# LilYau350/Variance-Aware-Weight

Hardware: AMD Instinct MI355X
Metric: training images/sec (higher is better)
Workload: dtype bf16; 1 GPU; DiT-B/4, 4x32x32 latents, 1000 classes; Trainer.train_step: q_sample + fwd + lambda-weighted MSE + bwd + AdamW + EMA; global batch 256 = 256 per GPU; global_batch=256, per_gpu_batch=256, parallelism=dp1, weight_type=lambda, hip_graph=False

## Files before the change

### include/vaw_hip.h

```cpp
#ifndef VAW_HIP_H
#define VAW_HIP_H
#include <stdint.h>

#ifdef __cplusplus
extern "C" {
#endif

typedef enum { VAW_OK = 0, VAW_ERR_INVALID = -1, VAW_ERR_LAUNCH = -2, VAW_ERR_UNSUPPORTED = -3 } vaw_status;
typedef enum { VAW_F32 = 0, VAW_BF16 = 1,
               VAW_FP8 = 2, VAW_BF8 = 3  } vaw_dtype;
typedef void* vaw_stream;

int vaw_version(void);
const char* vaw_last_error_string(void);


int vaw_qsample_fwd(const float* x0, const float* noise, const int64_t* t, const float* tab_a, const float* tab_s,
                    int num_timesteps, float* x_t, int B, int64_t per_sample, vaw_stream stream);

int vaw_mix_rows(const float* x, const float* y, const float* ca, const float* cb, float* out, int B,
                 int64_t per_sample, vaw_stream stream);

int vaw_wmse_fwd(const float* model_out, const float* x0, const float* noise, const float* ca, const float* cb,
                 const float* w, float* mse, int B, int64_t per_sample, vaw_stream stream);
int vaw_wmse_bwd(const float* model_out, const float* x0, const float* noise, const float* ca, const float* cb,
                 const float* w, const float* gmse, float* dout, int B, int64_t per_sample, vaw_stream stream);

int vaw_vb_fwd(const float* mean_out, const float* var_out, const float* x0, const float* x_t, const float* coef,
               int mean_mode, int var_mode, float scale, float* vb, int B, int64_t per_sample, vaw_stream stream);
int vaw_vb_bwd(const float* mean_out, const float* var_out, const float* x0, const float* x_t, const float* coef,
               int mean_mode, int var_mode, float scale, const float* gvb, float* d_mean, float* d_var, int B,
               int64_t per_sample, vaw_stream stream);

int vaw_sample_step(int kind, const float* mean_out, const float* var_out, const float* x, const float* noise,
                    const float* coef, int mean_mode, int var_mode, int clip_denoised, float eta, float* sample,
                    float* pred_xstart, float* mean, float* log_variance, int B, int64_t per_sample, vaw_stream stream);


typedef struct {
    const float* bias;
    int act;
    const void* aux_in;
    void* aux_out;
    const float* gate;
    int64_t gate_ld;
    const void* resid;
    const float* rowadd;
    int rows_per_batch;
    float alpha;
    float beta;
    int out_f32;
    float* colsum_out;
    float colsum_beta;
    int resid_is_act;
    float* rowsum_a_out;
    float rowsum_a_beta;
    float* colsum_partial_out;
    int64_t* colsum_rows_out;
} vaw_epilogue;

int vaw_gemm(vaw_dtype dt, int a_kmajor, int b_kmajor, int64_t M, int64_t N, int64_t K, const void* A, int64_t lda,
             const void* B, int64_t ldb, void* C, int64_t ldc, const vaw_epilogue* epi_host, float* workspace,
             int64_t workspace_floats, vaw_stream stream);

typedef struct {
    const void* dy;
    const void* x;
    float* dw;
    int64_t M, N, ld_dy, ld_x, ld_dw;
    float alpha;
    int pad_;
    const float* scale_dy;
    const float* scale_x;
} vaw_wgrad_problem;
int64_t vaw_wgrad_grouped_desc_bytes(int n_problems);
int vaw_wgrad_grouped(vaw_dtype dt, int n_problems, const vaw_wgrad_problem* problems, int64_t K, float beta, void* desc_dev,
                      int upload, float* workspace, int64_t workspace_floats, vaw_stream stream);

int64_t vaw_fp8_quantize_workspace_floats(void);
int vaw_fp8_quantize(vaw_dtype src_dt, vaw_dtype dst_format, const void* src, int64_t R, int64_t C, int64_t ld, void* q, int64_t ldq,
                     void* qt, int64_t ldt, float* scale_out, float* workspace, int64_t workspace_floats, vaw_stream stream);
int vaw_fp8_quantize_delayed(vaw_dtype src_dt, vaw_dtype dst_format, const void* src, int64_t R, int64_t C, int64_t ld, void* q,
                             int64_t ldq, void* qt, int64_t ldt, float* state, vaw_stream stream);
int vaw_fp8_scale_update(float* states, int64_t n, vaw_stream stream);
typedef struct {
    const float* src;
    void* q;
    void* qt;
    float* state;
    int64_t R, C, ld, ldq, ldt;
} vaw_fp8_quant_job;
int64_t vaw_fp8_quantize_batched_desc_bytes(int n_jobs);
int vaw_fp8_quantize_delayed_batched(int n_jobs, const vaw_fp8_quant_job* jobs, void* desc_dev, int upload, vaw_stream stream);
int vaw_gemm_fp8(vaw_dtype a_format, int64_t M, int64_t N, int64_t K, const void* A, int64_t lda, const float* scale_a,
                 const void* B, int64_t ldb, const float* scale_b, void* C, int64_t ldc, const vaw_epilogue* epi_host,
                 float* c_fp8_state, vaw_dtype c_fp8_format, float* workspace, int64_t workspace_floats, vaw_stream stream);
int vaw_fp8_transpose(const void* q, int64_t R, int64_t C, int64_t ldq, void* qt, int64_t ldt, vaw_stream stream);

void vaw_p8_set_reserved_cus(int n);
int vaw_gemm_uses_bf16_mfma(vaw_dtype dt, int64_t M, int64_t N, int64_t K, const void* A, int64_t lda, const void* B,
                            int64_t ldb);

int64_t vaw_colsum_workspace_floats(int64_t M, int64_t N);
int vaw_colsum(vaw_dtype dt, const void* X, int64_t M, int64_t N, int64_t ldx, float* out, float beta,
               float* workspace, int64_t workspace_floats, vaw_stream stream);
int vaw_reduce_rows(const float* partial, int64_t R, int64_t N, float* out, float beta, vaw_stream stream);
typedef struct {
    const float* partial;
    float* out;
    int64_t R, N;
} vaw_reduce_job;
int64_t vaw_reduce_rows_batched_desc_bytes(int n_jobs);
int vaw_reduce_rows_batched(int n_jobs, const vaw_reduce_job* jobs, float beta, void* desc_dev, int upload, vaw_stream stream);


int vaw_ln_modulate_fwd(vaw_dtype dt, const float* x, const float* shift, const float* scale, int64_t mod_ld,
                        void* out, float* mean, float* rstd, int B, int T, int D, float eps, vaw_stream stream);
int vaw_ln_modulate_bwd(vaw_dtype dt, const void* dout, const float* x, const float* mean, const float* rstd,
                        const float* scale, int64_t mod_ld, const float* dres_in, float* dx, float* dshift,
                        float* dscale, int64_t dmod_ld, int B, int T, int D, float* workspace, int64_t workspace_floats,
                        vaw_stream stream);
int vaw_ln_modulate_fwd_fp8(const float* x, const float* shift, const float* scale, int64_t mod_ld, void* q_out, float* q_state,
                            vaw_dtype q_format, float* mean, float* rstd, int B, int T, int D, float eps, vaw_stream stream);
int vaw_gate_bwd_fp8(const float* dres, const void* y, const float* gate, int64_t mod_ld, void* dy_q, float* q_state,
                     vaw_dtype q_format, float* dgate, int64_t dmod_ld, float* dy_colsum_partial, int B, int T, int D,
                     float* workspace, int64_t workspace_floats, vaw_stream stream);
int64_t vaw_row_bwd_workspace_floats(int B, int T, int D);
typedef enum { VAW_ROW_LN_FWD = 0, VAW_ROW_LN_FWD_FP8 = 1, VAW_ROW_LN_BWD = 2, VAW_ROW_GATE_BWD = 3, VAW_ROW_GATE_BWD_FP8 = 4,
               VAW_ROW_LN_BWD_GATE = 5, VAW_ROW_LN_BWD_GATE_FP8 = 6, VAW_ROW_COLSUM = 7 } vaw_row_kind;
typedef enum {
    VAW_RV_LN_FWD = 0,
    VAW_RV_ROW_BWD = 1,
    VAW_RV_ROW_GATE = 2,
    VAW_RV_ROW_FUSE = 3,
    VAW_RV_ROW_FUSE8 = 4,
    VAW_RV_COLSUM_BF16X8 = 5, VAW_RV_COLSUM_VEC4 = 6, VAW_RV_COLSUM_SCALAR = 7
} vaw_row_variant;
typedef struct {
    int variant;
    int nv;
    int nc, rows_per_chunk;
    int grid_x, block;
    int64_t lds_bytes;
    int64_t workspace_floats;
} vaw_row_launch;
int vaw_row_plan(vaw_row_kind kind, vaw_dtype dt, int64_t B, int64_t T, int64_t D, int64_t ldx, int64_t base_addr,
                 int64_t workspace_floats, vaw_row_launch* out);
int vaw_gate_bwd(vaw_dtype dt, const float* dres, const void* y, const float* gate, int64_t mod_ld, void* dy,
                 float* dgate, int64_t dmod_ld, float* dy_colsum_partial, int B, int T, int D, float* workspace, int64_t workspace_floats, vaw_stream stream);
int vaw_ln_modulate_bwd_gate(vaw_dtype dt, const void* dout, const float* x, const float* mean, const float* rstd,
                             const float* scale, int64_t mod_ld, const float* dres_in, float* dx, float* dshift, float* dscale,
                             int64_t dmod_ld, const void* y_next, const float* gate_next, void* dy_next, float* dgate_next,
                             float* dy_colsum_partial, int B, int T, int D, float* workspace, int64_t workspace_floats, vaw_stream stream);
int vaw_ln_modulate_bwd_gate_fp8(const void* dout, const float* x, const float* mean, const float* rstd, const float* scale,
                                 int64_t mod_ld, const float* dres_in, float* dx, float* dshift, float* dscale, int64_t dmod_ld,
                                 const void* y_next, const float* gate_next, void* dy_q, float* q_state, vaw_dtype q_format,
                                 float* dgate_next, float* dy_colsum_partial, int B, int T, int D, float* workspace,
                                 int64_t workspace_floats, vaw_stream stream);

int vaw_patchify(vaw_dtype dt, const float* img, void* tok, int B, int C, int H, int W, int p, vaw_stream stream);
int vaw_patchify_bwd(const float* dtok, float* dimg, int B, int C, int H, int W, int p, vaw_stream stream);
int vaw_unpatchify(vaw_dtype dt, const float* tok, float* img, int B, int C, int H, int W, int p,
                   vaw_stream stream);
int vaw_unpatchify_bwd(vaw_dtype dt, const float* dimg, void* dtok, int B, int C, int H, int W, int p,
                       vaw_stream stream);

int vaw_timestep_embedding(vaw_dtype dt, const float* t, void* out, int B, int dim, float max_period,
                           vaw_stream stream);
int vaw_silu_fwd(vaw_dtype dt, const float* x, void* out, int64_t n, vaw_stream stream);
int vaw_silu_bwd(const float* x, const float* dy, float* dx, int64_t n, vaw_stream stream);
int vaw_add_embedding(const float* a, const float* table, const int64_t* idx, float* out, int B, int D,
                      int num_rows, vaw_stream stream);
int vaw_embedding_bwd(const float* dc, const int64_t* idx, float* dtable, int B, int D, int num_rows, float beta,
                      vaw_stream stream);

typedef struct {
    int B, H, T, hd;
    int64_t q_sb, q_sh, q_st, q_sd;
    int64_t o_sb, o_sh, o_st, o_sd;
    float scale;
} vaw_attn_desc;
int vaw_attn_fwd(vaw_dtype dt, const vaw_attn_desc* d_host, const void* q, const void* k, const void* v, void* o,
                 float* lse, vaw_stream stream);
int vaw_attn_bwd(vaw_dtype dt, const vaw_attn_desc* d_host, const void* q, const void* k, const void* v,
                 const void* o, const void* d_o, const float* lse, float* delta, void* dq, void* dk, void* dv,
                 vaw_stream stream);
int vaw_attn_bwd_colsum(vaw_dtype dt, const vaw_attn_desc* d, const void* q, const void* k, const void* v, const void* o,
                        const void* d_o, const float* lse, float* delta, void* dq, void* dk, void* dv, float* colsum_partial,
                        int64_t* rows_out, vaw_stream stream);

typedef enum { VAW_ATTN_DIR_FWD = 0, VAW_ATTN_DIR_BWD = 1, VAW_ATTN_DIR_BWD_COLSUM = 2 } vaw_attn_dir;
typedef enum {
    VAW_AV_ROWWISE = 0,
    VAW_AV_FWD_T64 = 1,
    VAW_AV_FWD_G1 = 2,
    VAW_AV_FWD_G2 = 3,
    VAW_AV_FWD_BIG = 4,
    VAW_AV_BWD_T64 = 5,
    VAW_AV_BWD_G1 = 6,
    VAW_AV_BWD_G2 = 7,
    VAW_AV_BWD_BIG_NT2 = 8,
    VAW_AV_BWD_BIG_NT4 = 9
} vaw_attn_variant;
typedef struct {
    int variant;
    int hd_image;
    int launches;
    int grid_x, grid_y, block;
    int64_t lds_bytes;
    int lds_cap_raised;
    int64_t colsum_rows;
    int status;
} vaw_attn_launch;
int vaw_attn_plan(int dir, vaw_dtype dt, const vaw_attn_desc* d, int64_t q, int64_t k, int64_t v, int64_t o_or_do, int64_t dq,
                  int64_t dk, int64_t dv, vaw_attn_launch* out);


int vaw_conv3x3_narrow(vaw_dtype dt, int mode, const void* in, const void* w, const float* bias, void* out, int B, int H,
                       int W, int Cn, int Cw, vaw_stream stream);

int64_t vaw_groupnorm_workspace_floats(int B, int HW, int C);
int vaw_groupnorm_fwd(vaw_dtype dt, const void* x, const float* gamma, const float* beta, const float* scale,
                      const float* shift, int64_t film_ld, int silu, void* y, float* mean, float* rstd, int B, int HW,
                      int C, int G, float eps, float* workspace, vaw_stream stream);
int vaw_groupnorm_bwd(vaw_dtype dt, const void* dout, const void* x, const float* mean, const float* rstd,
                      const float* gamma, const float* beta, const float* scale, const float* shift, int64_t film_ld,
                      int silu, const void* dx_add, void* dx, float* dgamma, float* dbeta, float grad_beta, float* dscale,
                      float* dshift, int64_t dfilm_ld, int B, int HW, int C, int G, float* workspace, vaw_stream stream);
int vaw_im2col3x3(vaw_dtype dt, const void* x, void* col, int B, int H, int W, int C, vaw_stream stream);
int vaw_col2im3x3(vaw_dtype dt, const void* dcol, void* dx, int B, int H, int W, int C, vaw_stream stream);
int vaw_conv3x3(vaw_dtype dt, int mode, const void* act, const void* act2, const void* w, void* out, int B, int H, int W,
                int Ci, int Co, const vaw_epilogue* epi_host, float* workspace, int64_t workspace_floats, vaw_stream stream);
int64_t vaw_conv3x3_wgrad_small_workspace_floats(int B, int H, int W, int Ci, int Co);
int vaw_conv3x3_wgrad_small(vaw_dtype dt, const void* dy, const void* x, float* dw, float beta, int B, int H, int W, int Ci,
                            int Co, float* workspace, int64_t workspace_floats, vaw_stream stream);
int vaw_resample2(vaw_dtype dt, const void* in, void* out, int B, int Ho, int Wo, int C, int mode, float s,
                  vaw_stream stream);
int vaw_concat_channels(vaw_dtype dt, void* a, void* b, void* cat, int64_t M, int Ca, int Cb, int split,
                        vaw_stream stream);
int vaw_add_inplace(vaw_dtype dt, void* dst, const void* src, int64_t n, vaw_stream stream);
int vaw_mul(vaw_dtype dt, const void* a, const void* b, void* out, int64_t n, vaw_stream stream);
int vaw_subsample2(vaw_dtype dt, const void* in, void* out, int B, int Ho, int Wo, int C, int mode, vaw_stream stream);
int vaw_rowvec_add(vaw_dtype dt, void* h, const float* e, int64_t ld, int B, int HW, int C, vaw_stream stream);
int vaw_rowvec_sum(vaw_dtype dt, const void* dh, float* de, int64_t ld, int B, int HW, int C, float beta, vaw_stream stream);
int vaw_nchw_to_nhwc(vaw_dtype dt, const float* nchw, void* nhwc, int B, int C, int HW, vaw_stream stream);
int vaw_nhwc_to_nchw(vaw_dtype dt, const void* nhwc, float* nchw, int B, int C, int HW, vaw_stream stream);


int64_t vaw_sumsq_workspace_floats(void);
int vaw_sumsq(const float* g, int64_t n, float* sumsq_out, int accumulate, float* workspace, vaw_stream stream);
int vaw_adamw_ema_step(float* p, float* g, float* m, float* v, float* ema, void* shadow_bf16, int64_t n, float lr,
                       float beta1, float beta2, float eps, float weight_decay, float bc1, float bc2,
                       float ema_decay, const float* sumsq, float clip_max_norm, int zero_grad, vaw_stream stream);
// ... 21 lines not shown
```

### variance-aware-weight_amd/_lib.py

```python
import ctypes as C
import os

import torch

_HERE = os.path.dirname(os.path.abspath(__file__))
LIB_PATH = os.environ.get("VAW_HIP_LIB") or os.path.join(_HERE, "libvaw_hip.so")

F32, BF16, FP8, BF8 = 0, 1, 2, 3
TORCH_DTYPE = {F32: torch.float32, BF16: torch.bfloat16}

_p, _i, _l, _f = C.c_void_p, C.c_int, C.c_int64, C.c_float


class Epilogue(C.Structure):
    _fields_ = [("bias", _p), ("act", _i), ("aux_in", _p), ("aux_out", _p), ("gate", _p), ("gate_ld", _l),
                ("resid", _p), ("rowadd", _p), ("rows_per_batch", _i), ("alpha", _f), ("beta", _f), ("out_f32", _i),
                ("colsum_out", _p), ("colsum_beta", _f), ("resid_is_act", _i), ("rowsum_a_out", _p), ("rowsum_a_beta", _f),
                ("colsum_partial_out", _p), ("colsum_rows_out", C.POINTER(C.c_int64))]


class AttnDesc(C.Structure):
    _fields_ = [("B", _i), ("H", _i), ("T", _i), ("hd", _i), ("q_sb", _l), ("q_sh", _l), ("q_st", _l), ("q_sd", _l),
                ("o_sb", _l), ("o_sh", _l), ("o_st", _l), ("o_sd", _l), ("scale", _f)]


class RowLaunch(C.Structure):
    _fields_ = [("variant", _i), ("nv", _i), ("nc", _i), ("rows_per_chunk", _i), ("grid_x", _i), ("block", _i), ("lds_bytes", _l),
                ("workspace_floats", _l)]


class AttnLaunch(C.Structure):
    _fields_ = [("variant", _i), ("hd_image", _i), ("launches", _i), ("grid_x", _i), ("grid_y", _i), ("block", _i), ("lds_bytes", _l),
                ("lds_cap_raised", _i), ("colsum_rows", _l), ("status", _i)]


ATTN_FWD, ATTN_BWD, ATTN_BWD_COLSUM = range(3)
(AV_ROWWISE, AV_FWD_T64, AV_FWD_G1, AV_FWD_G2, AV_FWD_BIG, AV_BWD_T64, AV_BWD_G1, AV_BWD_G2, AV_BWD_BIG_NT2,
 AV_BWD_BIG_NT4) = range(10)
AV_NAMES = ("rowwise", "fwd_t64", "fwd_g1", "fwd_g2", "fwd_big", "bwd_t64", "bwd_g1", "bwd_g2", "bwd_big_nt2", "bwd_big_nt4")

ROW_LN_FWD, ROW_LN_FWD_FP8, ROW_LN_BWD, ROW_GATE_BWD, ROW_GATE_BWD_FP8, ROW_LN_BWD_GATE, ROW_LN_BWD_GATE_FP8, ROW_COLSUM = range(8)
RV_LN_FWD, RV_ROW_BWD, RV_ROW_GATE, RV_ROW_FUSE, RV_ROW_FUSE8, RV_COLSUM_BF16X8, RV_COLSUM_VEC4, RV_COLSUM_SCALAR = range(8)

_PROTOS = {
    "vaw_qsample_fwd": [_p, _p, _p, _p, _p, _i, _p, _i, _l, _p],
    "vaw_mix_rows": [_p, _p, _p, _p, _p, _i, _l, _p],
    "vaw_wmse_fwd": [_p, _p, _p, _p, _p, _p, _p, _i, _l, _p],
    "vaw_wmse_bwd": [_p, _p, _p, _p, _p, _p, _p, _p, _i, _l, _p],
    "vaw_gemm": [_i, _i, _i, _l, _l, _l, _p, _l, _p, _l, _p, _l, C.POINTER(Epilogue), _p, _l, _p],
    "vaw_gemm_uses_bf16_mfma": [_i, _l, _l, _l, _p, _l, _p, _l],
    "vaw_colsum": [_i, _p, _l, _l, _l, _p, _f, _p, _l, _p],
    "vaw_ln_modulate_fwd": [_i, _p, _p, _p, _l, _p, _p, _p, _i, _i, _i, _f, _p],
    "vaw_ln_modulate_bwd": [_i, _p, _p, _p, _p, _p, _l, _p, _p, _p, _p, _l, _i, _i, _i, _p, _l, _p],
    "vaw_gate_bwd": [_i, _p, _p, _p, _l, _p, _p, _l, _p, _i, _i, _i, _p, _l, _p],
    "vaw_reduce_rows": [_p, _l, _l, _p, _f, _p],
    "vaw_reduce_rows_batched": [_i, _p, _f, _p, _i, _p],
    "vaw_ln_modulate_bwd_gate": [_i, _p, _p, _p, _p, _p, _l, _p, _p, _p, _p, _l, _p, _p, _p, _p, _p, _i, _i, _i, _p, _l, _p],
    "vaw_ln_modulate_bwd_gate_fp8": [_p, _p, _p, _p, _p, _l, _p, _p, _p, _p, _l, _p, _p, _p, _p, _i, _p, _p, _i, _i, _i, _p, _l, _p],
    "vaw_patchify": [_i, _p, _p, _i, _i, _i, _i, _i, _p],
    "vaw_patchify_bwd": [_p, _p, _i, _i, _i, _i, _i, _p],
    "vaw_unpatchify": [_i, _p, _p, _i, _i, _i, _i, _i, _p],
    "vaw_unpatchify_bwd": [_i, _p, _p, _i, _i, _i, _i, _i, _p],
    "vaw_timestep_embedding": [_i, _p, _p, _i, _i, _f, _p],
    "vaw_silu_fwd": [_i, _p, _p, _l, _p],
    "vaw_silu_bwd": [_p, _p, _p, _l, _p],
    "vaw_add_embedding": [_p, _p, _p, _p, _i, _i, _i, _p],
    "vaw_embedding_bwd": [_p, _p, _p, _i, _i, _i, _f, _p],
    "vaw_attn_fwd": [_i, C.POINTER(AttnDesc), _p, _p, _p, _p, _p, _p],
    "vaw_attn_bwd": [_i, C.POINTER(AttnDesc), _p, _p, _p, _p, _p, _p, _p, _p, _p, _p, _p],
    "vaw_attn_bwd_colsum": [_i, C.POINTER(AttnDesc), _p, _p, _p, _p, _p, _p, _p, _p, _p, _p, _p, C.POINTER(C.c_int64), _p],
    "vaw_comm_unique_id": [_p],
    "vaw_comm_init": [_p, _i, _i],
    "vaw_comm_world": [],
    "vaw_comm_destroy": [],
    "vaw_allreduce_bucket_start": [_p, _l, _i, _p],
    "vaw_reduce_scatter_bucket_start": [_p, _l, _i, _p],
    "vaw_allgather_bucket_start": [_p, _l, _i, _p],
    "vaw_allreduce_bucket_wait": [_p],
    "vaw_groupnorm_fwd": [_i, _p, _p, _p, _p, _p, _l, _i, _p, _p, _p, _i, _i, _i, _i, _f, _p, _p],
    "vaw_groupnorm_bwd": [_i, _p, _p, _p, _p, _p, _p, _p, _p, _l, _i, _p, _p, _p, _p, _f, _p, _p, _l, _i, _i, _i, _i, _p, _p],
    "vaw_im2col3x3": [_i, _p, _p, _i, _i, _i, _i, _p],
    "vaw_col2im3x3": [_i, _p, _p, _i, _i, _i, _i, _p],
    "vaw_conv3x3": [_i, _i, _p, _p, _p, _p, _i, _i, _i, _i, _i, C.POINTER(Epilogue), _p, _l, _p],
    "vaw_vb_fwd": [_p, _p, _p, _p, _p, _i, _i, _f, _p, _i, _l, _p],
    "vaw_vb_bwd": [_p, _p, _p, _p, _p, _i, _i, _f, _p, _p, _p, _i, _l, _p],
    "vaw_sample_step": [_i, _p, _p, _p, _p, _p, _i, _i, _i, _f, _p, _p, _p, _p, _i, _l, _p],
    "vaw_conv3x3_narrow": [_i, _i, _p, _p, _p, _p, _i, _i, _i, _i, _i, _p],
    "vaw_conv3x3_wgrad_small": [_i, _p, _p, _p, _f, _i, _i, _i, _i, _i, _p, _l, _p],
    "vaw_resample2": [_i, _p, _p, _i, _i, _i, _i, _i, _f, _p],
    "vaw_concat_channels": [_i, _p, _p, _p, _l, _i, _i, _i, _p],
    "vaw_add_inplace": [_i, _p, _p, _l, _p],
    "vaw_mul": [_i, _p, _p, _p, _l, _p],
    "vaw_subsample2": [_i, _p, _p, _i, _i, _i, _i, _i, _p],
    "vaw_rowvec_add": [_i, _p, _p, _l, _i, _i, _i, _p],
    "vaw_rowvec_sum": [_i, _p, _p, _l, _i, _i, _i, _f, _p],
    "vaw_nchw_to_nhwc": [_i, _p, _p, _i, _i, _i, _p],
    "vaw_nhwc_to_nchw": [_i, _p, _p, _i, _i, _i, _p],
    "vaw_sumsq": [_p, _l, _p, _i, _p, _p],
    "vaw_adamw_ema_step_dev": [_p, _p, _p, _p, _p, _p, _l, _p, _f, _f, _f, _f, _f, _p, _f, _i, _p],
    "vaw_adamw_ema_step": [_p, _p, _p, _p, _p, _p, _l, _f, _f, _f, _f, _f, _f, _f, _f, _p, _f, _i, _p],
    "vaw_ema_update": [_p, _p, _l, _f, _p],
    "vaw_cast_bf16": [_p, _p, _l, _p],
    "vaw_uncast_bf16": [_p, _p, _l, _f, _p],
    "vaw_wgrad_grouped": [_i, _i, _p, _l, _f, _p, _i, _p, _l, _p],
    "vaw_fp8_quantize": [_i, _i, _p, _l, _l, _l, _p, _l, _p, _l, _p, _p, _l, _p],
    "vaw_fp8_quantize_delayed": [_i, _i, _p, _l, _l, _l, _p, _l, _p, _l, _p, _p],
    "vaw_fp8_scale_update": [_p, _l, _p],
    "vaw_fp8_quantize_delayed_batched": [_i, _p, _p, _i, _p],
    "vaw_gemm_fp8": [_i, _l, _l, _l, _p, _l, _p, _p, _l, _p, _p, _l, C.POINTER(Epilogue), _p, _i, _p, _l, _p],
    "vaw_fp8_transpose": [_p, _l, _l, _l, _p, _l, _p],
    "vaw_ln_modulate_fwd_fp8": [_p, _p, _p, _l, _p, _p, _i, _p, _p, _i, _i, _i, _f, _p],
    "vaw_gate_bwd_fp8": [_p, _p, _p, _l, _p, _p, _i, _p, _l, _p, _i, _i, _i, _p, _l, _p],
    "vaw_row_plan": [_i, _i, _l, _l, _l, _l, _l, _l, C.POINTER(RowLaunch)],
    "vaw_attn_plan": [_i, _i, C.POINTER(AttnDesc), _l, _l, _l, _l, _l, _l, _l, C.POINTER(AttnLaunch)],
}

_lib = None


class VawError(RuntimeError):
    pass


def lib():
    global _lib
    if _lib is None:
        if not os.path.exists(LIB_PATH):
            raise VawError(f"{LIB_PATH} not found: build it with `python -c 'import __graft_entry__ as g; g.build()'` "
                           "(there is no CPU fallback for the HIP path)")
        L = C.CDLL(LIB_PATH)
        for name, args in _PROTOS.items():
            if not hasattr(L, name) and os.environ.get("VAW_HIP_LIB"):
                continue
            fn = getattr(L, name)
            fn.argtypes = args
            fn.restype = _i
        L.vaw_version.restype = _i
        L.vaw_last_error_string.restype = C.c_char_p
        L.vaw_colsum_workspace_floats.argtypes = [_l, _l]
        L.vaw_colsum_workspace_floats.restype = _l
        L.vaw_row_bwd_workspace_floats.argtypes = [_i, _i, _i]
        L.vaw_row_bwd_workspace_floats.restype = _l
        L.vaw_conv3x3_wgrad_small_workspace_floats.argtypes = [_i, _i, _i, _i, _i]
        L.vaw_conv3x3_wgrad_small_workspace_floats.restype = _l
        L.vaw_groupnorm_workspace_floats.argtypes = [_i, _i, _i]
        L.vaw_groupnorm_workspace_floats.restype = _l
        L.vaw_wgrad_grouped_desc_bytes.argtypes = [_i]
        L.vaw_wgrad_grouped_desc_bytes.restype = _l
# ... 51 lines not shown
```

### variance-aware-weight_amd/csrc/capi.hip

```cpp
#include <stdarg.h>
#include <stdio.h>

#include "common.h"

static thread_local char g_err[512] = "";

void vaw_set_error(const char* fmt, ...) {
    va_list ap;
    va_start(ap, fmt);
    vsnprintf(g_err, sizeof(g_err), fmt, ap);
    va_end(ap);
}

extern "C" int vaw_version(void) { return 100; }
extern "C" const char* vaw_last_error_string(void) { return g_err; }

__global__ void __launch_bounds__(64) cu_hog_kernel(uint64_t ticks) {
    extern __shared__ char hog_lds[];
    if (threadIdx.x == 0) hog_lds[0] = 1;
    const uint64_t t0 = __builtin_amdgcn_s_memrealtime();
    while (__builtin_amdgcn_s_memrealtime() - t0 < ticks) __builtin_amdgcn_s_sleep(64);
}
extern "C" int vaw_debug_cu_hog(int n_wgs, int microseconds, vaw_stream stream) {
    VAW_CHECK_ARG(n_wgs > 0 && n_wgs <= 256 && microseconds > 0 && microseconds <= 2000000, "cu_hog: arguments");
    static bool attr = false;
    if (!attr) { (void)hipFuncSetAttribute((const void*)cu_hog_kernel, hipFuncAttributeMaxDynamicSharedMemorySize, 160 * 1024); attr = true; }
    cu_hog_kernel<<<n_wgs, 64, 160 * 1024, (hipStream_t)stream>>>((uint64_t)microseconds * 100);
    VAW_CHECK_LAUNCH("cu_hog");
    return VAW_OK;
}

#include <mutex>
#include <string.h>
#include <vector>
hipError_t vaw_upload_table(void* dev, const void* host, size_t bytes, hipStream_t s) {
    static std::mutex mu;
    static std::vector<void*> keep;
    void* pinned = nullptr;
    hipError_t rc = hipHostMalloc(&pinned, bytes, hipHostMallocDefault);
    if (rc != hipSuccess) return rc;
    memcpy(pinned, host, bytes);
    {
        std::lock_guard<std::mutex> g(mu);
        keep.push_back(pinned);
    }
    return hipMemcpyAsync(dev, pinned, bytes, hipMemcpyHostToDevice, s);
}
```

### variance-aware-weight_amd/csrc/elementwise.hip

```cpp
#include "common.h"

static inline int stream_grid(int64_t work_items, int block) {
    int64_t g = (work_items + block - 1) / block;
    const int64_t cap = 256 * 8;
    return (int)(g < 1 ? 1 : (g > cap ? cap : g));
}

template <bool GATHER>
__global__ void mix_rows_kernel(const float* __restrict__ x, const float* __restrict__ y, const float* __restrict__ ca,
                                const float* __restrict__ cb, const int64_t* __restrict__ t, int T,
                                float* __restrict__ out, int64_t n) {
    const int b = blockIdx.y;
    float a, c;
    if (GATHER) {
        const int64_t tt = t[b];
        const bool ok = tt >= 0 && tt < T;
        a = ok ? ca[tt] : __builtin_nanf("");
        c = ok ? cb[tt] : __builtin_nanf("");
    } else {
        a = ca[b];
        c = cb[b];
    }
    const float* xr = x + (int64_t)b * n;
    const float* yr = y + (int64_t)b * n;
    float* orow = out + (int64_t)b * n;
    const int64_t n4 = ((n & 3) == 0) ? n / 4 : 0;
    for (int64_t i = blockIdx.x * (int64_t)blockDim.x + threadIdx.x; i < n4; i += (int64_t)gridDim.x * blockDim.x) {
        f32x4 xv = load4(xr + 4 * i), yv = load4(yr + 4 * i);
        store4(orow + 4 * i, a * xv + c * yv);
    }
    for (int64_t i = n4 * 4 + blockIdx.x * (int64_t)blockDim.x + threadIdx.x; i < n; i += (int64_t)gridDim.x * blockDim.x)
        orow[i] = a * xr[i] + c * yr[i];
}

extern "C" int vaw_qsample_fwd(const float* x0, const float* noise, const int64_t* t, const float* tab_a,
                               const float* tab_s, int num_timesteps, float* x_t, int B, int64_t per_sample,
                               vaw_stream stream) {
    VAW_CHECK_ARG(B > 0 && per_sample > 0 && num_timesteps > 0, "qsample: bad sizes B=%d n=%ld", B, (long)per_sample);
    int gx = stream_grid(per_sample / 4 + 1, 256);
    dim3 grid(gx > 64 ? 64 : gx, B);
    mix_rows_kernel<true><<<grid, 256, 0, (hipStream_t)stream>>>(x0, noise, tab_a, tab_s, t, num_timesteps, x_t, per_sample);
    VAW_CHECK_LAUNCH("qsample");
    return VAW_OK;
}

extern "C" int vaw_mix_rows(const float* x, const float* y, const float* ca, const float* cb, float* out, int B,
                            int64_t per_sample, vaw_stream stream) {
    VAW_CHECK_ARG(B > 0 && per_sample > 0, "mix_rows: bad sizes");
    int gx = stream_grid(per_sample / 4 + 1, 256);
    dim3 grid(gx > 64 ? 64 : gx, B);
    mix_rows_kernel<false><<<grid, 256, 0, (hipStream_t)stream>>>(x, y, ca, cb, nullptr, 0, out, per_sample);
    VAW_CHECK_LAUNCH("mix_rows");
    return VAW_OK;
}

__global__ void wmse_fwd_kernel(const float* __restrict__ o, const float* __restrict__ x0, const float* __restrict__ nz,
                                const float* __restrict__ ca, const float* __restrict__ cb, const float* __restrict__ w,
                                float* __restrict__ mse, int64_t n) {
    __shared__ float scratch[16];
    const int b = blockIdx.x;
    const float a = ca[b], c = cb[b];
    const float* orow = o + (int64_t)b * n;
    const float* xr = x0 + (int64_t)b * n;
    const float* nr = nz + (int64_t)b * n;
    float acc = 0.f;
    const int64_t n4 = ((n & 3) == 0) ? n / 4 : 0;
    for (int64_t i = threadIdx.x; i < n4; i += blockDim.x) {
        f32x4 d = a * load4(xr + 4 * i) + c * load4(nr + 4 * i) - load4(orow + 4 * i);
        acc += d[0] * d[0] + d[1] * d[1] + d[2] * d[2] + d[3] * d[3];
    }
    for (int64_t i = n4 * 4 + threadIdx.x; i < n; i += blockDim.x) {
        float d = a * xr[i] + c * nr[i] - orow[i];
        acc += d * d;
    }
    float tot = block_sum(acc, scratch);
    if (threadIdx.x == 0) mse[b] = w[b] * (tot / (float)n);
}

__global__ void wmse_bwd_kernel(const float* __restrict__ o, const float* __restrict__ x0, const float* __restrict__ nz,
                                const float* __restrict__ ca, const float* __restrict__ cb, const float* __restrict__ w,
                                const float* __restrict__ gmse, float* __restrict__ dout, int64_t n) {
    const int b = blockIdx.y;
    const float a = ca[b], c = cb[b];
    const float k = gmse[b] * w[b] * 2.f / (float)n;
    const float* orow = o + (int64_t)b * n;
    const float* xr = x0 + (int64_t)b * n;
    const float* nr = nz + (int64_t)b * n;
    float* dr = dout + (int64_t)b * n;
    const int64_t n4 = ((n & 3) == 0) ? n / 4 : 0;
    for (int64_t i = blockIdx.x * (int64_t)blockDim.x + threadIdx.x; i < n4; i += (int64_t)gridDim.x * blockDim.x)
        store4(dr + 4 * i, k * (load4(orow + 4 * i) - a * load4(xr + 4 * i) - c * load4(nr + 4 * i)));
    for (int64_t i = n4 * 4 + blockIdx.x * (int64_t)blockDim.x + threadIdx.x; i < n; i += (int64_t)gridDim.x * blockDim.x)
        dr[i] = k * (orow[i] - a * xr[i] - c * nr[i]);
}

extern "C" int vaw_wmse_fwd(const float* model_out, const float* x0, const float* noise, const float* ca,
                            const float* cb, const float* w, float* mse, int B, int64_t per_sample,
                            vaw_stream stream) {
    VAW_CHECK_ARG(B > 0 && per_sample > 0, "wmse_fwd: bad sizes");
    wmse_fwd_kernel<<<B, 1024, 0, (hipStream_t)stream>>>(model_out, x0, noise, ca, cb, w, mse, per_sample);
    VAW_CHECK_LAUNCH("wmse_fwd");
    return VAW_OK;
}

extern "C" int vaw_wmse_bwd(const float* model_out, const float* x0, const float* noise, const float* ca,
                            const float* cb, const float* w, const float* gmse, float* dout, int B,
                            int64_t per_sample, vaw_stream stream) {
    VAW_CHECK_ARG(B > 0 && per_sample > 0, "wmse_bwd: bad sizes");
    int gx = stream_grid(per_sample / 4 + 1, 256);
    dim3 grid(gx > 64 ? 64 : gx, B);
    wmse_bwd_kernel<<<grid, 256, 0, (hipStream_t)stream>>>(model_out, x0, noise, ca, cb, w, gmse, dout, per_sample);
    VAW_CHECK_LAUNCH("wmse_bwd");
    return VAW_OK;
}

#define VB_NCOEF 8
struct VbElem {
    float val;
    float d_lv;
    float d_mean;
};
__device__ __forceinline__ float vb_cdf(float z, float& dcdf) {
    const float k = 0.7978845608028654f;
    const float th = tanhf(k * (z + 0.044715f * (z * z * z)));
    dcdf = 0.5f * (1.f - th * th) * k * (1.f + 3.f * 0.044715f * z * z);
    return 0.5f * (1.f + th);
}
__device__ __forceinline__ VbElem vb_elem(float x0, float true_mean, float true_lv, float mean, float lv, bool t0) {
    VbElem r;
    if (!t0) {
        const float e2 = expf(-lv), d = true_mean - mean, ratio = expf(true_lv - lv);
        r.val = 0.5f * (-1.0f + lv - true_lv + ratio + (d * d) * e2);
        r.d_lv = 0.5f * (1.f - ratio - (d * d) * e2);
        r.d_mean = -d * e2;
        return r;
    }
    const float cx = x0 - mean, inv = expf(-(0.5f * lv));
    const float pin = inv * (cx + 1.0f / 255.0f), mnn = inv * (cx - 1.0f / 255.0f);
    float dp, dm;
    const float cp = vb_cdf(pin, dp), cm = vb_cdf(mnn, dm);
    float lp, g_pin = 0.f, g_min = 0.f;
    if (x0 < -0.999f) {
        lp = logf(fmaxf(cp, 1e-12f));
        if (cp >= 1e-12f) g_pin = dp / cp;
    } else if (x0 > 0.999f) {
        const float q = 1.f - cm;
        lp = logf(fmaxf(q, 1e-12f));
        if (q >= 1e-12f) g_min = -dm / q;
    } else {
        const float dl = cp - cm;
        lp = logf(fmaxf(dl, 1e-12f));
        if (dl >= 1e-12f) { g_pin = dp / dl; g_min = -dm / dl; }
    }
    r.val = -lp;
    r.d_lv = 0.5f * (g_pin * pin + g_min * mnn);
    r.d_mean = inv * (g_pin + g_min);
    return r;
}
__device__ __forceinline__ void vb_model(const float* c, int mean_mode, int var_mode, float xt, float m, float v, float& mean,
                                         float& lv) {
    mean = mean_mode == 1 ? m : c[0] * (c[4] * xt + c[5] * m) + c[1] * xt;
    if (var_mode == 1) lv = v;
    else if (var_mode == 2) { const float frac = (v + 1.f) / 2.f; lv = frac * c[3] + (1.f - frac) * c[2]; }
    else lv = c[3];
}

__global__ void vb_fwd_kernel(const float* __restrict__ mean_out, const float* __restrict__ var_out, const float* __restrict__ x0,
                              const float* __restrict__ xt, const float* __restrict__ coef, int mean_mode, int var_mode,
                              float scale, float* __restrict__ vb, int64_t n) {
    __shared__ float scratch[16];
    const int b = blockIdx.x;
    float c[VB_NCOEF];
#pragma unroll
    for (int i = 0; i < VB_NCOEF; ++i) c[i] = coef[b * VB_NCOEF + i];
    const bool t0 = c[6] != 0.f;
    const int64_t base = (int64_t)b * n;
    float acc = 0.f;
    for (int64_t i = threadIdx.x; i < n; i += blockDim.x) {
        const float x = x0[base + i], z = xt[base + i];
        float mean, lv;
        vb_model(c, mean_mode, var_mode, z, mean_out[base + i], var_out ? var_out[base + i] : 0.f, mean, lv);
        acc += vb_elem(x, c[0] * x + c[1] * z, c[2], mean, lv, t0).val;
    }
    const float tot = block_sum(acc, scratch);
    if (threadIdx.x == 0) vb[b] = scale * ((tot / (float)n) / 0.6931471805599453f);
}

__global__ void vb_bwd_kernel(const float* __restrict__ mean_out, const float* __restrict__ var_out, const float* __restrict__ x0,
                              const float* __restrict__ xt, const float* __restrict__ coef, int mean_mode, int var_mode,
                              float scale, const float* __restrict__ gvb, float* __restrict__ d_mean, float* __restrict__ d_var,
                              int64_t n) {
    const int b = blockIdx.y;
    float c[VB_NCOEF];
#pragma unroll
    for (int i = 0; i < VB_NCOEF; ++i) c[i] = coef[b * VB_NCOEF + i];
// ... 48 lines not shown
    for (int i = 0; i < SS_NCOEF; ++i) c[i] = coef[b * SS_NCOEF + i];
    const float mask = c[11] != 0.f ? 0.f : 1.f;
    const float sigma = (eta * c[9]) * c[12];
    const float ddim_c = sqrtf(1.f - c[10] - sigma * sigma);
    const int64_t base = (int64_t)b * n;
    for (int64_t i = blockIdx.x * (int64_t)blockDim.x + threadIdx.x; i < n; i += (int64_t)gridDim.x * blockDim.x) {
        const float xv = x[base + i], m = mean_out[base + i];
        float pred = c[0] * xv + c[1] * m;
        if (clip) pred = fminf(fmaxf(pred, -1.f), 1.f);
        float lv;
        if (var_mode == 1) lv = var_out[base + i];
        else if (var_mode == 2) { const float frac = (var_out[base + i] + 1.f) / 2.f; lv = frac * c[5] + (1.f - frac) * c[4]; }
        else lv = c[5];
        const float mean = mean_mode == 1 ? m : c[2] * pred + c[3] * xv;
        if (pred_out) pred_out[base + i] = pred;
        if (mean_o) mean_o[base + i] = mean;
        if (logvar_o) logvar_o[base + i] = lv;
        if (kind == 1) {
            sample[base + i] = mean + (mask * expf(0.5f * lv)) * noise[base + i];
        } else if (kind == 2) {
            const float eps = (c[6] * xv - pred) / c[7];
            const float mp = pred * c[8] + ddim_c * eps;
            sample[base + i] = mp + (mask * sigma) * noise[base + i];
        }
    }
}

extern "C" int vaw_sample_step(int kind, const float* mean_out, const float* var_out, const float* x, const float* noise,
                               const float* coef, int mean_mode, int var_mode, int clip_denoised, float eta, float* sample,
                               float* pred_xstart, float* mean, float* log_variance, int B, int64_t per_sample,
                               vaw_stream stream) {
    VAW_CHECK_ARG(B > 0 && per_sample > 0 && mean_out && x && coef && kind >= 0 && kind <= 2, "sample_step: bad arguments");
    VAW_CHECK_ARG((mean_mode == 0 || mean_mode == 1) && var_mode >= 0 && var_mode <= 2 && (var_mode == 0 || var_out),
                  "sample_step: bad modes (learned variance needs var_out)");
    VAW_CHECK_ARG(kind == 0 || (sample && noise), "sample_step: kind 1/2 need noise and sample");
    int gx = stream_grid(per_sample, 256);
    dim3 grid(gx > 64 ? 64 : gx, B);
    sample_step_kernel<<<grid, 256, 0, (hipStream_t)stream>>>(mean_out, var_out, x, noise, coef, kind, mean_mode, var_mode,
                                                             clip_denoised, eta, sample, pred_xstart, mean, log_variance, per_sample);
    VAW_CHECK_LAUNCH("sample_step");
    return VAW_OK;
}

template <typename T>
__global__ void timestep_embedding_kernel(const float* __restrict__ t, T* __restrict__ out, int B, int dim,
                                          float neg_log_period) {
    const int half = dim / 2;
    for (int64_t idx = blockIdx.x * (int64_t)blockDim.x + threadIdx.x; idx < (int64_t)B * dim;
         idx += (int64_t)gridDim.x * blockDim.x) {
        const int b = (int)(idx / dim), j = (int)(idx % dim);
        float v = 0.f;
        if (j < 2 * half) {
            const int i = j < half ? j : j - half;
            const float f = expf(neg_log_period * (float)i / (float)half);
            const float ang = t[b] * f;
            v = j < half ? cosf(ang) : sinf(ang);
        }
        out[idx] = from_f32<T>(v);
    }
}

extern "C" int vaw_timestep_embedding(vaw_dtype dt, const float* t, void* out, int B, int dim, float max_period,
                                      vaw_stream stream) {
    VAW_CHECK_ARG(B > 0 && dim > 0, "timestep_embedding: bad sizes");
    const float nl = -logf(max_period);
    int grid = stream_grid((int64_t)B * dim, 256);
    if (dt == VAW_F32)
        timestep_embedding_kernel<float><<<grid, 256, 0, (hipStream_t)stream>>>(t, (float*)out, B, dim, nl);
    else
        timestep_embedding_kernel<bf16_t><<<grid, 256, 0, (hipStream_t)stream>>>(t, (bf16_t*)out, B, dim, nl);
    VAW_CHECK_LAUNCH("timestep_embedding");
    return VAW_OK;
}

template <typename T>
__global__ void silu_fwd_kernel(const float* __restrict__ x, T* __restrict__ out, int64_t n) {
    for (int64_t i = blockIdx.x * (int64_t)blockDim.x + threadIdx.x; i < n; i += (int64_t)gridDim.x * blockDim.x)
        out[i] = from_f32<T>(silu_f(x[i]));
}
__global__ void silu_bwd_kernel(const float* __restrict__ x, const float* __restrict__ dy, float* __restrict__ dx, int64_t n) {
    for (int64_t i = blockIdx.x * (int64_t)blockDim.x + threadIdx.x; i < n; i += (int64_t)gridDim.x * blockDim.x)
        dx[i] = dy[i] * silu_grad_f(x[i]);
}
extern "C" int vaw_silu_fwd(vaw_dtype dt, const float* x, void* out, int64_t n, vaw_stream stream) {
    VAW_CHECK_ARG(n > 0, "silu_fwd: n<=0");
    int grid = stream_grid(n, 256);
    if (dt == VAW_F32) silu_fwd_kernel<float><<<grid, 256, 0, (hipStream_t)stream>>>(x, (float*)out, n);
    else silu_fwd_kernel<bf16_t><<<grid, 256, 0, (hipStream_t)stream>>>(x, (bf16_t*)out, n);
    VAW_CHECK_LAUNCH("silu_fwd");
    return VAW_OK;
}
extern "C" int vaw_silu_bwd(const float* x, const float* dy, float* dx, int64_t n, vaw_stream stream) {
    VAW_CHECK_ARG(n > 0, "silu_bwd: n<=0");
    silu_bwd_kernel<<<stream_grid(n, 256), 256, 0, (hipStream_t)stream>>>(x, dy, dx, n);
    VAW_CHECK_LAUNCH("silu_bwd");
    return VAW_OK;
}

__global__ void add_embedding_kernel(const float* __restrict__ a, const float* __restrict__ table,
                                     const int64_t* __restrict__ idx, float* __restrict__ out, int B, int D, int rows) {
    for (int64_t i = blockIdx.x * (int64_t)blockDim.x + threadIdx.x; i < (int64_t)B * D; i += (int64_t)gridDim.x * blockDim.x) {
        const int b = (int)(i / D), d = (int)(i % D);
        const int64_t r = idx[b];
        out[i] = a[i] + ((r >= 0 && r < rows) ? table[r * D + d] : __builtin_nanf(""));
    }
}
__global__ void __launch_bounds__(256)
embedding_bwd_kernel(const float* __restrict__ dc, const int64_t* __restrict__ idx, float* __restrict__ dtable, int B, int D,
                     int rows, float beta) {
    __shared__ int s_idx[1024];
    const int r = blockIdx.x;
    constexpr int MAXC = 8;
    for (int d0 = 0; d0 < D; d0 += 256 * MAXC) {
        float acc[MAXC];
#pragma unroll
        for (int j = 0; j < MAXC; ++j) acc[j] = 0.f;
        for (int b0 = 0; b0 < B; b0 += 1024) {
            const int nb = B - b0 < 1024 ? B - b0 : 1024;
            __syncthreads();
            for (int i = threadIdx.x; i < nb; i += 256) s_idx[i] = (int)idx[b0 + i];
            __syncthreads();
            for (int i = 0; i < nb; ++i) {
                if (s_idx[i] != r) continue;
                const float* src = dc + (int64_t)(b0 + i) * D + d0;
#pragma unroll
                for (int j = 0; j < MAXC; ++j) {
                    const int d = threadIdx.x + 256 * j;
                    if (d0 + d < D) acc[j] += src[d];
                }
            }
        }
#pragma unroll
        for (int j = 0; j < MAXC; ++j) {
            const int d = d0 + threadIdx.x + 256 * j;
            if (d < D) {
                float* o = dtable + (int64_t)r * D + d;
                *o = (beta != 0.f ? beta * *o : 0.f) + acc[j];
            }
        }
    }
}
extern "C" int vaw_add_embedding(const float* a, const float* table, const int64_t* idx, float* out, int B, int D,
                                 int num_rows, vaw_stream stream) {
    VAW_CHECK_ARG(B > 0 && D > 0 && num_rows > 0, "add_embedding: bad sizes");
    add_embedding_kernel<<<stream_grid((int64_t)B * D, 256), 256, 0, (hipStream_t)stream>>>(a, table, idx, out, B, D, num_rows);
    VAW_CHECK_LAUNCH("add_embedding");
    return VAW_OK;
}
extern "C" int vaw_embedding_bwd(const float* dc, const int64_t* idx, float* dtable, int B, int D, int num_rows,
                                 float beta, vaw_stream stream) {
    VAW_CHECK_ARG(B > 0 && D > 0 && num_rows > 0, "embedding_bwd: bad sizes");
    embedding_bwd_kernel<<<num_rows, 256, 0, (hipStream_t)stream>>>(dc, idx, dtable, B, D, num_rows, beta);
    VAW_CHECK_LAUNCH("embedding_bwd");
    return VAW_OK;
}

template <typename T, bool CONV_ORDER, bool TO_TOKENS>
__global__ void patch_shuffle_kernel(const float* __restrict__ img_in, float* __restrict__ img_out,
                                     const float* __restrict__ tok_in_f32, T* __restrict__ tok_out, int B, int C, int H,
                                     int W, int p) {
    const int hp = H / p, wp = W / p;
    const int64_t total = (int64_t)B * C * H * W;
    const int K = C * p * p;
    for (int64_t e = blockIdx.x * (int64_t)blockDim.x + threadIdx.x; e < total; e += (int64_t)gridDim.x * blockDim.x) {
        int x = (int)(e % W);
        int64_t r = e / W;
        int y = (int)(r % H);
        r /= H;
        int c = (int)(r % C);
        int b = (int)(r / C);
        const int ty = y / p, i = y % p, tx = x / p, j = x % p;
        const int64_t row = ((int64_t)b * hp + ty) * wp + tx;
        const int col = CONV_ORDER ? (c * p + i) * p + j : (i * p + j) * C + c;
        if (TO_TOKENS) tok_out[row * K + col] = from_f32<T>(img_in[e]);
        else img_out[e] = tok_in_f32[row * K + col];
    }
}

extern "C" int vaw_patchify(vaw_dtype dt, const float* img, void* tok, int B, int C, int H, int W, int p,
                            vaw_stream stream) {
    VAW_CHECK_ARG(B > 0 && C > 0 && p > 0 && H % p == 0 && W % p == 0, "patchify: bad sizes");
    int grid = stream_grid((int64_t)B * C * H * W, 256);
    if (dt == VAW_F32)
        patch_shuffle_kernel<float, true, true><<<grid, 256, 0, (hipStream_t)stream>>>(img, nullptr, nullptr, (float*)tok, B, C, H, W, p);
    else
        patch_shuffle_kernel<bf16_t, true, true><<<grid, 256, 0, (hipStream_t)stream>>>(img, nullptr, nullptr, (bf16_t*)tok, B, C, H, W, p);
    VAW_CHECK_LAUNCH("patchify");
    return VAW_OK;
}
extern "C" int vaw_patchify_bwd(const float* dtok, float* dimg, int B, int C, int H, int W, int p, vaw_stream stream) {
    VAW_CHECK_ARG(B > 0 && C > 0 && p > 0 && H % p == 0 && W % p == 0, "patchify_bwd: bad sizes");
    int grid = stream_grid((int64_t)B * C * H * W, 256);
    patch_shuffle_kernel<float, true, false><<<grid, 256, 0, (hipStream_t)stream>>>(nullptr, dimg, dtok, nullptr, B, C, H, W, p);
    VAW_CHECK_LAUNCH("patchify_bwd");
    return VAW_OK;
}
extern "C" int vaw_unpatchify(vaw_dtype dt, const float* tok, float* img, int B, int C, int H, int W, int p,
                              vaw_stream stream) {
    (void)dt;
    VAW_CHECK_ARG(B > 0 && C > 0 && p > 0 && H % p == 0 && W % p == 0, "unpatchify: bad sizes");
    int grid = stream_grid((int64_t)B * C * H * W, 256);
    patch_shuffle_kernel<float, false, false><<<grid, 256, 0, (hipStream_t)stream>>>(nullptr, img, tok, nullptr, B, C, H, W, p);
    VAW_CHECK_LAUNCH("unpatchify");
    return VAW_OK;
}
extern "C" int vaw_unpatchify_bwd(vaw_dtype dt, const float* dimg, void* dtok, int B, int C, int H, int W, int p,
                                  vaw_stream stream) {
    VAW_CHECK_ARG(B > 0 && C > 0 && p > 0 && H % p == 0 && W % p == 0, "unpatchify_bwd: bad sizes");
    int grid = stream_grid((int64_t)B * C * H * W, 256);
    if (dt == VAW_F32)
        patch_shuffle_kernel<float, false, true><<<grid, 256, 0, (hipStream_t)stream>>>(dimg, nullptr, nullptr, (float*)dtok, B, C, H, W, p);
    else
        patch_shuffle_kernel<bf16_t, false, true><<<grid, 256, 0, (hipStream_t)stream>>>(dimg, nullptr, nullptr, (bf16_t*)dtok, B, C, H, W, p);
    VAW_CHECK_LAUNCH("unpatchify_bwd");
    return VAW_OK;
}

#define SUMSQ_MAX_BLOCKS 2048
__global__ void sumsq_partial_kernel(const float* __restrict__ g, int64_t n, float* __restrict__ partial) {
    __shared__ float scratch[16];
    float acc = 0.f;
    const int64_t n4 = n / 4;
    for (int64_t i = blockIdx.x * (int64_t)blockDim.x + threadIdx.x; i < n4; i += (int64_t)gridDim.x * blockDim.x) {
        f32x4 v = load4(g + 4 * i);
        acc += v[0] * v[0] + v[1] * v[1] + v[2] * v[2] + v[3] * v[3];
    }
    for (int64_t i = n4 * 4 + blockIdx.x * (int64_t)blockDim.x + threadIdx.x; i < n; i += (int64_t)gridDim.x * blockDim.x)
        acc += g[i] * g[i];
    float tot = block_sum(acc, scratch);
// ... 184 lines not shown
```

### variance-aware-weight_amd/csrc/layernorm.hip

```cpp
#include <stdio.h>
#include <stdlib.h>

#include "common.h"

template <typename T, int NV>
__global__ void __launch_bounds__(256)
ln_modulate_fwd_kernel(const float* __restrict__ x, const float* __restrict__ shift, const float* __restrict__ scale,
                       int64_t mod_ld, T* __restrict__ out, float* __restrict__ mean_out, float* __restrict__ rstd_out,
                       int64_t M, int Tt, int D, float eps, unsigned char* __restrict__ q_out = nullptr,
                       float* __restrict__ q_state = nullptr, int q_e5m2 = 0) {
    const int lane = threadIdx.x & 63;
    const float q_inv = q_out ? 1.f / q_state[0] : 1.f;
    float am = 0.f;
    const int wave = __builtin_amdgcn_readfirstlane(threadIdx.x >> 6);
    const int64_t row0 = (int64_t)blockIdx.x * 4 + wave, rstep = (int64_t)gridDim.x * 4;
    unsigned colc[NV];
#pragma unroll
    for (int i = 0; i < NV; ++i) {
        const unsigned c = (unsigned)(i * 64 + lane) * 4u;
        colc[i] = c < (unsigned)D ? c : 0u;
    }
    f32x4 nx[NV];
    if (row0 < M) {
#pragma unroll
        for (int i = 0; i < NV; ++i) nx[i] = __builtin_nontemporal_load(reinterpret_cast<const f32x4*>(x + row0 * D + colc[i]));
    }
    for (int64_t row = row0; row < M; row += rstep) {
        const int b = (int)(row / Tt);
        f32x4 v[NV];
        float s = 0.f;
#pragma unroll
        for (int i = 0; i < NV; ++i) {
            const int c = (i * 64 + lane) * 4;
            v[i] = c < D ? nx[i] : f32x4{0, 0, 0, 0};
            s += v[i][0] + v[i][1] + v[i][2] + v[i][3];
        }
        if (row + rstep < M) {
#pragma unroll
            for (int i = 0; i < NV; ++i) nx[i] = __builtin_nontemporal_load(reinterpret_cast<const f32x4*>(x + (row + rstep) * D + colc[i]));
        }
        const float mean = wave_sum(s) / (float)D;
        float q = 0.f;
#pragma unroll
        for (int i = 0; i < NV; ++i) {
            const int c = (i * 64 + lane) * 4;
            if (c < D) {
                f32x4 d = v[i] - mean;
                q += d[0] * d[0] + d[1] * d[1] + d[2] * d[2] + d[3] * d[3];
            }
        }
        const float rstd = rsqrtf(wave_sum(q) / (float)D + eps);
        if (lane == 0) {
            mean_out[row] = mean;
            rstd_out[row] = rstd;
        }
        const float* sh = shift + (int64_t)b * mod_ld;
        const float* sc = scale + (int64_t)b * mod_ld;
        if (q_out) {
#pragma unroll
            for (int i = 0; i < NV; ++i) {
                const int c = (i * 64 + lane) * 4;
                if (c < D) {
                    f32x4 xh = (v[i] - mean) * rstd;
                    *reinterpret_cast<unsigned*>(q_out + row * D + c) = fp8_word_of_bf16(xh * (1.f + load4(sc + c)) + load4(sh + c), q_inv, q_e5m2, am);
                }
            }
            continue;
        }
        T* orow = out + row * D;
#pragma unroll
        for (int i = 0; i < NV; ++i) {
            const int c = (i * 64 + lane) * 4;
            if (c < D) {
                f32x4 xh = (v[i] - mean) * rstd;
                store4(orow + c, xh * (1.f + load4(sc + c)) + load4(sh + c));
            }
        }
    }
    if (q_out) {
        __shared__ float wmax[4];
        am = wave_max(am);
        if (lane == 0) wmax[threadIdx.x >> 6] = am;
        __syncthreads();
        if (threadIdx.x < 64) fp8_amax_commit(fmaxf(fmaxf(wmax[0], wmax[1]), fmaxf(wmax[2], wmax[3])), q_state + 1, lane);
    }
}

template <typename T, int NV, bool GATE_ONLY, bool QOUT = false, bool FUSE = false>
__global__ void __launch_bounds__((FUSE && NV > 3) ? 512 : 1024)
row_bwd_kernel(const T* __restrict__ dout, const float* __restrict__ x, const float* __restrict__ mean,
               const float* __restrict__ rstd, const float* __restrict__ scale, int64_t mod_ld,
               const float* __restrict__ dres_in, float* __restrict__ dx, float* __restrict__ dshift,
               float* __restrict__ dscale, int64_t dmod_ld, int Tt, int D,
               const float* __restrict__ dres, const T* __restrict__ y, const float* __restrict__ gate,
               T* __restrict__ dy, float* __restrict__ dgate, float* __restrict__ dy_colpart,
               int rows_per_chunk, float* __restrict__ part,
               unsigned char* __restrict__ q_out = nullptr, float* __restrict__ q_state = nullptr, int q_e5m2 = 0) {
    static_assert(!(FUSE && GATE_ONLY), "FUSE extends the LayerNorm mode");
    constexpr int NQ = FUSE ? 4 : 2;
    extern __shared__ __attribute__((aligned(16))) float lds[];
    const float q_inv = ((GATE_ONLY || FUSE) && QOUT) ? 1.f / q_state[0] : 1.f;
    float q_am = 0.f;
    const int lane = threadIdx.x & 63, wid = threadIdx.x >> 6, nw = blockDim.x >> 6;
    const int b = blockIdx.x;
    const int t_begin = blockIdx.y * rows_per_chunk;
    const int t_end = t_begin + rows_per_chunk < Tt ? t_begin + rows_per_chunk : Tt;
    f32x4 acc0[NV], acc1[NV], sc[NV];
    f32x4 acc2[FUSE ? NV : 1], acc3[FUSE ? NV : 1];
    float* const sc_lds = lds + NQ * D;
    float* const gsc_lds = sc_lds + D;
#pragma unroll
    for (int i = 0; i < NV; ++i) {
        acc0[i] = f32x4{0, 0, 0, 0};
        acc1[i] = f32x4{0, 0, 0, 0};
        const int c = (i * 64 + lane) * 4;
        const float* src = GATE_ONLY ? gate : scale;
        sc[i] = c < D ? load4(src + (int64_t)b * mod_ld + c) : f32x4{0, 0, 0, 0};
        if (FUSE) {
            acc2[i] = acc3[i] = f32x4{0, 0, 0, 0};
            if (wid == 0 && c < D) {
                store4(sc_lds + c, 1.f + sc[i]);
                store4(gsc_lds + c, load4(gate + (int64_t)b * mod_ld + c));
            }
        }
    }
    if (FUSE) __syncthreads();
    for (int t = t_begin + wid; t < t_end; t += nw) {
        const int64_t row = (int64_t)b * Tt + t;
        if (GATE_ONLY) {
#pragma unroll
            for (int i = 0; i < NV; ++i) {
                const int c = (i * 64 + lane) * 4;
                if (c < D) {
                    f32x4 g = load4(dres + row * D + c);
                    f32x4 yv = load4(y + row * D + c);
                    f32x4 d = g * sc[i];
                    if (QOUT) *reinterpret_cast<unsigned*>(q_out + row * D + c) = fp8_word_of_bf16(d, q_inv, q_e5m2, q_am);
                    else store4(dy + row * D + c, d);
                    acc0[i] += g * yv;
                    f32x4 dr = {to_f32(from_f32<T>(d[0])), to_f32(from_f32<T>(d[1])), to_f32(from_f32<T>(d[2])), to_f32(from_f32<T>(d[3]))};
                    acc1[i] += dr;
                }
            }
        } else {
            const float mu = mean[row], rs = rstd[row];
            f32x4 g[NV], xh[NV];
            float s1 = 0.f, s2 = 0.f;
#pragma unroll
            for (int i = 0; i < NV; ++i) {
                const int c = (i * 64 + lane) * 4;
                if (c < D) {
                    f32x4 d = load4(dout + row * D + c);
                    xh[i] = (load4(x + row * D + c) - mu) * rs;
                    acc0[i] += d;
                    acc1[i] += d * xh[i];
                    g[i] = d * (FUSE ? load4(sc_lds + c) : 1.f + sc[i]);
                    s1 += g[i][0] + g[i][1] + g[i][2] + g[i][3];
                    f32x4 gx = g[i] * xh[i];
                    s2 += gx[0] + gx[1] + gx[2] + gx[3];
                } else {
                    g[i] = xh[i] = f32x4{0, 0, 0, 0};
                }
            }
            const float c1 = wave_sum(s1) / (float)D, c2 = wave_sum(s2) / (float)D;
#pragma unroll
            for (int i = 0; i < NV; ++i) {
                const int c = (i * 64 + lane) * 4;
                if (c < D) {
                    f32x4 r = (g[i] - c1 - xh[i] * c2) * rs;
                    if (dres_in) r += load4(dres_in + row * D + c);
                    store4(dx + row * D + c, r);
                    if (FUSE) {
                        const f32x4 yv = load4(y + row * D + c);
                        const f32x4 d = r * load4(gsc_lds + c);
                        if (QOUT) *reinterpret_cast<unsigned*>(q_out + row * D + c) = fp8_word_of_bf16(d, q_inv, q_e5m2, q_am);
                        else store4(dy + row * D + c, d);
                        acc2[i] += r * yv;
                        f32x4 dr = {to_f32(from_f32<T>(d[0])), to_f32(from_f32<T>(d[1])), to_f32(from_f32<T>(d[2])), to_f32(from_f32<T>(d[3]))};
                        acc3[i] += dr;
                    }
                }
            }
        }
    }
    if ((GATE_ONLY || FUSE) && QOUT) fp8_amax_commit(q_am, q_state + 1, lane);
    float* s0 = lds;
    float* s1p = lds + D;
    for (int i = threadIdx.x; i < NQ * D; i += blockDim.x) lds[i] = 0.f;
    __syncthreads();
    for (int w = 0; w < nw; ++w) {
        if (wid == w) {
#pragma unroll
            for (int i = 0; i < NV; ++i) {
                const int c = (i * 64 + lane) * 4;
                if (c < D) {
                    store4(s0 + c, load4(s0 + c) + acc0[i]);
                    store4(s1p + c, load4(s1p + c) + acc1[i]);
                    if (FUSE) {
                        store4(lds + 2 * D + c, load4(lds + 2 * D + c) + acc2[i]);
                        store4(lds + 3 * D + c, load4(lds + 3 * D + c) + acc3[i]);
                    }
                }
            }
        }
        __syncthreads();
    }
    if (part) {
        float* dst = part + ((int64_t)blockIdx.y * gridDim.x + b) * NQ * D;
        for (int c = threadIdx.x; c < NQ * D; c += blockDim.x) dst[c] = lds[c];
        return;
    }
    for (int c = threadIdx.x; c < D; c += blockDim.x) {
        if (GATE_ONLY) {
            dgate[(int64_t)b * dmod_ld + c] = s0[c];
            if (dy_colpart) dy_colpart[(int64_t)b * D + c] = s1p[c];
        } else {
            dshift[(int64_t)b * dmod_ld + c] = s0[c];
            dscale[(int64_t)b * dmod_ld + c] = s1p[c];
            if (FUSE) {
                dgate[(int64_t)b * dmod_ld + c] = lds[2 * D + c];
                if (dy_colpart) dy_colpart[(int64_t)b * D + c] = lds[3 * D + c];
            }
        }
    }
}

template <int NV, bool QOUT>
__global__ void __launch_bounds__(512)
row_bwd_fuse8_kernel(const bf16_t* __restrict__ dout, const float* __restrict__ x, const float* __restrict__ mean,
                     const float* __restrict__ rstd, const float* __restrict__ scale, int64_t mod_ld,
                     const float* __restrict__ dres_in, float* __restrict__ dx, float* __restrict__ dshift,
                     float* __restrict__ dscale, int64_t dmod_ld, int Tt, int D, const bf16_t* __restrict__ y,
                     const float* __restrict__ gate, bf16_t* __restrict__ dy, float* __restrict__ dgate, float* __restrict__ dy_colpart,
                     int rows_per_chunk, float* __restrict__ part, unsigned char* __restrict__ q_out, float* __restrict__ q_state,
                     int q_e5m2) {
    extern __shared__ __attribute__((aligned(16))) float lds[];
    const int lane = threadIdx.x & 63, wid = __builtin_amdgcn_readfirstlane(threadIdx.x >> 6), nw = blockDim.x >> 6;
    const int b = blockIdx.x;
    const int t_begin = blockIdx.y * rows_per_chunk;
    const int t_end = t_begin + rows_per_chunk < Tt ? t_begin + rows_per_chunk : Tt;
    float* const sc_lds = lds;
    float* const gsc_lds = lds + D;
    float* const slab = lds + 2 * D + wid * 4 * D;
    const float q_inv = QOUT ? 1.f / q_state[0] : 1.f;
    float q_am = 0.f;
    bool act[NV];
    unsigned col[NV], colc[NV];
#pragma unroll
    for (int i = 0; i < NV; ++i) {
        col[i] = (unsigned)(i * 64 + lane) * 4u;
        act[i] = col[i] < (unsigned)D;
        colc[i] = act[i] ? col[i] : 0u;
        if (act[i]) {
#pragma unroll
// ... 193 lines not shown
        p.variant = kind == VAW_ROW_LN_BWD ? VAW_RV_ROW_BWD : VAW_RV_ROW_GATE;
        p.block = pick_block(p.rows_per_chunk, row_waves(nv, 16));
        p.lds_bytes = 2 * D * (int64_t)sizeof(float);
    } else {
        p.block = pick_block(p.rows_per_chunk, 8);
        const int64_t lds8 = (2 + 4 * (int64_t)(p.block / 64)) * D * (int64_t)sizeof(float);
        const bool bf = kind == VAW_ROW_LN_BWD_GATE_FP8 || dt == VAW_BF16;
        if (bf && nv <= 5 && lds8 <= (int64_t)kRowLdsMax) {
            p.variant = VAW_RV_ROW_FUSE8;
            p.lds_bytes = lds8;
        } else {
            p.variant = VAW_RV_ROW_FUSE;
            p.lds_bytes = 6 * D * (int64_t)sizeof(float);
        }
    }
    *out = p;
    return VAW_OK;
}

#define DISPATCH_NV(nv, CALL)                                       \
    switch (nv) {                                                   \
        case 1: { constexpr int NV = 1; CALL; } break;              \
        case 2: { constexpr int NV = 2; CALL; } break;              \
        case 3: { constexpr int NV = 3; CALL; } break;              \
        case 4: { constexpr int NV = 4; CALL; } break;              \
        case 5: { constexpr int NV = 5; CALL; } break;              \
        case 6: { constexpr int NV = 6; CALL; } break;              \
        default: { constexpr int NV = 8; CALL; } break;             \
    }

#define ROW_PLAN(kind, dt, B, T, D, ldx, base, wsf)                                      \
    vaw_row_launch plan;                                                               \
    {                                                                                  \
        const int rc_ = vaw_row_plan(kind, dt, B, T, D, ldx, base, wsf, &plan);        \
        if (rc_ != VAW_OK) return rc_;                                                 \
    }

extern "C" int vaw_ln_modulate_fwd(vaw_dtype dt, const float* x, const float* shift, const float* scale, int64_t mod_ld,
                                   void* out, float* mean, float* rstd, int B, int T, int D, float eps,
                                   vaw_stream stream) {
    VAW_CHECK_ARG(B > 0 && T > 0 && D > 0 && D % 4 == 0 && D <= 2048 && mod_ld % 4 == 0,
                  "ln_modulate_fwd: need D%%4==0, D<=2048, mod_ld%%4==0 (D=%d)", D);
    ROW_PLAN(VAW_ROW_LN_FWD, dt, B, T, D, 0, 0, 0);
    const int64_t M = (int64_t)B * T;
    static int per_cu[2][9] = {};
    const int nvk = plan.nv, ti = dt == VAW_F32 ? 0 : 1;
    if (!per_cu[ti][nvk]) {
        int nb = 0;
        if (dt == VAW_F32) { DISPATCH_NV(nvk, (void)hipOccupancyMaxActiveBlocksPerMultiprocessor(&nb, ln_modulate_fwd_kernel<float, NV>, 256, 0)); }
        else { DISPATCH_NV(nvk, (void)hipOccupancyMaxActiveBlocksPerMultiprocessor(&nb, ln_modulate_fwd_kernel<bf16_t, NV>, 256, 0)); }
        per_cu[ti][nvk] = nb > 0 && nb <= 8 ? nb : 8;
    }
    const int64_t cap = 256LL * per_cu[ti][nvk];
    const int grid = (int)(plan.grid_x < cap ? plan.grid_x : cap);
    hipStream_t s = (hipStream_t)stream;
    if (dt == VAW_F32) {
        DISPATCH_NV(nvk, (ln_modulate_fwd_kernel<float, NV><<<grid, plan.block, 0, s>>>(x, shift, scale, mod_ld, (float*)out, mean, rstd, M, T, D, eps)));
    } else {
        DISPATCH_NV(nvk, (ln_modulate_fwd_kernel<bf16_t, NV><<<grid, plan.block, 0, s>>>(x, shift, scale, mod_ld, (bf16_t*)out, mean, rstd, M, T, D, eps)));
    }
    VAW_CHECK_LAUNCH("ln_modulate_fwd");
    return VAW_OK;
}

extern "C" int vaw_ln_modulate_fwd_fp8(const float* x, const float* shift, const float* scale, int64_t mod_ld, void* q_out,
                                       float* q_state, vaw_dtype q_format, float* mean, float* rstd, int B, int T, int D, float eps,
                                       vaw_stream stream) {
    VAW_CHECK_ARG(B > 0 && T > 0 && D > 0 && D % 4 == 0 && D <= 2048 && mod_ld % 4 == 0 && q_out && q_state,
                  "ln_modulate_fwd_fp8: need D%%4==0, D<=2048, mod_ld%%4==0 (D=%d)", D);
    VAW_CHECK_ARG(q_format == VAW_FP8 || q_format == VAW_BF8, "ln_modulate_fwd_fp8: q_format");
    ROW_PLAN(VAW_ROW_LN_FWD_FP8, VAW_BF16, B, T, D, 0, 0, 0);
    const int64_t M = (int64_t)B * T;
    hipStream_t s = (hipStream_t)stream;
    DISPATCH_NV(plan.nv, (ln_modulate_fwd_kernel<bf16_t, NV><<<plan.grid_x, plan.block, 0, s>>>(x, shift, scale, mod_ld, nullptr, mean, rstd, M, T, D, eps,
                                                                                             (unsigned char*)q_out, q_state, q_format == VAW_BF8)));
    VAW_CHECK_LAUNCH("ln_modulate_fwd_fp8");
    return VAW_OK;
}

extern "C" int vaw_ln_modulate_bwd(vaw_dtype dt, const void* dout, const float* x, const float* mean, const float* rstd,
                                   const float* scale, int64_t mod_ld, const float* dres_in, float* dx, float* dshift,
                                   float* dscale, int64_t dmod_ld, int B, int T, int D, float* workspace,
                                   int64_t workspace_floats, vaw_stream stream) {
    VAW_CHECK_ARG(B > 0 && T > 0 && D > 0 && D % 4 == 0 && D <= 2048 && mod_ld % 4 == 0,
                  "ln_modulate_bwd: need D%%4==0, D<=2048, mod_ld%%4==0 (D=%d)", D);
    ROW_PLAN(VAW_ROW_LN_BWD, dt, B, T, D, 0, 0, workspace ? workspace_floats : 0);
    hipStream_t s = (hipStream_t)stream;
    const int nc = plan.nc, rpc = plan.rows_per_chunk, block = plan.block;
    float* part = nc > 1 ? workspace : nullptr;
    const size_t lds = plan.lds_bytes;
    dim3 grid(B, nc);
    if (dt == VAW_F32) {
        DISPATCH_NV(plan.nv, (row_bwd_kernel<float, NV, false><<<grid, block, lds, s>>>((const float*)dout, x, mean, rstd, scale, mod_ld, dres_in, dx, dshift, dscale, dmod_ld, T, D, nullptr, nullptr, nullptr, nullptr, nullptr, nullptr, rpc, part)));
    } else {
        DISPATCH_NV(plan.nv, (row_bwd_kernel<bf16_t, NV, false><<<grid, block, lds, s>>>((const bf16_t*)dout, x, mean, rstd, scale, mod_ld, dres_in, dx, dshift, dscale, dmod_ld, T, D, nullptr, nullptr, nullptr, nullptr, nullptr, nullptr, rpc, part)));
    }
    if (nc > 1) row_bwd_finish_kernel<<<ceil_div((int64_t)B * D, 256), 256, 0, s>>>(part, nc, B, D, dshift, dmod_ld, dscale, dmod_ld);
    VAW_CHECK_LAUNCH("ln_modulate_bwd");
    return VAW_OK;
}

extern "C" int vaw_ln_modulate_bwd_gate(vaw_dtype dt, const void* dout, const float* x, const float* mean, const float* rstd,
                                        const float* scale, int64_t mod_ld, const float* dres_in, float* dx, float* dshift,
                                        float* dscale, int64_t dmod_ld, const void* y_next, const float* gate_next, void* dy_next,
                                        float* dgate_next, float* dy_colsum_partial, int B, int T, int D, float* workspace,
                                        int64_t workspace_floats, vaw_stream stream) {
    VAW_CHECK_ARG(B > 0 && T > 0 && D > 0 && D % 4 == 0 && D <= 2048 && mod_ld % 4 == 0,
                  "ln_modulate_bwd_gate: need D%%4==0, D<=2048, mod_ld%%4==0 (D=%d)", D);
    VAW_CHECK_ARG(y_next && gate_next && dy_next && dgate_next, "ln_modulate_bwd_gate: the gate operands are required");
    ROW_PLAN(VAW_ROW_LN_BWD_GATE, dt, B, T, D, 0, 0, workspace ? workspace_floats : 0);
    hipStream_t s = (hipStream_t)stream;
    const int nc = plan.nc, rpc = plan.rows_per_chunk, block = plan.block;
    float* part = nc > 1 ? workspace : nullptr;
    const size_t lds = plan.lds_bytes;
    dim3 grid(B, nc);
    if (plan.variant == VAW_RV_ROW_FUSE8) {
#define LAUNCH_FUSE8(NVv)                                                                                                              \
    row_bwd_fuse8_kernel<NVv, false><<<grid, block, row_fuse8_lds<NVv, false>(D, block), s>>>(                                          \
        (const bf16_t*)dout, x, mean, rstd, scale, mod_ld, dres_in, dx, dshift, dscale, dmod_ld, T, D, (const bf16_t*)y_next, gate_next, \
        (bf16_t*)dy_next, dgate_next, dy_colsum_partial, rpc, part, nullptr, nullptr, 0)
        const int nv = plan.nv;
        if (nv == 1) LAUNCH_FUSE8(1); else if (nv == 2) LAUNCH_FUSE8(2); else if (nv == 3) LAUNCH_FUSE8(3); else if (nv == 4) LAUNCH_FUSE8(4); else LAUNCH_FUSE8(5);
    } else if (dt == VAW_F32) {
        DISPATCH_NV(plan.nv, (row_bwd_kernel<float, NV, false, false, true><<<grid, block, lds, s>>>((const float*)dout, x, mean, rstd, scale, mod_ld, dres_in, dx, dshift, dscale, dmod_ld, T, D, nullptr, (const float*)y_next, gate_next, (float*)dy_next, dgate_next, dy_colsum_partial, rpc, part)));
    } else {
        DISPATCH_NV(plan.nv, (row_bwd_kernel<bf16_t, NV, false, false, true><<<grid, block, lds, s>>>((const bf16_t*)dout, x, mean, rstd, scale, mod_ld, dres_in, dx, dshift, dscale, dmod_ld, T, D, nullptr, (const bf16_t*)y_next, gate_next, (bf16_t*)dy_next, dgate_next, dy_colsum_partial, rpc, part)));
    }
    if (nc > 1)
        row_bwd_finish_kernel<<<ceil_div((int64_t)B * D, 256), 256, 0, s>>>(part, nc, B, D, dshift, dmod_ld, dscale, dmod_ld, 4, dgate_next, dmod_ld,
                                                                             dy_colsum_partial, D);
    VAW_CHECK_LAUNCH("ln_modulate_bwd_gate");
    return VAW_OK;
}

extern "C" int vaw_ln_modulate_bwd_gate_fp8(const void* dout, const float* x, const float* mean, const float* rstd, const float* scale,
                                            int64_t mod_ld, const float* dres_in, float* dx, float* dshift, float* dscale, int64_t dmod_ld,
                                            const void* y_next, const float* gate_next, void* dy_q, float* q_state, vaw_dtype q_format,
                                            float* dgate_next, float* dy_colsum_partial, int B, int T, int D, float* workspace,
                                            int64_t workspace_floats, vaw_stream stream) {
    VAW_CHECK_ARG(B > 0 && T > 0 && D > 0 && D % 4 == 0 && D <= 2048 && mod_ld % 4 == 0,
                  "ln_modulate_bwd_gate_fp8: need D%%4==0, D<=2048, mod_ld%%4==0 (D=%d)", D);
    VAW_CHECK_ARG(y_next && gate_next && dy_q && q_state && dgate_next, "ln_modulate_bwd_gate_fp8: the gate operands are required");
    VAW_CHECK_ARG(q_format == VAW_FP8 || q_format == VAW_BF8, "ln_modulate_bwd_gate_fp8: q_format");
    ROW_PLAN(VAW_ROW_LN_BWD_GATE_FP8, VAW_BF16, B, T, D, 0, 0, workspace ? workspace_floats : 0);
    hipStream_t s = (hipStream_t)stream;
    const int nc = plan.nc, rpc = plan.rows_per_chunk, block = plan.block;
    float* part = nc > 1 ? workspace : nullptr;
    const size_t lds = plan.lds_bytes;
    dim3 grid(B, nc);
    if (plan.variant == VAW_RV_ROW_FUSE8) {
#define LAUNCH_FUSE8Q(NVv)                                                                                                             \
    row_bwd_fuse8_kernel<NVv, true><<<grid, block, row_fuse8_lds<NVv, true>(D, block), s>>>(                                            \
        (const bf16_t*)dout, x, mean, rstd, scale, mod_ld, dres_in, dx, dshift, dscale, dmod_ld, T, D, (const bf16_t*)y_next, gate_next, \
        nullptr, dgate_next, dy_colsum_partial, rpc, part, (unsigned char*)dy_q, q_state, q_format == VAW_BF8)
        const int nv = plan.nv;
        if (nv == 1) LAUNCH_FUSE8Q(1); else if (nv == 2) LAUNCH_FUSE8Q(2); else if (nv == 3) LAUNCH_FUSE8Q(3); else if (nv == 4) LAUNCH_FUSE8Q(4); else LAUNCH_FUSE8Q(5);
    } else {
        DISPATCH_NV(plan.nv, (row_bwd_kernel<bf16_t, NV, false, true, true><<<grid, block, lds, s>>>((const bf16_t*)dout, x, mean, rstd, scale, mod_ld, dres_in, dx, dshift, dscale, dmod_ld, T, D, nullptr, (const bf16_t*)y_next, gate_next, nullptr, dgate_next, dy_colsum_partial, rpc, part, (unsigned char*)dy_q, q_state, q_format == VAW_BF8)));
    }
    if (nc > 1)
        row_bwd_finish_kernel<<<ceil_div((int64_t)B * D, 256), 256, 0, s>>>(part, nc, B, D, dshift, dmod_ld, dscale, dmod_ld, 4, dgate_next, dmod_ld,
                                                                             dy_colsum_partial, D);
    VAW_CHECK_LAUNCH("ln_modulate_bwd_gate_fp8");
    return VAW_OK;
}

extern "C" int vaw_gate_bwd(vaw_dtype dt, const float* dres, const void* y, const float* gate, int64_t mod_ld, void* dy,
                            float* dgate, int64_t dmod_ld, float* dy_colsum_partial, int B, int T, int D, float* workspace,
                            int64_t workspace_floats, vaw_stream stream) {
    VAW_CHECK_ARG(B > 0 && T > 0 && D > 0 && D % 4 == 0 && D <= 2048 && mod_ld % 4 == 0,
                  "gate_bwd: need D%%4==0, D<=2048, mod_ld%%4==0 (D=%d)", D);
    ROW_PLAN(VAW_ROW_GATE_BWD, dt, B, T, D, 0, 0, workspace ? workspace_floats : 0);
    hipStream_t s = (hipStream_t)stream;
    const int nc = plan.nc, rpc = plan.rows_per_chunk, block = plan.block;
    float* part = nc > 1 ? workspace : nullptr;
    const size_t lds = plan.lds_bytes;
    dim3 grid(B, nc);
    if (dt == VAW_F32) {
// ... 18 lines not shown
    float* part = nc > 1 ? workspace : nullptr;
    const size_t lds = plan.lds_bytes;
    dim3 grid(B, nc);
    DISPATCH_NV(plan.nv, (row_bwd_kernel<bf16_t, NV, true, true><<<grid, block, lds, s>>>(nullptr, nullptr, nullptr, nullptr, nullptr, mod_ld, nullptr, nullptr, nullptr, nullptr, dmod_ld, T, D, dres, (const bf16_t*)y, gate, nullptr, dgate, dy_colsum_partial, rpc, part, (unsigned char*)dy_q, q_state, q_format == VAW_BF8)));
    if (nc > 1) row_bwd_finish_kernel<<<ceil_div((int64_t)B * D, 256), 256, 0, s>>>(part, nc, B, D, dgate, dmod_ld, dy_colsum_partial, D);
    VAW_CHECK_LAUNCH("gate_bwd_fp8");
    return VAW_OK;
}

template <typename T>
__global__ void __launch_bounds__(256)
colsum_partial_kernel(const T* __restrict__ X, int64_t M, int64_t N, int64_t ldx, float* __restrict__ part_out) {
    __shared__ __attribute__((aligned(16))) float part[4][256];
    const int cg = threadIdx.x & 63, rg = threadIdx.x >> 6;
    const int64_t col = (int64_t)blockIdx.x * 256 + cg * 4;
    const int64_t r0 = (int64_t)blockIdx.y * 512;
    const int64_t r1 = r0 + 512 < M ? r0 + 512 : M;
    f32x4 acc = {0, 0, 0, 0};
    if (col < N) {
        if (col + 4 <= N) {
            for (int64_t r = r0 + rg; r < r1; r += 4) acc += load4(X + r * ldx + col);
        } else {
            for (int64_t r = r0 + rg; r < r1; r += 4)
                for (int j = 0; j < 4 && col + j < N; ++j) acc[j] += to_f32(X[r * ldx + col + j]);
        }
    }
    store4(&part[rg][cg * 4], acc);
    __syncthreads();
    const int64_t c = (int64_t)blockIdx.x * 256 + threadIdx.x;
    if (c < N)
        part_out[(int64_t)blockIdx.y * N + c] =
            ((part[0][threadIdx.x] + part[1][threadIdx.x]) + part[2][threadIdx.x]) + part[3][threadIdx.x];
}
__global__ void __launch_bounds__(1024)
colsum_final_kernel(const float* __restrict__ part, int64_t RB, int64_t N, float* __restrict__ out, float beta) {
    __shared__ float fold[32][33];
    const int cl = threadIdx.x & 31, grp = threadIdx.x >> 5;
    const int64_t c = (int64_t)blockIdx.x * 32 + cl;
    float acc = 0.f;
    if (c < N)
        for (int64_t r = grp; r < RB; r += 32) acc += part[r * N + c];
    fold[grp][cl] = acc;
    __syncthreads();
    if (grp == 0 && c < N) {
        float t = 0.f;
#pragma unroll
        for (int g = 0; g < 32; ++g) t += fold[g][cl];
        out[c] = (beta != 0.f ? beta * out[c] : 0.f) + t;
    }
}

__global__ void __launch_bounds__(256)
colsum_partial_bf16x8_kernel(const bf16_t* __restrict__ X, int64_t M, int64_t N, int64_t ldx, float* __restrict__ part_out) {
    __shared__ __attribute__((aligned(16))) float part[8][256];
    const int cg = threadIdx.x & 31, rg = threadIdx.x >> 5;
    const int64_t col = (int64_t)blockIdx.x * 256 + cg * 8;
    const int64_t r0 = (int64_t)blockIdx.y * 128;
    f32x4 a0 = {0, 0, 0, 0}, a1 = {0, 0, 0, 0};
    if (col < N) {
        bf16x8 v[16];
#pragma unroll
        for (int i = 0; i < 16; ++i) {
            const int64_t r = r0 + rg + 8 * i;
            v[i] = r < M ? *reinterpret_cast<const bf16x8*>(X + r * ldx + col) : bf16x8{0, 0, 0, 0, 0, 0, 0, 0};
        }
#pragma unroll
        for (int i = 0; i < 16; ++i) {
            a0 += f32x4{(float)v[i][0], (float)v[i][1], (float)v[i][2], (float)v[i][3]};
            a1 += f32x4{(float)v[i][4], (float)v[i][5], (float)v[i][6], (float)v[i][7]};
        }
    }
    store4(&part[rg][cg * 8], a0);
    store4(&part[rg][cg * 8 + 4], a1);
    __syncthreads();
    const int64_t c = (int64_t)blockIdx.x * 256 + threadIdx.x;
    if (c < N) {
        float t = 0.f;
#pragma unroll
        for (int g = 0; g < 8; ++g) t += part[g][threadIdx.x];
        part_out[(int64_t)blockIdx.y * N + c] = t;
    }
}

template <typename T>
__global__ void colsum_partial_scalar_kernel(const T* __restrict__ X, int64_t M, int64_t N, int64_t ldx, float* __restrict__ part_out) {
    const int64_t c = (int64_t)blockIdx.x * blockDim.x + threadIdx.x;
    if (c >= N) return;
    const int64_t r0 = (int64_t)blockIdx.y * 512, r1 = r0 + 512 < M ? r0 + 512 : M;
    float acc = 0.f;
    for (int64_t r = r0; r < r1; ++r) acc += to_f32(X[r * ldx + c]);
    part_out[(int64_t)blockIdx.y * N + c] = acc;
}

struct ReduceJobDev {
    const float* part;
    float* out;
    int64_t R, N;
    int block0, pad_;
};
__global__ void __launch_bounds__(1024)
colsum_final_batched_kernel(const ReduceJobDev* __restrict__ jobs, int n_jobs, float beta) {
    __shared__ float fold[32][33];
    int lo = 0, hi = n_jobs - 1;
    while (lo < hi) {
        const int mid = (lo + hi + 1) >> 1;
        if (jobs[mid].block0 <= (int)blockIdx.x) lo = mid; else hi = mid - 1;
    }
    const ReduceJobDev jb = jobs[lo];
    const int cl = threadIdx.x & 31, grp = threadIdx.x >> 5;
    const int64_t c = (int64_t)(blockIdx.x - jb.block0) * 32 + cl;
    float acc = 0.f;
    if (c < jb.N)
        for (int64_t r = grp; r < jb.R; r += 32) acc += jb.part[r * jb.N + c];
    fold[grp][cl] = acc;
    __syncthreads();
    if (grp == 0 && c < jb.N) {
        float t = 0.f;
#pragma unroll
        for (int g = 0; g < 32; ++g) t += fold[g][cl];
        jb.out[c] = (beta != 0.f ? beta * jb.out[c] : 0.f) + t;
    }
}

extern "C" int64_t vaw_reduce_rows_batched_desc_bytes(int n_jobs) { return (int64_t)n_jobs * (int64_t)sizeof(ReduceJobDev); }

extern "C" int vaw_reduce_rows_batched(int n_jobs, const vaw_reduce_job* jobs, float beta, void* desc_dev, int upload, vaw_stream stream) {
    VAW_CHECK_ARG(n_jobs > 0 && n_jobs <= 4096 && jobs && desc_dev, "reduce_rows_batched: bad arguments");
    static thread_local ReduceJobDev host[4096];
    int64_t blocks = 0;
    for (int j = 0; j < n_jobs; ++j) {
        VAW_CHECK_ARG(jobs[j].partial && jobs[j].out && jobs[j].R > 0 && jobs[j].N > 0, "reduce_rows_batched: job %d", j);
        host[j] = ReduceJobDev{jobs[j].partial, jobs[j].out, jobs[j].R, jobs[j].N, (int)blocks, 0};
        blocks += (jobs[j].N + 31) / 32;
        VAW_CHECK_ARG(blocks < (1 << 30), "reduce_rows_batched: too many columns");
    }
    hipStream_t s = (hipStream_t)stream;
    if (upload) {
        const hipError_t rc = vaw_upload_table(desc_dev, host, sizeof(ReduceJobDev) * n_jobs, s);
        VAW_CHECK_ARG(rc == hipSuccess, "reduce_rows_batched: descriptor upload failed: %s", hipGetErrorString(rc));
    }
    colsum_final_batched_kernel<<<(unsigned)blocks, 1024, 0, s>>>((const ReduceJobDev*)desc_dev, n_jobs, beta);
    VAW_CHECK_LAUNCH("reduce_rows_batched");
    return VAW_OK;
}

extern "C" int64_t vaw_colsum_workspace_floats(int64_t M, int64_t N) { return ((M + 127) / 128) * N; }

extern "C" int vaw_reduce_rows(const float* partial, int64_t R, int64_t N, float* out, float beta, vaw_stream stream) {
    VAW_CHECK_ARG(R > 0 && N > 0 && partial && out, "reduce_rows: bad arguments");
    colsum_final_kernel<<<ceil_div(N, 32), 1024, 0, (hipStream_t)stream>>>(partial, R, N, out, beta);
    VAW_CHECK_LAUNCH("reduce_rows");
    return VAW_OK;
}

extern "C" int vaw_colsum(vaw_dtype dt, const void* X, int64_t M, int64_t N, int64_t ldx, float* out, float beta,
                          float* workspace, int64_t workspace_floats, vaw_stream stream) {
    VAW_CHECK_ARG(M > 0 && N > 0 && ldx >= N, "colsum: bad sizes");
    ROW_PLAN(VAW_ROW_COLSUM, dt, M, 1, N, ldx, (int64_t)(uintptr_t)X, workspace_floats);
    const int64_t RB = plan.nc;
    VAW_CHECK_ARG(workspace && workspace_floats >= plan.workspace_floats, "colsum: workspace too small (%ld < %ld floats)",
                  (long)workspace_floats, (long)plan.workspace_floats);
    hipStream_t s = (hipStream_t)stream;
    dim3 grid(plan.grid_x, (int)RB);
    if (plan.variant == VAW_RV_COLSUM_BF16X8) {
        colsum_partial_bf16x8_kernel<<<grid, plan.block, 0, s>>>((const bf16_t*)X, M, N, ldx, workspace);
    } else if (plan.variant == VAW_RV_COLSUM_VEC4) {
        if (dt == VAW_F32) colsum_partial_kernel<float><<<grid, plan.block, 0, s>>>((const float*)X, M, N, ldx, workspace);
        else colsum_partial_kernel<bf16_t><<<grid, plan.block, 0, s>>>((const bf16_t*)X, M, N, ldx, workspace);
    } else {
        if (dt == VAW_F32) colsum_partial_scalar_kernel<float><<<grid, plan.block, 0, s>>>((const float*)X, M, N, ldx, workspace);
        else colsum_partial_scalar_kernel<bf16_t><<<grid, plan.block, 0, s>>>((const bf16_t*)X, M, N, ldx, workspace);
    }
    colsum_final_kernel<<<ceil_div(N, 32), 1024, 0, s>>>(workspace, RB, N, out, beta);
    VAW_CHECK_LAUNCH("colsum");
    return VAW_OK;
}
```

### variance-aware-weight_amd/dit.py

```python
import os

import numpy as np
import torch
import torch.nn as nn

from . import _lib as L
from . import ops
from ._lib import BF16, F32, ptr
from .flat import FlatModule

__all__ = ["DiT", "DiT_S", "DiT_B", "DiT_L", "DiT_XL", "DiT_models"]


def _sincos_1d(dim, pos):
    omega = 1.0 / 10000 ** (np.arange(dim // 2, dtype=np.float64) / (dim / 2.0))
    ang = np.einsum("m,d->md", pos.reshape(-1), omega)
    return np.concatenate([np.sin(ang), np.cos(ang)], axis=1)


def get_2d_sincos_pos_embed(dim, grid_size):
    gh = np.arange(grid_size, dtype=np.float32)
    gw = np.arange(grid_size, dtype=np.float32)
    grid = np.stack(np.meshgrid(gw, gh), axis=0).reshape([2, 1, grid_size, grid_size])
    return np.concatenate([_sincos_1d(dim // 2, grid[0]), _sincos_1d(dim // 2, grid[1])], axis=1)
# ... 47 lines not shown
    def __init__(self, dim, heads, mlp_ratio):
        super().__init__()
        self.norm1 = nn.LayerNorm(dim, elementwise_affine=False, eps=1e-6)
        self.attn = _Attention(dim, heads)
        self.norm2 = nn.LayerNorm(dim, elementwise_affine=False, eps=1e-6)
        self.mlp = _Mlp(dim, int(dim * mlp_ratio))
        self.adaLN_modulation = nn.Sequential(nn.SiLU(), nn.Linear(dim, 6 * dim, bias=True))


class _FinalLayer(_Holder):
    def __init__(self, dim, patch, out_ch):
        super().__init__()
        self.norm_final = nn.LayerNorm(dim, elementwise_affine=False, eps=1e-6)
        self.linear = nn.Linear(dim, patch * patch * out_ch, bias=True)
        self.adaLN_modulation = nn.Sequential(nn.SiLU(), nn.Linear(dim, 2 * dim, bias=True))


class _Workspace:

    def __init__(self, m, B, adt):
        dev = m._flat.device
        f32, T, D, Lyr = torch.float32, m.T, m.D, m.depth
        M = B * T
        e = lambda *s, dtype=adt: torch.empty(*s, device=dev, dtype=dtype)
        self.B, self.adt, self.gen = B, adt, 0
        self.Bk = Bk = ((B + 63) // 64) * 64 if adt == torch.bfloat16 else B
        z = lambda cols: torch.zeros(Bk, cols, device=dev, dtype=adt)
        self.tfreq, self.h1, self.h1s = z(256), e(B, D, dtype=f32), z(D)
        self.temb, self.c, self.cs = e(B, D, dtype=f32), e(B, D, dtype=f32), z(D)
        self.mod = e(B, m.mod_cols, dtype=f32)
        self.xp = e(M, m.Kp)
        self.xres = [e(M, D, dtype=f32) for _ in range(2 * Lyr + 1)]
        self.blk = [dict(xm=e(M, D), qkv=e(M, 3 * D), ao=e(M, D), lse=e(B * m.num_heads * T, dtype=f32), y1=e(M, D),
                         xm2=e(M, D), hpre=e(M, m.Dm), a=e(M, m.Dm), y2=e(M, D),
                         mean1=e(M, dtype=f32), rstd1=e(M, dtype=f32), mean2=e(M, dtype=f32), rstd2=e(M, dtype=f32))
                    for _ in range(Lyr)]
        self.xf, self.meanf, self.rstdf = e(M, D), e(M, dtype=f32), e(M, dtype=f32)
        self.otok = e(M, m.No, dtype=f32)
        self.dotok, self.dres, self.dD = e(M, m.No), e(M, D, dtype=f32), e(M, D)
        self.dDm, self.dqkv, self.dao = e(M, m.Dm), e(M, 3 * D), e(M, D)
        self.fp8 = bool(m._fp8)
        self.defer = (bool(m.defer_wgrad) or self.fp8) and adt == torch.bfloat16 and M % 64 == 0
        if self.fp8:
            gf = L.BF8 if m.fp8_grad_format == "e5m2" else L.FP8
            fmts = [L.FP8] * 4 + [gf] * 4
            self.fp8_states = ops.fp8_states(fmts * Lyr, dev, m.fp8_margin)
            self.calib_fwd = self.calib_bwd = False
            self.d_fwd = self.d_bwd = False
            for l, b in enumerate(self.blk):
                F = lambda i, cols: ops.Fp8(M, cols, dev, transposed=True, plain=False, fmt=fmts[i], state=self.fp8_states[8 * l + i])
                b.update(f_xm=F(0, D), f_ao=F(1, D), f_xm2=F(2, D), f_a=F(3, m.Dm), f_dy2=F(4, D), f_dhid=F(5, m.Dm), f_dy1=F(6, D),
                         f_dqkv=F(7, 3 * D))
        elif self.defer:
            for b in self.blk:
                b.update(dy2=e(M, D), dDm=e(M, m.Dm), dy1=e(M, D), dqkv=e(M, 3 * D))
        self.wgrad_groups = {}
        self.bias_groups = {}
        for b in self.blk:
            b.update(cp_fc2=ops.ColsumPartial(B, D, dev), cp_proj=ops.ColsumPartial(B, D, dev),
                     cp_fc1=ops.ColsumPartial((M + 63) // 64, m.Dm, dev), cp_qkv=ops.ColsumPartial(max(B, M // 64), 3 * D, dev))
            b["cp_fc2"].rows.value = b["cp_proj"].rows.value = B
        self.dyb = e(M, D)
        self.delta = e(B * m.num_heads * T, dtype=f32)
        self.dmod, self.dmod_a = e(B, m.mod_cols, dtype=f32), z(m.mod_cols)
        self.dcs, self.dc, self.dc_a = e(B, D, dtype=f32), e(B, D, dtype=f32), z(D)
        self.dh1s, self.dh1, self.dh1_a = e(B, D, dtype=f32), e(B, D, dtype=f32), z(D)
        self.dxp = e(M, m.Kp, dtype=f32)


class _DiTFn(torch.autograd.Function):
    @staticmethod
    def forward(ctx, anchor, model, x, t, y):
        out = model._forward_impl(x, t, y)
        ctx.model, ctx.gen, ctx.need_dx = model, model._ws_cur.gen, x.requires_grad
        ctx.x_shape = x.shape
        return out

    @staticmethod
    def backward(ctx, dout):
        m = ctx.model
        if m._ws_cur.gen != ctx.gen:
            raise L.VawError("DiT backward: activations were overwritten by a later forward of the same batch size")
        dx = m._backward_impl(dout.contiguous(), ctx.need_dx)
        return torch.zeros_like(m._anchor), None, dx, None, None


class DiT(FlatModule):
    def __init__(self, image_size=32, patch_size=2, in_channels=4, hidden_size=1152, depth=28, num_heads=16,
                 mlp_ratio=4.0, class_dropout_prob=0.1, num_classes=1000, learn_sigma=False, learn_align=False,
                 encoder_depth=8, z_dims=768, projector_dim=2048, compute_dtype="bf16"):
        super().__init__()
        if learn_align:
            raise NotImplementedError("learn_align (REPA feature alignment) is outside the hot path (SURVEY §2.1 row 12)")
        assert hidden_size % num_heads == 0 and hidden_size % 4 == 0
        self.learn_sigma, self.learn_align = learn_sigma, learn_align
        self.in_channels = in_channels
        self.out_channels = in_channels * 2 if learn_sigma else in_channels
        self.patch_size, self.num_heads, self.depth = patch_size, num_heads, depth
        self.image_size = image_size
        self.encoder_depth = encoder_depth
        self.x_embedder = _PatchEmbed(image_size, patch_size, in_channels, hidden_size)
        self.t_embedder = _TimestepEmbedder(hidden_size)
        self.y_embedder = _LabelEmbedder(num_classes, hidden_size, class_dropout_prob)
        self.pos_embed = nn.Parameter(torch.zeros(1, self.x_embedder.num_patches, hidden_size), requires_grad=False)
        self.blocks = nn.ModuleList([_Block(hidden_size, num_heads, mlp_ratio) for _ in range(depth)])
        self.projectors = None
        self.final_layer = _FinalLayer(hidden_size, patch_size, self.out_channels)
        self.initialize_weights()
        self.D, self.T = hidden_size, self.x_embedder.num_patches
        self.Dm = int(hidden_size * mlp_ratio)
        self.Kp = in_channels * patch_size * patch_size
        self.No = patch_size * patch_size * self.out_channels
        self.mod_cols = (6 * depth + 2) * hidden_size
        self.fp8_grad_format = "e5m2"
        self.fp8_scaling, self.fp8_margin = "delayed", 2.0
        self.fp8_fuse_epilogue = os.environ.get("VAW_FP8_FUSE", "1") != "0"
        self.fp8_fuse_rows = os.environ.get("VAW_FP8_FUSE_ROWS", "1") != "0"
        self._fp8_w, self._fp8_epoch, self._fp8_wstates, self._fp8_wgroup = {}, None, None, None
        self.set_compute_dtype(compute_dtype)
        self._anchor = torch.zeros(1, requires_grad=True)
        self._ws, self._ws_cur = {}, None
        self.grad_ready_hook = None
        self.defer_wgrad = True

    def initialize_weights(self):
        def basic(mod):
            if isinstance(mod, nn.Linear):
                nn.init.xavier_uniform_(mod.weight)
                if mod.bias is not None:
                    nn.init.constant_(mod.bias, 0)
        self.apply(basic)
        pe = get_2d_sincos_pos_embed(self.pos_embed.shape[-1], int(self.x_embedder.num_patches ** 0.5))
        self.pos_embed.data.copy_(torch.from_numpy(pe).float().unsqueeze(0))
        w = self.x_embedder.proj.weight.data
        nn.init.xavier_uniform_(w.view([w.shape[0], -1]))
        nn.init.constant_(self.x_embedder.proj.bias, 0)
        nn.init.normal_(self.y_embedder.embedding_table.weight, std=0.02)
        nn.init.normal_(self.t_embedder.mlp[0].weight, std=0.02)
        nn.init.normal_(self.t_embedder.mlp[2].weight, std=0.02)
        for blk in self.blocks:
            nn.init.constant_(blk.adaLN_modulation[-1].weight, 0)
            nn.init.constant_(blk.adaLN_modulation[-1].bias, 0)
        nn.init.constant_(self.final_layer.adaLN_modulation[-1].weight, 0)
        nn.init.constant_(self.final_layer.adaLN_modulation[-1].bias, 0)
        nn.init.constant_(self.final_layer.linear.weight, 0)
        nn.init.constant_(self.final_layer.linear.bias, 0)

    def set_compute_dtype(self, name):
        name = {"float32": "fp32", "f32": "fp32", "bfloat16": "bf16", "float8": "fp8"}.get(name, name)
        if name not in ("bf16", "fp32", "fp8"):
            raise ValueError(f"compute_dtype must be 'bf16', 'fp32' or 'fp8', got {name}")
        if name == "fp8" and (self.D % 128 or self.Dm % 128):
            raise ValueError("compute_dtype='fp8' needs hidden and MLP widths that are multiples of 128 (one fp8 MFMA K tile)")
        if name != getattr(self, "compute_dtype", name):
            self.require_fresh_masters("set_compute_dtype()")
        self.compute_dtype = name
        self._dt = F32 if name == "fp32" else BF16
        self._fp8 = name == "fp8"
        self._fp8_w, self._fp8_epoch, self._fp8_wstates, self._fp8_wgroup = {}, None, None, None
        self._ws = {}

    def _flat_groups(self):
        ada_w = [f"blocks.{i}.adaLN_modulation.1.weight" for i in range(self.depth)] + ["final_layer.adaLN_modulation.1.weight"]
        ada_b = [f"blocks.{i}.adaLN_modulation.1.bias" for i in range(self.depth)] + ["final_layer.adaLN_modulation.1.bias"]
        return [ada_w, ada_b]

    def _apply(self, fn, recurse=True):
# ... 56 lines not shown

    def _p32(self, name):
        o, _ = self._flat_offsets[name]
        return self._flat.data_ptr() + 4 * o

    def _prepare(self, B):
        self.ensure_flat()
        if self._dt == BF16:
            sh = self.shadow_bf16()
            self._wbase, self._wsize = sh.data_ptr(), 2
        else:
            self._wbase, self._wsize = self._flat.data_ptr(), 4
        adt = L.TORCH_DTYPE[self._dt]
        if self._fp8:
            if (B * self.T) % 128:
                raise L.VawError("compute_dtype='fp8': batch * tokens must be a multiple of 128 (K tile of the weight gradients)")
            self._refresh_fp8_weights()
        key = (B, adt, self._fp8)
        if key not in self._ws:
            self._ws[key] = _Workspace(self, B, adt)
        self._ws_cur = ws = self._ws[key]
        if ws.fp8:
            delayed = self.fp8_scaling == "delayed"
            ws.d_fwd, ws.d_bwd = delayed and ws.calib_fwd, delayed and ws.calib_bwd
            if ws.d_fwd or ws.d_bwd:
                ops.fp8_scale_update(ws.fp8_states)
        return ws

    _FP8_LINEARS = (("attn.qkv.", 3, 1), ("attn.proj.", 1, 1), ("mlp.fc1.", 0, 1), ("mlp.fc2.", 1, 0))

    def _refresh_fp8_weights(self):
        epoch = (self._weights_epoch, self._flat.data_ptr())
        if self._fp8_epoch == epoch:
            return
        self.require_fresh_masters("re-quantising the fp8 weights")
        dev = self._flat.device
        if self._fp8_wstates is None or self._fp8_wstates.device != dev:
            self._fp8_wstates, self._fp8_w, self._fp8_wgroup = ops.fp8_states([L.FP8] * (4 * self.depth), dev, self.fp8_margin), {}, None
        delayed = self.fp8_scaling == "delayed" and bool(self._fp8_w)
        if delayed:
            ops.fp8_scale_update(self._fp8_wstates)
            grp = getattr(self, "_fp8_wgroup", None)
            if grp is None or grp[0] != self._flat.data_ptr():
                pairs = [(self._p32(f"blocks.{l}.{nm}weight"), self._fp8_w[f"blocks.{l}.{nm}weight"])
                         for l in range(self.depth) for nm, _, _ in self._FP8_LINEARS]
                grp = self._fp8_wgroup = (self._flat.data_ptr(), ops.Fp8QuantGroup(pairs, dev))
            grp[1].launch()
            self._fp8_epoch = epoch
            return
        i = 0
        for l in range(self.depth):
            for nm, nf, kf in self._FP8_LINEARS:
                name = f"blocks.{l}.{nm}weight"
                N, K = (nf * self.D or self.Dm), (kf * self.D or self.Dm)
                f = self._fp8_w.get(name)
                if f is None:
                    f = self._fp8_w[name] = ops.Fp8(N, K, dev, state=self._fp8_wstates[i])
                f.quantize(self._p32(name), src_dt=F32, delayed=False)
                i += 1
        self._fp8_epoch = epoch

    def _forward_impl(self, x, t, y):
        B, C, H, W = x.shape
        assert C == self.in_channels and H == W == self.image_size, f"expected [N,{self.in_channels},{self.image_size},{self.image_size}], got {tuple(x.shape)}"
        assert t.shape == (B,) and y.shape == (B,) and y.dtype == torch.int64
        ws = self._prepare(B)
        ws.gen += 1
        dt, D, T, Dm, Lyr, ld = self._dt, self.D, self.T, self.Dm, self.depth, self.mod_cols
        M, lib, st = B * T, L.lib(), L.stream_ptr()
        x = x.float().contiguous()
        tf = t.float().contiguous()
        ye = self.y_embedder
        if (self.training and ye.dropout_prob > 0):
            drop = torch.rand(B, device=y.device) < ye.dropout_prob
            y = torch.where(drop, ye.num_classes, y)
        ws.y = y.contiguous()
        self._need(0)
        L.check(lib.vaw_timestep_embedding(dt, ptr(tf), ptr(ws.tfreq), B, 256, 10000.0, st), "timestep_embedding")
        ops.gemm(dt, 1, 1, B, D, 256, ptr(ws.tfreq), 256, self._w("t_embedder.mlp.0.weight"), 256, ptr(ws.h1), D,
                 bias=self._p32("t_embedder.mlp.0.bias"), out_f32=True)
        L.check(lib.vaw_silu_fwd(dt, ptr(ws.h1), ptr(ws.h1s), B * D, st), "silu")
        ops.gemm(dt, 1, 1, B, D, D, ptr(ws.h1s), D, self._w("t_embedder.mlp.2.weight"), D, ptr(ws.temb), D,
                 bias=self._p32("t_embedder.mlp.2.bias"), out_f32=True)
        L.check(lib.vaw_add_embedding(ptr(ws.temb), self._p32("y_embedder.embedding_table.weight"), ptr(ws.y), ptr(ws.c),
                                      B, D, ye.embedding_table.num_embeddings, st), "add_embedding")
        L.check(lib.vaw_silu_fwd(dt, ptr(ws.c), ptr(ws.cs), B * D, st), "silu")
        self._need("ada_hi")
        ops.gemm(dt, 1, 1, B, ld, D, ptr(ws.cs), D, self._w("blocks.0.adaLN_modulation.1.weight"), D, ptr(ws.mod), ld,
                 bias=self._p32("blocks.0.adaLN_modulation.1.bias"), out_f32=True)
        L.check(lib.vaw_patchify(dt, ptr(x), ptr(ws.xp), B, C, H, W, self.patch_size, st), "patchify")
        ops.gemm(dt, 1, 1, M, D, self.Kp, ptr(ws.xp), self.Kp, self._w("x_embedder.proj.weight"), self.Kp, ptr(ws.xres[0]), D,
                 bias=self._p32("x_embedder.proj.bias"), rowadd=self._p32("pos_embed"), rows_per_batch=T, out_f32=True)
        mod = ptr(ws.mod)
        for l in range(Lyr):
            b, pre = ws.blk[l], f"blocks.{l}."
            mo = mod + 4 * (6 * l * D)
            xin, xmid, xout = ptr(ws.xres[2 * l]), ptr(ws.xres[2 * l + 1]), ptr(ws.xres[2 * l + 2])
            self._need(l + 1)
            fuse_rows = ws.fp8 and ws.d_fwd and self.fp8_fuse_epilogue and self.fp8_fuse_rows and M % 64 == 0 and D % 128 == 0
            if fuse_rows:
                ops.ln_modulate_fwd_fp8(xin, mo, mo + 4 * D, ld, b["f_xm"], ptr(b["mean1"]), ptr(b["rstd1"]), B, T, D)
            else:
                ops.ln_modulate_fwd(dt, xin, mo, mo + 4 * D, ld, ptr(b["xm"]), ptr(b["mean1"]), ptr(b["rstd1"]), B, T, D)
            self._linear_fwd(ws, b, "f_xm", None if fuse_rows else b["xm"], pre + "attn.qkv.", M, 3 * D, D, ptr(b["qkv"]), 3 * D)
            q = ptr(b["qkv"])
            es = self._wsize
            ops.attn_fwd(dt, self._attn_desc(B), q, q + es * D, q + 2 * es * D, ptr(b["ao"]), ptr(b["lse"]))
            self._linear_fwd(ws, b, "f_ao", b["ao"], pre + "attn.proj.", M, D, D, xmid, D, aux_out=ptr(b["y1"]), gate=mo + 4 * 2 * D,
                             gate_ld=ld, resid=xin, rows_per_batch=T, out_f32=True)
            if fuse_rows:
                ops.ln_modulate_fwd_fp8(xmid, mo + 4 * 3 * D, mo + 4 * 4 * D, ld, b["f_xm2"], ptr(b["mean2"]), ptr(b["rstd2"]), B, T, D)
            else:
                ops.ln_modulate_fwd(dt, xmid, mo + 4 * 3 * D, mo + 4 * 4 * D, ld, ptr(b["xm2"]), ptr(b["mean2"]), ptr(b["rstd2"]), B, T, D)
            fuse_a = ws.fp8 and ws.d_fwd and self.fp8_fuse_epilogue and M % 64 == 0
            self._linear_fwd(ws, b, "f_xm2", None if fuse_rows else b["xm2"], pre + "mlp.fc1.", M, Dm, D, b["f_a"].epilogue_target() if fuse_a else ptr(b["a"]), Dm,
                             act=1, aux_out=ptr(b["hpre"]), **({"out_fp8": b["f_a"]} if fuse_a else {}))
            self._linear_fwd(ws, b, "f_a", None if fuse_a else b["a"], pre + "mlp.fc2.", M, D, Dm, xout, D, aux_out=ptr(b["y2"]),
                             gate=mo + 4 * 5 * D, gate_ld=ld, resid=xmid, rows_per_batch=T, out_f32=True)
        mo = mod + 4 * (6 * Lyr * D)
        self._need(Lyr + 1)
        ops.ln_modulate_fwd(dt, ptr(ws.xres[2 * Lyr]), mo, mo + 4 * D, ld, ptr(ws.xf), ptr(ws.meanf), ptr(ws.rstdf), B, T, D)
        ops.gemm(dt, 1, 1, M, self.No, D, ptr(ws.xf), D, self._w("final_layer.linear.weight"), D, ptr(ws.otok), self.No,
                 bias=self._p32("final_layer.linear.bias"), out_f32=True)
        out = torch.empty(B, self.out_channels, H, W, device=x.device, dtype=torch.float32)
        L.check(lib.vaw_unpatchify(dt, ptr(ws.otok), ptr(out), B, self.out_channels, H, W, self.patch_size, st), "unpatchify")
        if ws.fp8:
            ws.calib_fwd = True
        return out

    def _linear_fwd(self, ws, b, fkey, x, name, M, N, K, out, ldc, **epi):
        if not ws.fp8:
            ops.gemm(self._dt, 1, 1, M, N, K, ptr(x), K, self._w(name + "weight"), K, out, ldc, bias=self._p32(name + "bias"), **epi)
            return
        f = b[fkey].quantize(x, delayed=ws.d_fwd) if x is not None else b[fkey].transpose_from_q()
        w = self._fp8_w[name + "weight"]
        ops.gemm_fp8(M, N, K, f.last_q, K, ptr(f.scale), ptr(w.q), K, ptr(w.scale), out, ldc, bias=self._p32(name + "bias"), **epi)

    def _linear_dgrad(self, ws, b, fkey, dy, name, M, N, K, out, **epi):
        if not ws.fp8:
            ops.gemm(self._dt, 1, 0, M, K, N, ptr(dy) if isinstance(dy, torch.Tensor) else dy, N, self._w(name + "weight"), K, out, K, **epi)
            return
        f = b[fkey].quantize(dy, src_dt=BF16, delayed=ws.d_bwd) if dy is not None else b[fkey].transpose_from_q()
        w = self._fp8_w[name + "weight"]
        ops.gemm_fp8(M, K, N, f.last_q, N, ptr(f.scale), ptr(w.qt), N, ptr(w.scale), out, K, a_format=f.fmt, **epi)

    def _attn_desc(self, B):
        d = getattr(self, "_adesc", None)
        if d is None or d.B != B:
            d = self._adesc = ops.attn_desc_token_major(B, self.num_heads, self.T, self.D // self.num_heads)
        return d

    def _wgrad(self, dt, name, dy, x, Nw, Kw, M, beta, bias=True):
        ops.gemm(dt, 0, 0, Nw, Kw, M, dy, Nw, x, Kw, self._g(name + "weight"), Kw, beta=beta, out_f32=True,
                 rowsum_a_out=self._g(name + "bias") if bias else None, rowsum_a_beta=beta)

    def _adaln_wgrad(self, dt, ws, r0, nrows, B, beta):
        D, ld = self.D, self.mod_cols
        if dt == BF16:
            ops.cast_bf16(ws.dmod, ws.dmod_a)
            dmod_a, es = ptr(ws.dmod_a), 2
        else:
            dmod_a, es = ptr(ws.dmod), 4
        ops.gemm(dt, 0, 0, nrows, D, ws.Bk, dmod_a + es * r0, ld, ptr(ws.cs), D, self._g("blocks.0.adaLN_modulation.1.weight") + 4 * r0 * D,
                 D, beta=beta, out_f32=True)
        ops.colsum(dt, dmod_a + es * r0, B, nrows, ld, self._g("blocks.0.adaLN_modulation.1.bias") + 4 * r0, beta)
        return dmod_a

    def _backward_impl(self, dout, need_dx):
        ws = self._ws_cur
        B = ws.B
        dt, D, T, Dm, Lyr, ld = self._dt, self.D, self.T, self.Dm, self.depth, self.mod_cols
        M, lib, st = B * T, L.lib(), L.stream_ptr()
        H = W = self.image_size
        beta = 1.0 if self.grads_live() else 0.0
        self._gbase = self.flat_grads().data_ptr()
        hook = self.grad_ready_hook
        ada_half = self._ada_split_block() if hook else None
        dres, dD, dDm, dmod = ptr(ws.dres), ptr(ws.dD), ptr(ws.dDm), ptr(ws.dmod)
        mod = ptr(ws.mod)
        es = self._wsize
        defer = ws.defer and dt == BF16
        fp8 = ws.fp8
        own_dy = defer and not fp8
        fuse_rows = fp8 and ws.d_bwd and self.fp8_fuse_epilogue and self.fp8_fuse_rows and M % 64 == 0 and D % 128 == 0

        def ln_bwd_and_gate(dout_p, x_p, mean_p, rstd_p, scale_p, dres_in, dsh, dsc, nxt):
            if nxt is None:
                ops.ln_modulate_bwd(dt, dout_p, x_p, mean_p, rstd_p, scale_p, ld, dres_in, dres, dsh, dsc, ld, B, T, D)
                return
            l2, which = nxt
            nb = ws.blk[l2]
            mo2, dmo2 = mod + 4 * (6 * l2 * D), dmod + 4 * (6 * l2 * D)
            gcol = 5 if which == "mlp" else 2
            y, cp = (nb["y2"], nb["cp_fc2"]) if which == "mlp" else (nb["y1"], nb["cp_proj"])
            if fuse_rows:
                ops.ln_modulate_bwd_gate_fp8(dout_p, x_p, mean_p, rstd_p, scale_p, ld, dres_in, dres, dsh, dsc, ld, ptr(y),
                                             mo2 + 4 * gcol * D, nb["f_dy2" if which == "mlp" else "f_dy1"], dmo2 + 4 * gcol * D,
                                             B, T, D, cp.buf.data_ptr())
            else:
                dy = ptr(nb["dy2" if which == "mlp" else "dy1"]) if own_dy else ptr(ws.dyb)
                ops.ln_modulate_bwd_gate(dt, dout_p, x_p, mean_p, rstd_p, scale_p, ld, dres_in, dres, dsh, dsc, ld, ptr(y),
                                         mo2 + 4 * gcol * D, dy, dmo2 + 4 * gcol * D, B, T, D, cp.buf.data_ptr())

        L.check(lib.vaw_unpatchify_bwd(dt, ptr(dout), ptr(ws.dotok), B, self.out_channels, H, W, self.patch_size, st), "unpatchify_bwd")
        self._wgrad(dt, "final_layer.linear.", ptr(ws.dotok), ptr(ws.xf), self.No, D, M, beta)
        ops.gemm(dt, 1, 0, M, D, self.No, ptr(ws.dotok), self.No, self._w("final_layer.linear.weight"), D, dD, D)
        mo, dmo = mod + 4 * (6 * Lyr * D), dmod + 4 * (6 * Lyr * D)
        ln_bwd_and_gate(dD, ptr(ws.xres[2 * Lyr]), ptr(ws.meanf), ptr(ws.rstdf), mo + 4 * D, 0, dmo, dmo + 4 * D,
                        (Lyr - 1, "mlp") if Lyr else None)
        if hook:
            hook(Lyr + 1)
        pending = []
        group_cut = Lyr // 2 if (hook and Lyr >= 4) else 0

        def fold_bias(blocks, qkv_too):
            key = (blocks[0], blocks[-1], self._gbase, qkv_too)
            cps = []
            for l in blocks:
                b, pre = ws.blk[l], f"blocks.{l}."
                names = [("cp_fc2", "mlp.fc2."), ("cp_fc1", "mlp.fc1."), ("cp_proj", "attn.proj.")] + ([("cp_qkv", "attn.qkv.")] if qkv_too else [])
                cps += [(b[key_cp], pre + nm) for key_cp, nm in names]
            rows = tuple(int(cp.rows.value) for cp, _ in cps)
            ent = ws.bias_groups.get(key)
            if ent is None or ent[1] != rows:
                jobs = [(cp.buf.data_ptr(), self._g(nm + "bias"), r, cp.N) for (cp, nm), r in zip(cps, rows)]
                ent = ws.bias_groups[key] = (ops.ReduceGroup(jobs, dout.device), rows)
            grp = ent[0]
            grp.launch(beta)

        def flush():
            if not pending:
                return
            key = (pending[0], pending[-1], self._gbase)
            grp = ws.wgrad_groups.get(key)
            if grp is None:
                probs = []
                for l in pending:
                    b, pre = ws.blk[l], f"blocks.{l}."
                    if fp8:
                        for name, fdy, fx, Nw, Kw in ((pre + "mlp.fc2.", b["f_dy2"], b["f_a"], D, Dm), (pre + "mlp.fc1.", b["f_dhid"], b["f_xm2"], Dm, D),
                                                      (pre + "attn.proj.", b["f_dy1"], b["f_ao"], D, D), (pre + "attn.qkv.", b["f_dqkv"], b["f_xm"], 3 * D, D)):
                            probs.append((ptr(fdy.qt), ptr(fx.qt), self._g(name + "weight"), Nw, Kw, M, M, Kw, 0.0, 0, ptr(fdy.scale), ptr(fx.scale)))
                        continue
                    for name, dy, x, Nw, Kw in ((pre + "mlp.fc2.", b["dy2"], b["a"], D, Dm), (pre + "mlp.fc1.", b["dDm"], b["xm2"], Dm, D),
                                                (pre + "attn.proj.", b["dy1"], b["ao"], D, D), (pre + "attn.qkv.", b["dqkv"], b["xm"], 3 * D, D)):
                        probs.append((ptr(dy), ptr(x), self._g(name + "weight"), Nw, Kw, Nw, Kw, Kw))
                grp = ws.wgrad_groups[key] = ops.WgradGroup(probs, M, dout.device)
            grp.launch((L.BF8 if self.fp8_grad_format == "e5m2" else L.FP8) if fp8 else dt, beta)
            fold_bias(list(pending), True)
            if hook:
                for l in pending:
                    hook(l + 1)
            pending.clear()

        for l in reversed(range(Lyr)):
            b, pre = ws.blk[l], f"blocks.{l}."
            mo, dmo = mod + 4 * (6 * l * D), dmod + 4 * (6 * l * D)
            xin, xmid = ptr(ws.xres[2 * l]), ptr(ws.xres[2 * l + 1])
            dy2, dhid, dy1, dq = ((ptr(b["dy2"]), ptr(b["dDm"]), ptr(b["dy1"]), ptr(b["dqkv"])) if own_dy
                                  else (ptr(ws.dyb), dDm, ptr(ws.dyb), ptr(ws.dqkv)))
            if not defer:
                self._wgrad(dt, pre + "mlp.fc2.", dy2, ptr(b["a"]), D, Dm, M, beta, bias=False)
            fuse_dh = fp8 and ws.d_bwd and self.fp8_fuse_epilogue and M % 64 == 0
            self._linear_dgrad(ws, b, "f_dy2", None if fuse_rows else dy2, pre + "mlp.fc2.", M, D, Dm, b["f_dhid"].epilogue_target() if fuse_dh else dhid, act=2,
                               aux_in=ptr(b["hpre"]), colsum_partial=b["cp_fc1"], **({"out_fp8": b["f_dhid"]} if fuse_dh else {}))
            if not defer:
                self._wgrad(dt, pre + "mlp.fc1.", dhid, ptr(b["xm2"]), Dm, D, M, beta, bias=False)
            self._linear_dgrad(ws, b, "f_dhid", None if (fp8 and fuse_dh) else dhid, pre + "mlp.fc1.", M, Dm, D, dD)
            ln_bwd_and_gate(dD, xmid, ptr(b["mean2"]), ptr(b["rstd2"]), mo + 4 * 4 * D, dres, dmo + 4 * 3 * D, dmo + 4 * 4 * D, (l, "attn"))
            if not defer:
                self._wgrad(dt, pre + "attn.proj.", dy1, ptr(b["ao"]), D, D, M, beta, bias=False)
            self._linear_dgrad(ws, b, "f_dy1", None if fuse_rows else dy1, pre + "attn.proj.", M, D, D, ptr(ws.dao))
            q = ptr(b["qkv"])
            qkv_bias_folded = False
            if defer:
                qkv_bias_folded = ops.attn_bwd_colsum(dt, self._attn_desc(B), q, q + es * D, q + 2 * es * D, ptr(b["ao"]), ptr(ws.dao),
                                                      ptr(b["lse"]), ptr(ws.delta), dq, dq + es * D, dq + 2 * es * D, b["cp_qkv"])
            if not qkv_bias_folded:
                ops.attn_bwd(dt, self._attn_desc(B), q, q + es * D, q + 2 * es * D, ptr(b["ao"]), ptr(ws.dao), ptr(b["lse"]),
                             ptr(ws.delta), dq, dq + es * D, dq + 2 * es * D)
                if defer:
                    ops.colsum(dt, dq, M, 3 * D, 3 * D, b["cp_qkv"].buf.data_ptr(), 0.0, device=dout.device)
                    b["cp_qkv"].rows.value = 1
                else:
                    self._wgrad(dt, pre + "attn.qkv.", dq, ptr(b["xm"]), 3 * D, D, M, beta)
            self._linear_dgrad(ws, b, "f_dqkv", dq, pre + "attn.qkv.", M, 3 * D, D, dD)
            ln_bwd_and_gate(dD, xin, ptr(b["mean1"]), ptr(b["rstd1"]), mo + 4 * D, dres, dmo, dmo + 4 * D, (l - 1, "mlp") if l else None)
            if defer:
                pending.append(l)
                if l == group_cut:
                    pending.reverse()
                    flush()
            else:
                fold_bias([l], False)
            if hook:
                if not defer:
                    hook(l + 1)
                if l == ada_half:
                    r0 = 6 * l * D
                    self._adaln_wgrad(dt, ws, r0, ld - r0, B, beta)
                    hook("ada_hi")
        pending.reverse()
        flush()
        if dt == BF16:
            ops.cast_bf16(ws.dres, ws.dD)
            dx0 = dD
        else:
            dx0 = dres
        self._wgrad(dt, "x_embedder.proj.", dx0, ptr(ws.xp), D, self.Kp, M, beta)
        dx = None
        if need_dx:
            ops.gemm(dt, 1, 0, M, self.Kp, D, dx0, D, self._w("x_embedder.proj.weight"), self.Kp, ptr(ws.dxp), self.Kp, out_f32=True)
            dx = torch.empty(B, self.in_channels, H, W, device=dout.device, dtype=torch.float32)
            L.check(lib.vaw_patchify_bwd(ptr(ws.dxp), ptr(dx), B, self.in_channels, H, W, self.patch_size, st), "patchify_bwd")
        rows = ld if ada_half is None else 6 * ada_half * D
        dmod_a = self._adaln_wgrad(dt, ws, 0, rows, B, beta)
        ops.gemm(dt, 1, 0, B, D, ld, dmod_a, ld, self._w("blocks.0.adaLN_modulation.1.weight"), D, ptr(ws.dcs), D, out_f32=True)
        L.check(lib.vaw_silu_bwd(ptr(ws.c), ptr(ws.dcs), ptr(ws.dc), B * D, st), "silu_bwd")
        ye = self.y_embedder.embedding_table
        L.check(lib.vaw_embedding_bwd(ptr(ws.dc), ptr(ws.y), self._g("y_embedder.embedding_table.weight"), B, D,
                                      ye.num_embeddings, beta, st), "embedding_bwd")
        if dt == BF16:
            ops.cast_bf16(ws.dc, ws.dc_a)
            dc_a = ptr(ws.dc_a)
        else:
            dc_a = ptr(ws.dc)
        self._wgrad(dt, "t_embedder.mlp.2.", dc_a, ptr(ws.h1s), D, D, ws.Bk, beta)
        ops.gemm(dt, 1, 0, B, D, D, dc_a, D, self._w("t_embedder.mlp.2.weight"), D, ptr(ws.dh1s), D, out_f32=True)
        L.check(lib.vaw_silu_bwd(ptr(ws.h1), ptr(ws.dh1s), ptr(ws.dh1), B * D, st), "silu_bwd")
        if dt == BF16:
            ops.cast_bf16(ws.dh1, ws.dh1_a)
            dh1_a = ptr(ws.dh1_a)
        else:
            dh1_a = ptr(ws.dh1)
        self._wgrad(dt, "t_embedder.mlp.0.", dh1_a, ptr(ws.tfreq), D, 256, ws.Bk, beta)
        self.attach_grads()
        if fp8:
            ws.calib_bwd = True
        if hook:
            hook(0)
        return dx


_PRESETS = {"DiT-S": (384, 12, 6), "DiT-B": (768, 12, 12), "DiT-L": (1024, 24, 16), "DiT-XL": (1152, 28, 16)}


def _make(name):
    hidden, depth, heads = _PRESETS[name]

    def build(image_size, patch_size, in_channels, class_dropout_prob, num_classes, learn_sigma, **kwargs):
        return DiT(image_size=image_size, patch_size=patch_size, in_channels=in_channels, hidden_size=hidden,
                   depth=depth, num_heads=heads, class_dropout_prob=class_dropout_prob, num_classes=num_classes,
                   learn_sigma=learn_sigma, **kwargs)
    build.__name__ = name.replace("-", "_")
    return build


DiT_S, DiT_B, DiT_L, DiT_XL = (_make(n) for n in ("DiT-S", "DiT-B", "DiT-L", "DiT-XL"))
DiT_models = {"DiT-S": DiT_S, "DiT-B": DiT_B, "DiT-L": DiT_L, "DiT-XL": DiT_XL}
```

### variance-aware-weight_amd/gaussian_diffusion.py

```python
import enum
import math

import numpy as np
import torch

from . import ops


class ModelMeanType(enum.Enum):
    PREVIOUS_X = enum.auto()
    START_X = enum.auto()
    EPSILON = enum.auto()
    VELOCITY = enum.auto()
    VECTOR = enum.auto()
    SCORE = enum.auto()


class ModelVarType(enum.Enum):
    LEARNED = enum.auto()
    FIXED_SMALL = enum.auto()
    FIXED_LARGE = enum.auto()
    LEARNED_RANGE = enum.auto()


# ... 277 lines not shown
        return self._loop(self.ddim_sample, model, shape, noise, device, progress, clip_denoised=clip_denoised,
                          denoised_fn=denoised_fn, cond_fn=cond_fn, model_kwargs=model_kwargs, eta=eta)

    def ddim_sample_loop(self, model, shape, noise=None, clip_denoised=True, denoised_fn=None, cond_fn=None, model_kwargs=None,
                         device=None, progress=False, eta=0.0):
        final = None
        for final in self.ddim_sample_loop_progressive(model, shape, noise, clip_denoised, denoised_fn, cond_fn, model_kwargs,
                                                       device, progress, eta):
            pass
        return final["sample"]

    def _vb_terms_bpd(self, mean_out, var_out, x_start, x_t, t, scale=1.0):
        mt, vt = self.model_mean_type, self.model_var_type
        if mt == ModelMeanType.VELOCITY:
            raise RuntimeError("VELOCITY with a variational-bound term: the reference's _predict_xstart_from_v fails to broadcast")
        if mt not in (ModelMeanType.EPSILON, ModelMeanType.START_X, ModelMeanType.PREVIOUS_X):
            raise NotImplementedError(mt)
        var_mode = {ModelVarType.LEARNED: 1, ModelVarType.LEARNED_RANGE: 2}.get(vt, 0)
        coef = self._tables(x_start.device)["vb"][t]
        return ops.vb_terms(mean_out, var_out, x_start, x_t, coef, 1 if mt == ModelMeanType.PREVIOUS_X else 0, var_mode, scale)

    def _scale_timesteps(self, t):
        if self.rescale_timesteps:
            return t.float() * (1000.0 / self.num_timesteps)
        return t

    def q_sample(self, x_start, t, noise=None):
        if noise is None:
            noise = torch.randn_like(x_start)
        assert noise.shape == x_start.shape
        tb = self._tables(x_start.device)
        return ops.qsample(x_start.contiguous(), noise.contiguous(), t, tb["a"], tb["s"])

    def sample_t(self, x_start):
        if self.args.time_dist[0] == "uniform":
            return torch.randint(0, self.num_timesteps, (x_start.shape[0],), device=x_start.device)
        raise NotImplementedError(f"Unknown time_dist: {self.args.time_dist}")

    def compute_target(self, x_start, noise, t, alpha=None, sigma=None):
        tb = self._tables(x_start.device)
        if self.model_mean_type == ModelMeanType.START_X:
            return x_start
        if self.model_mean_type == ModelMeanType.EPSILON:
            return noise
        return ops.mix_rows(x_start.contiguous(), noise.contiguous(), tb["ca"][t], tb["cb"][t])

    def training_losses(self, model, x_start, features=None, t=None, model_kwargs=None, noise=None):
        if model_kwargs is None:
            model_kwargs = {}
        if noise is None:
            noise = torch.randn_like(x_start)
        if t is None:
            t = self.sample_t(x_start)
        kl_loss = self.loss_type in (LossType.KL, LossType.RESCALED_KL)
        if not kl_loss and self.loss_type not in (LossType.MSE, LossType.RESCALED_MSE):
            raise NotImplementedError(self.loss_type)
        if getattr(self.args, "learn_align", False):
            raise NotImplementedError("learn_align: feature-alignment teachers are out of scope (SURVEY.md §2.1 row 12)")
        x_start = x_start.contiguous()
        noise = noise.contiguous()
        tb = self._tables(x_start.device)
        x_t = ops.qsample(x_start, noise, t, tb["a"], tb["s"])
        raw_output = model(x_t, self._scale_timesteps(t), **model_kwargs)
        model_output = raw_output[0] if isinstance(raw_output, tuple) else raw_output
        learned = self.model_var_type in (ModelVarType.LEARNED, ModelVarType.LEARNED_RANGE)
        var_values = None
        if learned:
            B, C = x_t.shape[:2]
            assert model_output.shape == (B, C * 2, *x_t.shape[2:])
            model_output, var_values = torch.split(model_output, C, dim=1)
        if kl_loss:
            scale = float(self.num_timesteps) if self.loss_type == LossType.RESCALED_KL else 1.0
            return {"loss": self._vb_terms_bpd(model_output, var_values, x_start, x_t, t, scale)}
        terms = {}
        if learned:
            scale = self.num_timesteps / 1000.0 if self.loss_type == LossType.RESCALED_MSE else 1.0
            terms["vb"] = self._vb_terms_bpd(model_output.detach(), var_values, x_start, x_t, t, scale)
        assert model_output.shape == x_start.shape
        terms["mse"] = ops.weighted_mse(model_output, x_start, noise, tb["ca"][t], tb["cb"][t], tb["w"][t])
        terms["loss"] = terms["mse"] + terms["vb"] if "vb" in terms else terms["mse"]
        return terms


class FlowMatching:

    def __init__(self, *, args, model_mean_type, device="cuda"):
        self.args = args
        self.model_mean_type = model_mean_type
        self.mse_loss_weight_type = args.weight_type
        self.path_type = args.path_type
        self.sampler_type = getattr(args, "sampler_type", "ode")
        self.p2_gamma = args.p2_gamma
        self.p2_k = args.p2_k
        self.gamma = args.gamma
        self.learn_sigma = args.learn_sigma

    def expand_t_like_x(self, t, x):
        if t.dim() == 0:
            t = t.expand(x.shape[0])
        return t.view(t.size(0), *([1] * (len(x.size()) - 1))).to(x)

    def interpolant(self, t):
        if self.path_type == "linear":
            return 1 - t, t, torch.full_like(t, -1.0), torch.full_like(t, 1.0)
        if self.path_type == "cosine":
            return (torch.cos(t * np.pi / 2), torch.sin(t * np.pi / 2), -np.pi / 2 * torch.sin(t * np.pi / 2),
                    np.pi / 2 * torch.cos(t * np.pi / 2))
        if self.path_type == "linear_logsnr":
            lam = 10 + t * (-10.0 - 10)
            alpha_t, sigma_t = torch.sigmoid(0.5 * lam), torch.sigmoid(-0.5 * lam)
            d_alpha_t = -10.0 * alpha_t * sigma_t
            return alpha_t, sigma_t, d_alpha_t, -d_alpha_t
        raise NotImplementedError()

    def sample_t(self, x_start):
        td = self.args.time_dist
        if td[0] == "uniform":
            return torch.rand(x_start.shape[0], device=x_start.device)
        if td[0] == "lognorm":
            mu, sigma = float(td[-2]), float(td[-1])
            return torch.sigmoid(torch.randn(x_start.shape[0], device=x_start.device) * sigma + mu)
        raise NotImplementedError(f"Unknown time_dist: {td}")

    def q_sample(self, x_start, noise, t):
        alpha_t, sigma_t, _, _ = self.interpolant(t.float())
        return ops.mix_rows(x_start.contiguous(), noise.contiguous(), alpha_t.contiguous(), sigma_t.contiguous())

    def _target_coefs(self, alpha_t, sigma_t, d_alpha_t, d_sigma_t):
        mt = self.model_mean_type
        one, zero = torch.ones_like(alpha_t), torch.zeros_like(alpha_t)
        if mt == ModelMeanType.START_X:
            return one, zero
        if mt == ModelMeanType.EPSILON:
            return zero, one
        if mt == ModelMeanType.VELOCITY:
            return -sigma_t, alpha_t
        if mt == ModelMeanType.VECTOR:
            return d_alpha_t, d_sigma_t
        if mt == ModelMeanType.SCORE:
            return zero, -1.0 / sigma_t
        raise KeyError(mt)

    def compute_target(self, x_start, noise, t, alpha_t=None, sigma_t=None, d_alpha_t=None, d_sigma_t=None):
        if alpha_t is None or sigma_t is None or d_alpha_t is None or d_sigma_t is None:
            alpha_t, sigma_t, d_alpha_t, d_sigma_t = self.interpolant(t)
        ca, cb = self._target_coefs(alpha_t, sigma_t, d_alpha_t, d_sigma_t)
        return ops.mix_rows(x_start.contiguous(), noise.contiguous(), ca.float().contiguous(), cb.float().contiguous())

    def training_losses(self, model, x_start, features=None, t=None, model_kwargs=None, noise=None):
        if model_kwargs is None:
            model_kwargs = {}
        if noise is None:
            noise = torch.randn_like(x_start)
        if t is None:
            t = self.sample_t(x_start)
        if getattr(self.args, "learn_align", False):
            raise NotImplementedError("learn_align: feature-alignment teachers are out of scope (SURVEY.md §2.1 row 12)")
        x_start, noise = x_start.contiguous(), noise.contiguous()
        alpha_t, sigma_t, d_alpha_t, d_sigma_t = self.interpolant(t)
        x_t = ops.mix_rows(x_start, noise, alpha_t.contiguous(), sigma_t.contiguous())
        ca, cb = self._target_coefs(alpha_t, sigma_t.clone(), d_alpha_t, d_sigma_t)
        w = compute_mse_loss_weight(self.model_mean_type, self.mse_loss_weight_type, t, alpha_t, sigma_t, self.p2_k,
                                    self.p2_gamma)
        raw_output = model(x_t, t, **model_kwargs)
        model_output = raw_output[0] if isinstance(raw_output, tuple) else raw_output
        assert model_output.shape == x_start.shape
# ... 5 lines not shown
```

### variance-aware-weight_amd/ops.py

```python
import ctypes as C

import torch

from . import _lib as L
from ._lib import BF16, F32, AttnDesc, Epilogue, check, need_cuda, ptr, stream_ptr


def dt_of(t):
    if t.dtype == torch.float32:
        return F32
    if t.dtype == torch.bfloat16:
        return BF16
    raise L.VawError(f"unsupported activation dtype {t.dtype}")


def _f32c(*ts):
    for t in ts:
        if t is not None and (t.dtype != torch.float32 or not t.is_contiguous()):
            raise L.VawError(f"expected a contiguous float32 tensor, got {t.dtype} contiguous={t.is_contiguous()}")


def qsample(x0, noise, t, tab_a, tab_s):
    need_cuda(x0, noise, t, tab_a, tab_s)
    _f32c(x0, noise, tab_a, tab_s)
    assert noise.shape == x0.shape and t.dtype == torch.int64 and t.shape == (x0.shape[0],)
    out = torch.empty_like(x0)
    B = x0.shape[0]
    check(L.lib().vaw_qsample_fwd(ptr(x0), ptr(noise), ptr(t), ptr(tab_a), ptr(tab_s), tab_a.numel(), ptr(out), B,
                                  x0.numel() // B, stream_ptr()), "vaw_qsample_fwd")
    return out


def mix_rows(x, y, ca, cb):
    need_cuda(x, y, ca, cb)
    _f32c(x, y, ca, cb)
    assert x.shape == y.shape and ca.shape == cb.shape == (x.shape[0],)
    out = torch.empty_like(x)
    B = x.shape[0]
    check(L.lib().vaw_mix_rows(ptr(x), ptr(y), ptr(ca), ptr(cb), ptr(out), B, x.numel() // B, stream_ptr()), "vaw_mix_rows")
    return out


class _WeightedMSE(torch.autograd.Function):
    @staticmethod
    def forward(ctx, model_out, x0, noise, ca, cb, w):
        need_cuda(model_out, x0, noise, ca, cb, w)
        model_out = model_out.contiguous()
        _f32c(model_out, x0, noise, ca, cb, w)
        B = x0.shape[0]
        assert model_out.shape == x0.shape == noise.shape and ca.shape == cb.shape == w.shape == (B,)
        mse = torch.empty(B, device=x0.device, dtype=torch.float32)
        check(L.lib().vaw_wmse_fwd(ptr(model_out), ptr(x0), ptr(noise), ptr(ca), ptr(cb), ptr(w), ptr(mse), B,
                                   x0.numel() // B, stream_ptr()), "vaw_wmse_fwd")
        ctx.save_for_backward(model_out, x0, noise, ca, cb, w)
        return mse

    @staticmethod
    def backward(ctx, gmse):
        model_out, x0, noise, ca, cb, w = ctx.saved_tensors
        gmse = gmse.contiguous().float()
        dout = torch.empty_like(model_out)
        B = x0.shape[0]
        check(L.lib().vaw_wmse_bwd(ptr(model_out), ptr(x0), ptr(noise), ptr(ca), ptr(cb), ptr(w), ptr(gmse), ptr(dout),
                                   B, x0.numel() // B, stream_ptr()), "vaw_wmse_bwd")
        return dout, None, None, None, None, None


def weighted_mse(model_out, x0, noise, ca, cb, w):
    return _WeightedMSE.apply(model_out, x0, noise, ca, cb, w)


class _VbTerms(torch.autograd.Function):

    @staticmethod
    def forward(ctx, mean_out, var_out, x0, x_t, coef, mean_mode, var_mode, scale):
        need_cuda(mean_out, x0, x_t, coef)
        _f32c(mean_out, x0, x_t, coef)
        B = x0.shape[0]
        assert mean_out.shape == x0.shape == x_t.shape and coef.shape == (B, 8)
        if var_out is not None:
            need_cuda(var_out)
            _f32c(var_out)
            assert var_out.shape == x0.shape
        vb = torch.empty(B, device=x0.device, dtype=torch.float32)
        check(L.lib().vaw_vb_fwd(ptr(mean_out), ptr(var_out) if var_out is not None else None, ptr(x0), ptr(x_t), ptr(coef),
                                 mean_mode, var_mode, scale, ptr(vb), B, x0.numel() // B, stream_ptr()), "vaw_vb_fwd")
        ctx.save_for_backward(mean_out, var_out, x0, x_t, coef)
        ctx.modes = (mean_mode, var_mode, scale)
        return vb

    @staticmethod
    def backward(ctx, gvb):
        mean_out, var_out, x0, x_t, coef = ctx.saved_tensors
        mean_mode, var_mode, scale = ctx.modes
        gvb = gvb.contiguous().float()
        d_mean = torch.empty_like(mean_out) if ctx.needs_input_grad[0] else None
        d_var = torch.empty_like(var_out) if (var_out is not None and ctx.needs_input_grad[1]) else None
        B = x0.shape[0]
        if d_mean is not None or d_var is not None:
            check(L.lib().vaw_vb_bwd(ptr(mean_out), ptr(var_out) if var_out is not None else None, ptr(x0), ptr(x_t), ptr(coef),
                                     mean_mode, var_mode, scale, ptr(gvb), ptr(d_mean) if d_mean is not None else None,
                                     ptr(d_var) if d_var is not None else None, B, x0.numel() // B, stream_ptr()), "vaw_vb_bwd")
        return d_mean, d_var, None, None, None, None, None, None


def vb_terms(mean_out, var_out, x0, x_t, coef, mean_mode, var_mode, scale=1.0):
    return _VbTerms.apply(mean_out.contiguous(), None if var_out is None else var_out.contiguous(), x0, x_t, coef,
                          int(mean_mode), int(var_mode), float(scale))


def sample_step(kind, mean_out, var_out, x, noise, coef, mean_mode, var_mode, clip_denoised, eta=0.0, want_all=False):
    need_cuda(mean_out, x, coef)
    mean_out, x = mean_out.contiguous().float(), x.contiguous().float()
    var_out = None if var_out is None else var_out.contiguous().float()
    noise = None if noise is None else noise.contiguous().float()
    coef = coef.contiguous()
    B = x.shape[0]
    assert mean_out.shape == x.shape and coef.shape == (B, 16) and coef.dtype == torch.float32
    res = {"pred_xstart": torch.empty_like(x)}
    if kind:
        res["sample"] = torch.empty_like(x)
    if want_all:
        res["mean"], res["log_variance"] = torch.empty_like(x), torch.empty_like(x)
# ... 213 lines not shown
fallbacks = {}


class GemmTrace:

    def __init__(self):
        self.rows = []

    def events(self):
        return torch.cuda.Event(enable_timing=True), torch.cuda.Event(enable_timing=True)

    def add(self, mfma, ak, bk, M, N, K, e0, e1, nbytes=0.0, tag="gemm"):
        self.rows.append((mfma, ak, bk, 2.0 * M * N * K, e0, e1, nbytes, (tag, int(M), int(N), int(K))))

    def add_flop(self, mfma, ak, bk, flop, e0, e1, nbytes=0.0):
        self.rows.append((mfma, ak, bk, flop, e0, e1, nbytes, None))

    @staticmethod
    def _name(mfma, ak, bk):
        return ("fp8_mfma" if mfma == 2 else "bf16_mfma" if mfma else "generic_f32mfma") + ("/fwd" if ak and bk else "/dgrad" if ak else "/wgrad")

    def by_shape(self):
        acc = {}
        for mfma, ak, bk, flop, e0, e1, nbytes, shape in self.rows:
            d = acc.setdefault((self._name(mfma, ak, bk), shape), [0, 0.0, 0.0])
            d[0] += 1
            d[1] += e0.elapsed_time(e1)
            d[2] += flop
        return sorted(((k[0], k[1], v[0], v[1], v[2]) for k, v in acc.items()), key=lambda r: -r[3])

    def summarize(self):
        out = {}
        for mfma, ak, bk, flop, e0, e1, nbytes, _shape in self.rows:
            name = self._name(mfma, ak, bk)
            d = out.setdefault(name, {"launches": 0, "flop": 0.0, "ms": 0.0, "bytes": 0.0})
            d["launches"] += 1
            d["flop"] += flop
            d["bytes"] += nbytes
            d["ms"] += e0.elapsed_time(e1)
        return out


gemm_trace = None


def gemm_t(A, B, *, a_kmajor=True, b_kmajor=True, out_dtype=None, bias=None, act=0, aux_in=None, want_aux=False,
           gate=None, resid=None, rowadd=None, rows_per_batch=0, alpha=1.0, beta=0.0, out=None, colsum_out=None,
           colsum_beta=0.0, rowsum_a_out=None, rowsum_a_beta=0.0):
    need_cuda(A, B)
    assert A.dim() == 2 and B.dim() == 2 and A.is_contiguous() and B.is_contiguous() and A.dtype == B.dtype
    dt = dt_of(A)
    M, K = (A.shape if a_kmajor else A.shape[::-1])
    N, Kb = (B.shape if b_kmajor else B.shape[::-1])
    assert K == Kb, (A.shape, B.shape, a_kmajor, b_kmajor)
    out_dtype = out_dtype or A.dtype
    if out is None:
        out = torch.empty(M, N, device=A.device, dtype=out_dtype)
    aux = torch.empty(M, N, device=A.device, dtype=A.dtype) if want_aux else None
    _f32c(bias, gate, resid, rowadd)
    gemm(dt, a_kmajor, b_kmajor, M, N, K, ptr(A), A.shape[1], ptr(B), B.shape[1], ptr(out), N, bias=ptr(bias), act=act,
         aux_in=ptr(aux_in), aux_out=ptr(aux), gate=ptr(gate), gate_ld=(gate.shape[-1] if gate is not None else 0),
         resid=ptr(resid), rowadd=ptr(rowadd), rows_per_batch=rows_per_batch, alpha=alpha, beta=beta,
         out_f32=(out.dtype == torch.float32), colsum_out=ptr(colsum_out), colsum_beta=colsum_beta,
         rowsum_a_out=ptr(rowsum_a_out), rowsum_a_beta=rowsum_a_beta)
    return (out, aux) if want_aux else out


_scratch = {}


def scratch_f32(device, n):
    t = _scratch.get(device)
    if t is None or t.numel() < n:
        t = _scratch[device] = torch.empty(max(n, 1 << 26), device=device, dtype=torch.float32)
    return t


def colsum(dt, X, M, N, ldx, out, beta=0.0, device=None):
    need = L.lib().vaw_colsum_workspace_floats(M, N)
    ws = scratch_f32(device or torch.device("cuda", torch.cuda.current_device()), need)
    check(L.lib().vaw_colsum(dt, X, M, N, ldx, out, beta, ptr(ws), ws.numel(), stream_ptr()), "vaw_colsum")


def ln_modulate_fwd(dt, x, shift, scale, mod_ld, out, mean, rstd, B, T, D, eps=1e-6):
    check(L.lib().vaw_ln_modulate_fwd(dt, x, shift, scale, mod_ld, out, mean, rstd, B, T, D, eps, stream_ptr()),
          "vaw_ln_modulate_fwd")


def ln_modulate_fwd_fp8(x, shift, scale, mod_ld, f8, mean, rstd, B, T, D, eps=1e-6, pool=2):
    q = f8.epilogue_target(pool)
    check(L.lib().vaw_ln_modulate_fwd_fp8(x, shift, scale, mod_ld, q, f8.state.data_ptr(), f8.fmt, mean, rstd, B, T, D, eps, stream_ptr()),
          "vaw_ln_modulate_fwd_fp8")


def gate_bwd_fp8(dres, y, gate, mod_ld, f8, dgate, dmod_ld, B, T, D, dy_colpart=0, pool=2):
    ws = _row_ws(B, T, D)
    q = f8.epilogue_target(pool)
    check(L.lib().vaw_gate_bwd_fp8(dres, y, gate, mod_ld, q, f8.state.data_ptr(), f8.fmt, dgate, dmod_ld, dy_colpart or None, B, T, D,
                                   ws.data_ptr(), ws.numel(), stream_ptr()), "vaw_gate_bwd_fp8")


def row_plan(kind, dt, B, T, D, workspace_floats=0, ldx=0, base_addr=0):
    p = L.RowLaunch()
    check(L.lib().vaw_row_plan(kind, dt, B, T, D, ldx, base_addr, workspace_floats, C.byref(p)), "vaw_row_plan")
    return p


def _row_ws(B, T, D):
    return scratch_f32(torch.device("cuda", torch.cuda.current_device()), L.lib().vaw_row_bwd_workspace_floats(B, T, D))


def ln_modulate_bwd(dt, dout, x, mean, rstd, scale, mod_ld, dres_in, dx, dshift, dscale, dmod_ld, B, T, D):
    ws = _row_ws(B, T, D)
    check(L.lib().vaw_ln_modulate_bwd(dt, dout, x, mean, rstd, scale, mod_ld, dres_in or None, dx, dshift, dscale,
                                      dmod_ld, B, T, D, ws.data_ptr(), ws.numel(), stream_ptr()), "vaw_ln_modulate_bwd")


def ln_modulate_bwd_gate(dt, dout, x, mean, rstd, scale, mod_ld, dres_in, dx, dshift, dscale, dmod_ld, y_next, gate_next, dy_next,
                         dgate_next, B, T, D, dy_colpart=0):
    if D > 1280:
        ln_modulate_bwd(dt, dout, x, mean, rstd, scale, mod_ld, dres_in, dx, dshift, dscale, dmod_ld, B, T, D)
        gate_bwd(dt, dx, y_next, gate_next, mod_ld, dy_next, dgate_next, dmod_ld, B, T, D, dy_colpart)
        return
    ws = _row_ws(B, T, D)
    check(L.lib().vaw_ln_modulate_bwd_gate(dt, dout, x, mean, rstd, scale, mod_ld, dres_in or None, dx, dshift, dscale, dmod_ld,
                                           y_next, gate_next, dy_next, dgate_next, dy_colpart or None, B, T, D, ws.data_ptr(),
                                           ws.numel(), stream_ptr()), "vaw_ln_modulate_bwd_gate")


def ln_modulate_bwd_gate_fp8(dout, x, mean, rstd, scale, mod_ld, dres_in, dx, dshift, dscale, dmod_ld, y_next, gate_next, f8,
                             dgate_next, B, T, D, dy_colpart=0, pool=2):
    if D > 1280:
        ln_modulate_bwd(BF16, dout, x, mean, rstd, scale, mod_ld, dres_in, dx, dshift, dscale, dmod_ld, B, T, D)
        gate_bwd_fp8(dx, y_next, gate_next, mod_ld, f8, dgate_next, dmod_ld, B, T, D, dy_colpart, pool)
        return
    ws = _row_ws(B, T, D)
    q = f8.epilogue_target(pool)
    check(L.lib().vaw_ln_modulate_bwd_gate_fp8(dout, x, mean, rstd, scale, mod_ld, dres_in or None, dx, dshift, dscale, dmod_ld,
                                               y_next, gate_next, q, f8.state.data_ptr(), f8.fmt, dgate_next, dy_colpart or None,
                                               B, T, D, ws.data_ptr(), ws.numel(), stream_ptr()), "vaw_ln_modulate_bwd_gate_fp8")


class ColsumPartial:

    def __init__(self, max_rows, N, device):
        self.buf = torch.empty(max_rows, N, device=device, dtype=torch.float32)
        self.N = int(N)
        self.rows = C.c_int64(0)


class ReduceJob(C.Structure):
    _fields_ = [("partial", C.c_void_p), ("out", C.c_void_p), ("R", C.c_int64), ("N", C.c_int64)]


class ReduceGroup:

    def __init__(self, jobs, device):
        self.n = len(jobs)
        self.table = (ReduceJob * self.n)(*[ReduceJob(*j) for j in jobs])
        self.desc = torch.empty(L.lib().vaw_reduce_rows_batched_desc_bytes(self.n), device=device, dtype=torch.uint8)
        self.uploaded = False

    def launch(self, beta):
        check(L.lib().vaw_reduce_rows_batched(self.n, C.cast(self.table, C.c_void_p), float(beta), self.desc.data_ptr(),
                                              0 if self.uploaded else 1, stream_ptr()), "vaw_reduce_rows_batched")
        self.uploaded = True


def gate_bwd(dt, dres, y, gate, mod_ld, dy, dgate, dmod_ld, B, T, D, dy_colpart=0):
    ws = _row_ws(B, T, D)
    check(L.lib().vaw_gate_bwd(dt, dres, y, gate, mod_ld, dy, dgate, dmod_ld, dy_colpart or None, B, T, D, ws.data_ptr(),
                               ws.numel(), stream_ptr()), "vaw_gate_bwd")


def reduce_rows(partial, R, N, out, beta):
    check(L.lib().vaw_reduce_rows(partial, R, N, out, beta, stream_ptr()), "vaw_reduce_rows")


def attn_desc_token_major(B, H, T, hd):
    return AttnDesc(B, H, T, hd, T * 3 * H * hd, hd, 3 * H * hd, 1, T * H * hd, hd, H * hd, 1, hd ** -0.5)


def attn_desc_channel_major(B, H, T, ch):
    return AttnDesc(B, H, T, ch, 3 * H * ch * T, ch * T, 1, T, H * ch * T, ch * T, 1, T, ch ** -0.5)


def attn_desc_nhwc(B, H, T, ch, new_order):
    C_ = H * ch
    desc = AttnDesc(B, H, T, ch, T * 3 * C_, ch if new_order else 3 * ch, 3 * C_, 1, T * C_, ch, C_, 1, ch ** -0.5)
    return (desc, C_, 2 * C_) if new_order else (desc, ch, 2 * ch)


def attn_plan(direction, dt, desc, q, k, v, o_or_do, dq=0, dk=0, dv=0):
    p = L.AttnLaunch()
    check(L.lib().vaw_attn_plan(direction, dt, C.byref(desc), q, k, v, o_or_do, dq, dk, dv, C.byref(p)), "vaw_attn_plan")
    return p
# ... 58 lines not shown
```

### variance-aware-weight_amd/trainer.py

```python
from contextlib import nullcontext

import torch
import torch.nn as nn

from . import dist_util, ops
from .flat import FlatModule
from .optim import FusedAdamW


def ema(source, target, decay):
    s, t = getattr(source, "module", source), getattr(target, "module", target)
    with torch.no_grad():
        if isinstance(s, FlatModule) and isinstance(t, FlatModule):
            s.ensure_flat(); t.ensure_flat()
            if s._flat_offsets == t._flat_offsets and s._flat.is_cuda and not list(s.buffers()):
                ops.ema_update(t._flat, s._flat, decay)
                t.mark_weights_changed()
                return
        src, dst = source.state_dict(), target.state_dict()
        for k in src:
            dst[k].data.copy_(dst[k].data * decay + src[k].data * (1 - decay))
        if isinstance(t, FlatModule) and getattr(t, "_flat", None) is not None:
            t.mark_weights_changed()


def sample_from_latent(latent, latent_scale=1.0, cpu_rng=False):
    mean, std = torch.chunk(latent, 2, dim=1)
    eps = torch.randn(mean.shape).to(mean.device) if cpu_rng else torch.randn_like(mean)
    return (mean + std * eps) * latent_scale


class Trainer:
    def __init__(self, args, device, model, ema_model, optimizer, scheduler, diffusion, train_loader, pbar=None):
        if getattr(args, "learn_align", False):
            raise NotImplementedError("learn_align needs network-fetched teacher encoders: out of scope (SURVEY.md §2.1 row 12)")
        self.args, self.device = args, device
        self.model, self.ema_model = model, ema_model
        self.optimizer, self.scheduler, self.diffusion = optimizer, scheduler, diffusion
        self.train_loader = train_loader
        self.datalooper = iter(train_loader)
        self.pbar = pbar
        self.scaler = None
        inner = getattr(model, "module", model)
        if hasattr(inner, "set_compute_dtype"):
            low = getattr(args, "amp_dtype", None) or (inner.compute_dtype if inner.compute_dtype in ("bf16", "fp8") else "bf16")
            want = low if args.amp else "fp32"
            if inner.compute_dtype != want:
                inner.set_compute_dtype(want)
        if hasattr(inner, "host_dropout_rng"):
            inner.host_dropout_rng = bool(getattr(args, "cpu_rng", False))
        self._fused = isinstance(optimizer, FusedAdamW)
        self._zero = self._fused and getattr(optimizer, "zero", None) is not None
        if getattr(inner, "_zero", None) is not None and not self._zero:
            raise ValueError("the model was wrapped with shard_optimizer=True: it needs a vaw_amd.FusedAdamW built after the wrap "
                             f"(got {type(optimizer).__name__}{' built before the wrap' if self._fused else ''})")
        if self._zero:
            if getattr(args, "ema_decay", None) is not None:
                optimizer.attach_ema_sharded(args.ema_decay, ema_model)
        elif self._fused and ema_model is not None and dist_util.is_main_process():
            optimizer.attach_ema(ema_model, args.ema_decay)
        self.last_mse = None
        self._cpu_rng = bool(getattr(args, "cpu_rng", False))
        self.schedule_sampler = None
        name = getattr(args, "schedule_sampler", None)
        if name and name != "uniform":
            from .resample import create_named_schedule_sampler
            self.schedule_sampler = create_named_schedule_sampler(name, diffusion)
            if getattr(args, "hip_graph", False):
                raise ValueError("args.schedule_sampler updates its history on the host every step: not with args.hip_graph")
        self._graph, self._graph_calls, self._gin, self._gout = None, 0, None, None
        hg = getattr(args, "hip_graph", False)
        self._graph_auto = hg == "auto"
        self._use_graph = bool(hg)
        if self._use_graph:
            why = ("needs vaw_amd.FusedAdamW" if not self._fused else "not with DDP (args.parallel)" if args.parallel else
                   "not with grad_accumulation > 1" if max(1, args.grad_accumulation) > 1 else
                   "not with args.cpu_rng" if self._cpu_rng else "needs a CUDA device" if torch.device(device).type != "cuda" else
                   "the model draws its label-drop mask on the host every step (UNet drop_label_prob > 0)"
                   if getattr(inner, "host_rng_in_forward", False) else None)
            if why and self._graph_auto:
                self._use_graph = False
            elif why:
                raise ValueError(f"args.hip_graph: {why}")
            else:
                optimizer.enable_device_hyper()

    def _get_next_batch(self):
        try:
            images, labels = next(self.datalooper)
        except StopIteration:
            self.datalooper = iter(self.train_loader)
            return self._get_next_batch()
        return (images.to(self.device, non_blocking=True),
                labels.to(self.device, non_blocking=True) if self.args.class_cond else None)

    def _compute_loss(self, images, labels, features):
        model_kwargs = {"y": labels} if self.args.class_cond else {}
        if self._cpu_rng:
            noise = torch.randn(images.shape).to(images.device)
            t = torch.randint(0, self.diffusion.num_timesteps, (images.shape[0],)).to(images.device)
            return self.diffusion.training_losses(self.model, images, features, t=t, model_kwargs=model_kwargs, noise=noise)
        if self.schedule_sampler is not None:
            t, w = self.schedule_sampler.sample(images.shape[0], images.device)
            terms = self.diffusion.training_losses(self.model, images, features, t=t, model_kwargs=model_kwargs)
            self.schedule_sampler.update_with_local_losses(t, terms["loss"].detach())
            terms = dict(terms)
            terms["loss"] = terms["loss"] * w
            return terms
        return self.diffusion.training_losses(self.model, images, features, model_kwargs=model_kwargs)

    def _apply_gradient_clipping(self):
        if self.args.grad_clip:
            if self._fused:
                self.optimizer.max_grad_norm = float(self.args.grad_clip)
            else:
                nn.utils.clip_grad_norm_(self.model.parameters(), self.args.grad_clip)

    def consolidate(self):
        if self._zero:
            self.optimizer.consolidate()
            if getattr(self.optimizer, "_ema_shard", None) is not None:
                self.optimizer.consolidate_ema(self.ema_model)

    def _update_ema(self):
        if self._zero:
            return
        if dist_util.is_main_process() and self.ema_model is not None:
            if self._fused and getattr(self.optimizer, "ema_done_in_step", False):
                return
            ema(self.model, self.ema_model, self.args.ema_decay)

    def _graph_body(self, images, labels):
        a = self.args
        if a.in_chans == 4:
            images = sample_from_latent(images, a.latent_scale, False)
        loss_dict = self._compute_loss(images, labels, None)
        loss = loss_dict["loss"].mean()
        loss.backward()
        self._apply_gradient_clipping()
        self.optimizer.step()
        self.optimizer.zero_grad()
        return loss.detach(), (loss_dict["mse"].detach().mean() if "mse" in loss_dict else torch.zeros_like(loss.detach()))

    def eager_from_now_on(self):
        if self._use_graph:
            self._graph, self._gin, self._gout = None, None, None
            self._graph_calls = -(1 << 60)

    def _train_step_graph(self, step):
        a = self.args
        self.model.train()
        images, labels = self._get_next_batch()
        self.optimizer.prepare_step()
        self._graph_calls += 1
        if self._graph is None and self._graph_calls <= 2:
            if self._graph_auto and self._graph_calls == 2:
                import time
                e0, e1 = torch.cuda.Event(enable_timing=True), torch.cuda.Event(enable_timing=True)
                torch.cuda.synchronize()
                t0 = time.perf_counter()
                e0.record()
                total, mse = self._graph_body(images, labels)
                e1.record()
                host_ms = 1e3 * (time.perf_counter() - t0)
                torch.cuda.synchronize()
                self.graph_decision = dict(host_ms=host_ms, gpu_ms=e0.elapsed_time(e1))
                if host_ms < 0.7 * self.graph_decision["gpu_ms"]:
                    self._graph_calls = -(1 << 60)
            else:
                total, mse = self._graph_body(images, labels)
        elif self._graph_calls < 0:
            total, mse = self._graph_body(images, labels)
        else:
            if self._graph is None:
                self._gin = (images.clone(), None if labels is None else labels.clone())
                torch.cuda.synchronize()
                g = torch.cuda.CUDAGraph()
                with torch.cuda.graph(g):
                    self._gout = self._graph_body(*self._gin)
                self._graph = g
            else:
                self._gin[0].copy_(images, non_blocking=True)
                if labels is not None:
                    self._gin[1].copy_(labels, non_blocking=True)
            self._graph.replay()
            total, mse = self._gout
        self.scheduler.step()
        if dist_util.is_main_process():
            self._update_ema()
        self.last_mse = mse
        if dist_util.is_main_process() and self.pbar is not None:
            self.pbar.update(1)
        if getattr(a, "defer_loss_sync", False):
            return total
        total_f = float(total.item())
        if dist_util.is_main_process() and self.pbar is not None:
            self.pbar.set_postfix(mse=f"{float(mse.item()):.4f}")
        return total_f

    def train_step(self, step):
        if self._use_graph:
            return self._train_step_graph(step)
        a = self.args
        self.model.train()
        if a.parallel:
            self.train_loader.sampler.set_epoch(step)
        accum = max(1, a.grad_accumulation)
        total, mse_avg = None, None
        for i in range(accum):
            images, labels = self._get_next_batch()
            if a.in_chans == 4:
                images = sample_from_latent(images, a.latent_scale, self._cpu_rng)
            if a.parallel and accum > 1 and i < accum - 1:
                ctx = self.model.no_sync()
            else:
                ctx = nullcontext()
            with ctx:
                loss_dict = self._compute_loss(images, labels, None)
                loss = loss_dict["loss"].mean() / accum
                loss.backward()
            ld = loss.detach()
            md = loss_dict["mse"].detach().mean() / accum if "mse" in loss_dict else torch.zeros_like(ld)
            total = ld if total is None else total + ld
            mse_avg = md if mse_avg is None else mse_avg + md
            if (i + 1) % accum == 0:
                self._apply_gradient_clipping()
                self.optimizer.step()
                self.optimizer.zero_grad()
        self.scheduler.step()
        if dist_util.is_main_process():
            self._update_ema()
        self.last_mse = mse_avg
        if getattr(a, "defer_loss_sync", False):
            if dist_util.is_main_process() and self.pbar is not None:
                self.pbar.update(1)
            return total
        total_f = float(total.item())
        if dist_util.is_main_process() and self.pbar is not None:
            self.pbar.update(1)
            self.pbar.set_postfix(mse=f"{float(mse_avg.item()):.4f}")
        return total_f
```

Before: 20110 images/sec.

## Fuse latent sampling, q_sample, weighted MSE and several backward casts into single kernels

Adds a fused latent_qsample kernel that draws x_start from the latent mean/std and computes x_t in one pass. Weighted-MSE forward and backward now gather coefficients from timestep tables on device, and the mean is computed by a kernel. Fused cast variants are added for silu backward, LN-modulate backward, colsum and embedding+silu. Pinned staging buffers for table uploads are pooled instead of leaking. Together these cut launch count, elementwise memory traffic and host gathers, at the cost of many new code paths enabled by default through an env flag.

```diff
diff --git a/include/vaw_hip.h b/include/vaw_hip.h
--- a/include/vaw_hip.h
+++ b/include/vaw_hip.h
@@ -25,6 +25,17 @@
                  const float* w, float* mse, int B, int64_t per_sample, vaw_stream stream);
 int vaw_wmse_bwd(const float* model_out, const float* x0, const float* noise, const float* ca, const float* cb,
                  const float* w, const float* gmse, float* dout, int B, int64_t per_sample, vaw_stream stream);
+
+int vaw_latent_qsample(const float* latent, const float* eps, const float* noise, const int64_t* t, const float* tab_a,
+                       const float* tab_s, int num_timesteps, float latent_scale, float t_mul, float* x_start, float* x_t,
+                       float* t_scaled, int B, int64_t per_sample, vaw_stream stream);
+int vaw_wmse_fwd_t(const float* model_out, const float* x0, const float* noise, const int64_t* t, const float* tab_ca,
+                   const float* tab_cb, const float* tab_w, int num_timesteps, float* mse, float* mean_out, int B,
+                   int64_t per_sample, vaw_stream stream);
+int vaw_wmse_bwd_t(const float* model_out, const float* x0, const float* noise, const int64_t* t, const float* tab_ca,
+                   const float* tab_cb, const float* tab_w, int num_timesteps, float gscale, float* dout, int B,
+                   int64_t per_sample, vaw_stream stream);
+int vaw_mean_f32(const float* v, int64_t n, float* out, vaw_stream stream);
 
 int vaw_vb_fwd(const float* mean_out, const float* var_out, const float* x0, const float* x_t, const float* coef,
                int mean_mode, int var_mode, float scale, float* vb, int B, int64_t per_sample, vaw_stream stream);
@@ -104,6 +115,7 @@
 int64_t vaw_colsum_workspace_floats(int64_t M, int64_t N);
 int vaw_colsum(vaw_dtype dt, const void* X, int64_t M, int64_t N, int64_t ldx, float* out, float beta,
                float* workspace, int64_t workspace_floats, vaw_stream stream);
+int vaw_colsum_cast(const float* X, void* Xa, int64_t M, int64_t N, int64_t ldx, float* out, float beta, vaw_stream stream);
 int vaw_reduce_rows(const float* partial, int64_t R, int64_t N, float* out, float beta, vaw_stream stream);
 typedef struct {
     const float* partial;
@@ -120,6 +132,10 @@
                         const float* scale, int64_t mod_ld, const float* dres_in, float* dx, float* dshift,
                         float* dscale, int64_t dmod_ld, int B, int T, int D, float* workspace, int64_t workspace_floats,
                         vaw_stream stream);
+int vaw_ln_modulate_bwd_lo(vaw_dtype dt, const void* dout, const float* x, const float* mean, const float* rstd,
+                           const float* scale, int64_t mod_ld, const float* dres_in, float* dx, void* dx_bf16, float* dshift,
+                           float* dscale, int64_t dmod_ld, int B, int T, int D, float* workspace, int64_t workspace_floats,
+                           vaw_stream stream);
 int vaw_ln_modulate_fwd_fp8(const float* x, const float* shift, const float* scale, int64_t mod_ld, void* q_out, float* q_state,
                             vaw_dtype q_format, float* mean, float* rstd, int B, int T, int D, float eps, vaw_stream stream);
 int vaw_gate_bwd_fp8(const float* dres, const void* y, const float* gate, int64_t mod_ld, void* dy_q, float* q_state,
@@ -169,6 +185,9 @@
                            vaw_stream stream);
 int vaw_silu_fwd(vaw_dtype dt, const float* x, void* out, int64_t n, vaw_stream stream);
 int vaw_silu_bwd(const float* x, const float* dy, float* dx, int64_t n, vaw_stream stream);
+int vaw_silu_bwd_cast(const float* x, const float* dy, float* dx, void* dx_bf16, int64_t n, vaw_stream stream);
+int vaw_add_embedding_silu(vaw_dtype dt, const float* a, const float* table, const int64_t* idx, float* c, void* cs, int B,
+                           int D, int num_rows, vaw_stream stream);
 int vaw_add_embedding(const float* a, const float* table, const int64_t* idx, float* out, int B, int D,
                       int num_rows, vaw_stream stream);
 int vaw_embedding_bwd(const float* dc, const int64_t* idx, float* dtable, int B, int D, int num_rows, float beta,
diff --git a/variance-aware-weight_amd/_lib.py b/variance-aware-weight_amd/_lib.py
--- a/variance-aware-weight_amd/_lib.py
+++ b/variance-aware-weight_amd/_lib.py
@@ -47,11 +47,17 @@
     "vaw_mix_rows": [_p, _p, _p, _p, _p, _i, _l, _p],
     "vaw_wmse_fwd": [_p, _p, _p, _p, _p, _p, _p, _i, _l, _p],
     "vaw_wmse_bwd": [_p, _p, _p, _p, _p, _p, _p, _p, _i, _l, _p],
+    "vaw_latent_qsample": [_p, _p, _p, _p, _p, _p, _i, _f, _f, _p, _p, _p, _i, _l, _p],
+    "vaw_wmse_fwd_t": [_p, _p, _p, _p, _p, _p, _p, _i, _p, _p, _i, _l, _p],
+    "vaw_wmse_bwd_t": [_p, _p, _p, _p, _p, _p, _p, _i, _f, _p, _i, _l, _p],
+    "vaw_mean_f32": [_p, _l, _p, _p],
     "vaw_gemm": [_i, _i, _i, _l, _l, _l, _p, _l, _p, _l, _p, _l, C.POINTER(Epilogue), _p, _l, _p],
     "vaw_gemm_uses_bf16_mfma": [_i, _l, _l, _l, _p, _l, _p, _l],
     "vaw_colsum": [_i, _p, _l, _l, _l, _p, _f, _p, _l, _p],
     "vaw_ln_modulate_fwd": [_i, _p, _p, _p, _l, _p, _p, _p, _i, _i, _i, _f, _p],
     "vaw_ln_modulate_bwd": [_i, _p, _p, _p, _p, _p, _l, _p, _p, _p, _p, _l, _i, _i, _i, _p, _l, _p],
+    "vaw_ln_modulate_bwd_lo": [_i, _p, _p, _p, _p, _p, _l, _p, _p, _p, _p, _p, _l, _i, _i, _i, _p, _l, _p],
+    "vaw_colsum_cast": [_p, _p, _l, _l, _l, _p, _f, _p],
     "vaw_gate_bwd": [_i, _p, _p, _p, _l, _p, _p, _l, _p, _i, _i, _i, _p, _l, _p],
     "vaw_reduce_rows": [_p, _l, _l, _p, _f, _p],
     "vaw_reduce_rows_batched": [_i, _p, _f, _p, _i, _p],
@@ -64,6 +70,8 @@
     "vaw_timestep_embedding": [_i, _p, _p, _i, _i, _f, _p],
     "vaw_silu_fwd": [_i, _p, _p, _l, _p],
     "vaw_silu_bwd": [_p, _p, _p, _l, _p],
+    "vaw_silu_bwd_cast": [_p, _p, _p, _p, _l, _p],
+    "vaw_add_embedding_silu": [_i, _p, _p, _p, _p, _p, _i, _i, _i, _p],
     "vaw_add_embedding": [_p, _p, _p, _p, _i, _i, _i, _p],
     "vaw_embedding_bwd": [_p, _p, _p, _i, _i, _i, _f, _p],
     "vaw_attn_fwd": [_i, C.POINTER(AttnDesc), _p, _p, _p, _p, _p, _p],
diff --git a/variance-aware-weight_amd/csrc/capi.hip b/variance-aware-weight_amd/csrc/capi.hip
--- a/variance-aware-weight_amd/csrc/capi.hip
+++ b/variance-aware-weight_amd/csrc/capi.hip
@@ -33,16 +33,39 @@
 #include <mutex>
 #include <string.h>
 #include <vector>
+namespace {
+struct Staging {
+    void* pinned;
+    size_t cap;
+    hipEvent_t done;
+};
+}
 hipError_t vaw_upload_table(void* dev, const void* host, size_t bytes, hipStream_t s) {
     static std::mutex mu;
-    static std::vector<void*> keep;
-    void* pinned = nullptr;
-    hipError_t rc = hipHostMalloc(&pinned, bytes, hipHostMallocDefault);
+    static std::vector<Staging> pool;
+    hipStreamCaptureStatus cs = hipStreamCaptureStatusNone;
+    if (hipStreamIsCapturing(s, &cs) == hipSuccess && cs != hipStreamCaptureStatusNone) {
+        void* own = nullptr;
+        const hipError_t rc = hipHostMalloc(&own, bytes, hipHostMallocDefault);
+        if (rc != hipSuccess) return rc;
+        memcpy(own, host, bytes);
+        return hipMemcpyAsync(dev, own, bytes, hipMemcpyHostToDevice, s);
+    }
+    std::lock_guard<std::mutex> g(mu);
+    Staging* st = nullptr;
+    for (Staging& c : pool)
+        if (c.cap >= bytes && hipEventQuery(c.done) == hipSuccess) { st = &c; break; }
+    if (!st) {
+        Staging n{nullptr, bytes < 4096 ? (size_t)4096 : bytes, nullptr};
+        hipError_t rc = hipHostMalloc(&n.pinned, n.cap, hipHostMallocDefault);
+        if (rc != hipSuccess) return rc;
+        rc = hipEventCreateWithFlags(&n.done, hipEventDisableTiming);
+        if (rc != hipSuccess) { (void)hipHostFree(n.pinned); return rc; }
+        pool.push_back(n);
+        st = &pool.back();
+    }
+    memcpy(st->pinned, host, bytes);
+    hipError_t rc = hipMemcpyAsync(dev, st->pinned, bytes, hipMemcpyHostToDevice, s);
     if (rc != hipSuccess) return rc;
-    memcpy(pinned, host, bytes);
-    {
-        std::lock_guard<std::mutex> g(mu);
-        keep.push_back(pinned);
-    }
-    return hipMemcpyAsync(dev, pinned, bytes, hipMemcpyHostToDevice, s);
+    return hipEventRecord(st->done, s);
 }
diff --git a/variance-aware-weight_amd/csrc/elementwise.hip b/variance-aware-weight_amd/csrc/elementwise.hip
--- a/variance-aware-weight_amd/csrc/elementwise.hip
+++ b/variance-aware-weight_amd/csrc/elementwise.hip
@@ -54,12 +54,70 @@
     return VAW_OK;
 }
 
+__global__ void latent_qsample_kernel(const float* __restrict__ latent, const float* __restrict__ eps, const float* __restrict__ nz,
+                                      const int64_t* __restrict__ t, const float* __restrict__ tab_a,
+                                      const float* __restrict__ tab_s, int T, float scale, float t_mul,
+                                      float* __restrict__ x0, float* __restrict__ xt, float* __restrict__ t_scaled, int64_t n) {
+    const int b = blockIdx.y;
+    const int64_t tt = t[b];
+    const bool ok = tt >= 0 && tt < T;
+    const float a = ok ? tab_a[tt] : __builtin_nanf("");
+    const float c = ok ? tab_s[tt] : __builtin_nanf("");
+    if (t_scaled && blockIdx.x == 0 && threadIdx.x == 0) t_scaled[b] = (float)tt * t_mul;
+    const float* mr = latent + (int64_t)b * 2 * n;
+    const float* sr = mr + n;
+    const float* er = eps + (int64_t)b * n;
+    const float* nr = nz + (int64_t)b * n;
+    float* x0r = x0 + (int64_t)b * n;
+    float* xtr = xt + (int64_t)b * n;
+    const int64_t n4 = ((n & 3) == 0) ? n / 4 : 0;
+    for (int64_t i = blockIdx.x * (int64_t)blockDim.x + threadIdx.x; i < n4; i += (int64_t)gridDim.x * blockDim.x) {
+        const f32x4 xs = (load4(mr + 4 * i) + load4(sr + 4 * i) * load4(er + 4 * i)) * scale;
+        store4(x0r + 4 * i, xs);
+        store4(xtr + 4 * i, a * xs + c * load4(nr + 4 * i));
+    }
+    for (int64_t i = n4 * 4 + blockIdx.x * (int64_t)blockDim.x + threadIdx.x; i < n; i += (int64_t)gridDim.x * blockDim.x) {
+        const float xs = (mr[i] + sr[i] * er[i]) * scale;
+        x0r[i] = xs;
+        xtr[i] = a * xs + c * nr[i];
+    }
+}
+
+extern "C" int vaw_latent_qsample(const float* latent, const float* eps, const float* noise, const int64_t* t, const float* tab_a,
+                                  const float* tab_s, int num_timesteps, float latent_scale, float t_mul, float* x_start,
+                                  float* x_t, float* t_scaled, int B, int64_t per_sample, vaw_stream stream) {
+    VAW_CHECK_ARG(B > 0 && B < 65536 && per_sample > 0 && num_timesteps > 0, "latent_qsample: bad sizes B=%d n=%ld", B, (long)per_sample);
+    VAW_CHECK_ARG(latent && eps && noise && t && tab_a && tab_s && x_start && x_t, "latent_qsample: null operand");
+    VAW_CHECK_ARG((((uintptr_t)latent | (uintptr_t)eps | (uintptr_t)noise | (uintptr_t)x_start | (uintptr_t)x_t) & 15) == 0,
+                  "latent_qsample: operands must be 16-byte aligned");
+    int gx = stream_grid(per_sample / 4 + 1, 256);
+    dim3 grid(gx > 64 ? 64 : gx, B);
+    latent_qsample_kernel<<<grid, 256, 0, (hipStream_t)stream>>>(latent, eps, noise, t, tab_a, tab_s, num_timesteps, latent_scale,
+                                                                 t_mul, x_start, x_t, t_scaled, per_sample);
+    VAW_CHECK_LAUNCH("latent_qsample");
+    return VAW_OK;
+}
+
+struct WmseCoef {
+    float a, c, w;
+};
+template <bool GATHER>
+__device__ __forceinline__ WmseCoef wmse_coef(const float* __restrict__ ca, const float* __restrict__ cb, const float* __restrict__ w,
+                                              const int64_t* __restrict__ t, int T, int b) {
+    if (!GATHER) return WmseCoef{ca[b], cb[b], w[b]};
+    const int64_t tt = t[b];
+    const float nan = __builtin_nanf("");
+    return (tt >= 0 && tt < T) ? WmseCoef{ca[tt], cb[tt], w[tt]} : WmseCoef{nan, nan, nan};
+}
+
+template <bool GATHER>
 __global__ void wmse_fwd_kernel(const float* __restrict__ o, const float* __restrict__ x0, const float* __restrict__ nz,
                                 const float* __restrict__ ca, const float* __restrict__ cb, const float* __restrict__ w,
-                                float* __restrict__ mse, int64_t n) {
+                                const int64_t* __restrict__ t, int T, float* __restrict__ mse, int64_t n) {
     __shared__ float scratch[16];
     const int b = blockIdx.x;
-    const float a = ca[b], c = cb[b];
+    const WmseCoef k3 = wmse_coef<GATHER>(ca, cb, w, t, T, b);
+    const float a = k3.a, c = k3.c;
     const float* orow = o + (int64_t)b * n;
     const float* xr = x0 + (int64_t)b * n;
     const float* nr = nz + (int64_t)b * n;
@@ -74,15 +132,18 @@
         acc += d * d;
     }
     float tot = block_sum(acc, scratch);
-    if (threadIdx.x == 0) mse[b] = w[b] * (tot / (float)n);
-}
-
+    if (threadIdx.x == 0) mse[b] = k3.w * (tot / (float)n);
+}
+
+template <bool GATHER>
 __global__ void wmse_bwd_kernel(const float* __restrict__ o, const float* __restrict__ x0, const float* __restrict__ nz,
                                 const float* __restrict__ ca, const float* __restrict__ cb, const float* __restrict__ w,
-                                const float* __restrict__ gmse, float* __restrict__ dout, int64_t n) {
+                                const int64_t* __restrict__ t, int T, const float* __restrict__ gmse, float gscale,
+                                float* __restrict__ dout, int64_t n) {
     const int b = blockIdx.y;
-    const float a = ca[b], c = cb[b];
-    const float k = gmse[b] * w[b] * 2.f / (float)n;
+    const WmseCoef k3 = wmse_coef<GATHER>(ca, cb, w, t, T, b);
+    const float a = k3.a, c = k3.c;
+    const float k = (gmse ? gmse[b] : gscale) * k3.w * 2.f / (float)n;
     const float* orow = o + (int64_t)b * n;
     const float* xr = x0 + (int64_t)b * n;
     const float* nr = nz + (int64_t)b * n;
@@ -98,7 +159,7 @@
                             const float* cb, const float* w, float* mse, int B, int64_t per_sample,
                             vaw_stream stream) {
     VAW_CHECK_ARG(B > 0 && per_sample > 0, "wmse_fwd: bad sizes");
-    wmse_fwd_kernel<<<B, 1024, 0, (hipStream_t)stream>>>(model_out, x0, noise, ca, cb, w, mse, per_sample);
+    wmse_fwd_kernel<false><<<B, 1024, 0, (hipStream_t)stream>>>(model_out, x0, noise, ca, cb, w, nullptr, 0, mse, per_sample);
     VAW_CHECK_LAUNCH("wmse_fwd");
     return VAW_OK;
 }
@@ -109,8 +170,44 @@
     VAW_CHECK_ARG(B > 0 && per_sample > 0, "wmse_bwd: bad sizes");
     int gx = stream_grid(per_sample / 4 + 1, 256);
     dim3 grid(gx > 64 ? 64 : gx, B);
-    wmse_bwd_kernel<<<grid, 256, 0, (hipStream_t)stream>>>(model_out, x0, noise, ca, cb, w, gmse, dout, per_sample);
+    wmse_bwd_kernel<false><<<grid, 256, 0, (hipStream_t)stream>>>(model_out, x0, noise, ca, cb, w, nullptr, 0, gmse, 0.f, dout, per_sample);
     VAW_CHECK_LAUNCH("wmse_bwd");
+    return VAW_OK;
+}
+
+__global__ void __launch_bounds__(256) mean_final_kernel(const float* __restrict__ v, int64_t n, float* __restrict__ out) {
+    __shared__ float scratch[16];
+    float acc = 0.f;
+    for (int64_t i = threadIdx.x; i < n; i += 256) acc += v[i];
+    const float tot = block_sum(acc, scratch);
+    if (threadIdx.x == 0) out[0] = tot / (float)n;
+}
+extern "C" int vaw_mean_f32(const float* v, int64_t n, float* out, vaw_stream stream) {
+    VAW_CHECK_ARG(v && out && n > 0, "mean_f32: bad arguments");
+    mean_final_kernel<<<1, 256, 0, (hipStream_t)stream>>>(v, n, out);
+    VAW_CHECK_LAUNCH("mean_f32");
+    return VAW_OK;
+}
+
+extern "C" int vaw_wmse_fwd_t(const float* model_out, const float* x0, const float* noise, const int64_t* t, const float* tab_ca,
+                              const float* tab_cb, const float* tab_w, int num_timesteps, float* mse, float* mean_out, int B,
+                              int64_t per_sample, vaw_stream stream) {
+    VAW_CHECK_ARG(B > 0 && per_sample > 0 && num_timesteps > 0 && t && tab_ca && tab_cb && tab_w && mse, "wmse_fwd_t: bad arguments");
+    wmse_fwd_kernel<true><<<B, 1024, 0, (hipStream_t)stream>>>(model_out, x0, noise, tab_ca, tab_cb, tab_w, t, num_timesteps, mse, per_sample);
+    if (mean_out) mean_final_kernel<<<1, 256, 0, (hipStream_t)stream>>>(mse, B, mean_out);
+    VAW_CHECK_LAUNCH("wmse_fwd_t");
+    return VAW_OK;
+}
+
+extern "C" int vaw_wmse_bwd_t(const float* model_out, const float* x0, const float* noise, const int64_t* t, const float* tab_ca,
+                              const float* tab_cb, const float* tab_w, int num_timesteps, float gscale, float* dout, int B,
+                              int64_t per_sample, vaw_stream stream) {
+    VAW_CHECK_ARG(B > 0 && B < 65536 && per_sample > 0 && num_timesteps > 0 && t && tab_ca && tab_cb && tab_w && dout, "wmse_bwd_t: bad arguments");
+    int gx = stream_grid(per_sample / 4 + 1, 256);
+    dim3 grid(gx > 64 ? 64 : gx, B);
+    wmse_bwd_kernel<true><<<grid, 256, 0, (hipStream_t)stream>>>(model_out, x0, noise, tab_ca, tab_cb, tab_w, t, num_timesteps, nullptr, gscale,
+                                                                 dout, per_sample);
+    VAW_CHECK_LAUNCH("wmse_bwd_t");
     return VAW_OK;
 }
 
@@ -325,6 +422,14 @@
     for (int64_t i = blockIdx.x * (int64_t)blockDim.x + threadIdx.x; i < n; i += (int64_t)gridDim.x * blockDim.x)
         dx[i] = dy[i] * silu_grad_f(x[i]);
 }
+__global__ void silu_bwd_cast_kernel(const float* __restrict__ x, const float* __restrict__ dy, float* __restrict__ dx,
+                                     bf16_t* __restrict__ dx_lo, int64_t n) {
+    for (int64_t i = blockIdx.x * (int64_t)blockDim.x + threadIdx.x; i < n; i += (int64_t)gridDim.x * blockDim.x) {
+        const float d = dy[i] * silu_grad_f(x[i]);
+        dx[i] = d;
+        if (dx_lo) dx_lo[i] = (bf16_t)d;
+    }
+}
 extern "C" int vaw_silu_fwd(vaw_dtype dt, const float* x, void* out, int64_t n, vaw_stream stream) {
     VAW_CHECK_ARG(n > 0, "silu_fwd: n<=0");
     int grid = stream_grid(n, 256);
@@ -340,6 +445,25 @@
     return VAW_OK;
 }
 
+extern "C" int vaw_silu_bwd_cast(const float* x, const float* dy, float* dx, void* dx_bf16, int64_t n, vaw_stream stream) {
+    VAW_CHECK_ARG(n > 0 && x && dy && dx, "silu_bwd_cast: bad arguments");
+    silu_bwd_cast_kernel<<<stream_grid(n, 256), 256, 0, (hipStream_t)stream>>>(x, dy, dx, (bf16_t*)dx_bf16, n);
+    VAW_CHECK_LAUNCH("silu_bwd_cast");
+    return VAW_OK;
+}
+
+template <typename T>
+__global__ void add_embedding_silu_kernel(const float* __restrict__ a, const float* __restrict__ table,
+                                          const int64_t* __restrict__ idx, float* __restrict__ out, T* __restrict__ out_s, int B,
+                                          int D, int rows) {
+    for (int64_t i = blockIdx.x * (int64_t)blockDim.x + threadIdx.x; i < (int64_t)B * D; i += (int64_t)gridDim.x * blockDim.x) {
+        const int b = (int)(i / D), d = (int)(i % D);
+        const int64_t r = idx[b];
+        const float v = a[i] + ((r >= 0 && r < rows) ? table[r * D + d] : __builtin_nanf(""));
+        out[i] = v;
+        out_s[i] = from_f32<T>(silu_f(v));
+    }
+}
 __global__ void add_embedding_kernel(const float* __restrict__ a, const float* __restrict__ table,
                                      const int64_t* __restrict__ idx, float* __restrict__ out, int B, int D, int rows) {
     for (int64_t i = blockIdx.x * (int64_t)blockDim.x + threadIdx.x; i < (int64_t)B * D; i += (int64_t)gridDim.x * blockDim.x) {
@@ -388,6 +512,16 @@
     VAW_CHECK_ARG(B > 0 && D > 0 && num_rows > 0, "add_embedding: bad sizes");
     add_embedding_kernel<<<stream_grid((int64_t)B * D, 256), 256, 0, (hipStream_t)stream>>>(a, table, idx, out, B, D, num_rows);
     VAW_CHECK_LAUNCH("add_embedding");
+    return VAW_OK;
+}
+extern "C" int vaw_add_embedding_silu(vaw_dtype dt, const float* a, const float* table, const int64_t* idx, float* c, void* cs,
+                                      int B, int D, int num_rows, vaw_stream stream) {
+    VAW_CHECK_ARG(B > 0 && D > 0 && num_rows > 0 && a && table && idx && c && cs, "add_embedding_silu: bad arguments");
+    VAW_CHECK_ARG(dt == VAW_F32 || dt == VAW_BF16, "add_embedding_silu: dt");
+    const int grid = stream_grid((int64_t)B * D, 256);
+    if (dt == VAW_F32) add_embedding_silu_kernel<float><<<grid, 256, 0, (hipStream_t)stream>>>(a, table, idx, c, (float*)cs, B, D, num_rows);
+    else add_embedding_silu_kernel<bf16_t><<<grid, 256, 0, (hipStream_t)stream>>>(a, table, idx, c, (bf16_t*)cs, B, D, num_rows);
+    VAW_CHECK_LAUNCH("add_embedding_silu");
     return VAW_OK;
 }
 extern "C" int vaw_embedding_bwd(const float* dc, const int64_t* idx, float* dtable, int B, int D, int num_rows,
diff --git a/variance-aware-weight_amd/csrc/layernorm.hip b/variance-aware-weight_amd/csrc/layernorm.hip
--- a/variance-aware-weight_amd/csrc/layernorm.hip
+++ b/variance-aware-weight_amd/csrc/layernorm.hip
@@ -95,7 +95,8 @@
                const float* __restrict__ dres, const T* __restrict__ y, const float* __restrict__ gate,
                T* __restrict__ dy, float* __restrict__ dgate, float* __restrict__ dy_colpart,
                int rows_per_chunk, float* __restrict__ part,
-               unsigned char* __restrict__ q_out = nullptr, float* __restrict__ q_state = nullptr, int q_e5m2 = 0) {
+               unsigned char* __restrict__ q_out = nullptr, float* __restrict__ q_state = nullptr, int q_e5m2 = 0,
+               T* __restrict__ dx_lo = nullptr) {
     static_assert(!(FUSE && GATE_ONLY), "FUSE extends the LayerNorm mode");
     constexpr int NQ = FUSE ? 4 : 2;
     extern __shared__ __attribute__((aligned(16))) float lds[];
@@ -170,6 +171,7 @@
                     f32x4 r = (g[i] - c1 - xh[i] * c2) * rs;
                     if (dres_in) r += load4(dres_in + row * D + c);
                     store4(dx + row * D + c, r);
+                    if (dx_lo) store4(dx_lo + row * D + c, r);
                     if (FUSE) {
                         const f32x4 yv = load4(y + row * D + c);
                         const f32x4 d = r * load4(gsc_lds + c);
@@ -529,8 +531,17 @@
                                    const float* scale, int64_t mod_ld, const float* dres_in, float* dx, float* dshift,
                                    float* dscale, int64_t dmod_ld, int B, int T, int D, float* workspace,
                                    int64_t workspace_floats, vaw_stream stream) {
+    return vaw_ln_modulate_bwd_lo(dt, dout, x, mean, rstd, scale, mod_ld, dres_in, dx, nullptr, dshift, dscale, dmod_ld, B, T, D,
+                                  workspace, workspace_floats, stream);
+}
+
+extern "C" int vaw_ln_modulate_bwd_lo(vaw_dtype dt, const void* dout, const float* x, const float* mean, const float* rstd,
+                                      const float* scale, int64_t mod_ld, const float* dres_in, float* dx, void* dx_bf16,
+                                      float* dshift, float* dscale, int64_t dmod_ld, int B, int T, int D, float* workspace,
+                                      int64_t workspace_floats, vaw_stream stream) {
     VAW_CHECK_ARG(B > 0 && T > 0 && D > 0 && D % 4 == 0 && D <= 2048 && mod_ld % 4 == 0,
                   "ln_modulate_bwd: need D%%4==0, D<=2048, mod_ld%%4==0 (D=%d)", D);
+    VAW_CHECK_ARG(!dx_bf16 || (dt == VAW_BF16 && ((uintptr_t)dx_bf16 & 7) == 0), "ln_modulate_bwd: the bf16 copy of dx needs dt = bf16 and 8-byte alignment");
     ROW_PLAN(VAW_ROW_LN_BWD, dt, B, T, D, 0, 0, workspace ? workspace_floats : 0);
     hipStream_t s = (hipStream_t)stream;
     const int nc = plan.nc, rpc = plan.rows_per_chunk, block = plan.block;
@@ -540,7 +551,7 @@
     if (dt == VAW_F32) {
         DISPATCH_NV(plan.nv, (row_bwd_kernel<float, NV, false><<<grid, block, lds, s>>>((const float*)dout, x, mean, rstd, scale, mod_ld, dres_in, dx, dshift, dscale, dmod_ld, T, D, nullptr, nullptr, nullptr, nullptr, nullptr, nullptr, rpc, part)));
     } else {
-        DISPATCH_NV(plan.nv, (row_bwd_kernel<bf16_t, NV, false><<<grid, block, lds, s>>>((const bf16_t*)dout, x, mean, rstd, scale, mod_ld, dres_in, dx, dshift, dscale, dmod_ld, T, D, nullptr, nullptr, nullptr, nullptr, nullptr, nullptr, rpc, part)));
+        DISPATCH_NV(plan.nv, (row_bwd_kernel<bf16_t, NV, false><<<grid, block, lds, s>>>((const bf16_t*)dout, x, mean, rstd, scale, mod_ld, dres_in, dx, dshift, dscale, dmod_ld, T, D, nullptr, nullptr, nullptr, nullptr, nullptr, nullptr, rpc, part, nullptr, nullptr, 0, (bf16_t*)dx_bf16)));
     }
     if (nc > 1) row_bwd_finish_kernel<<<ceil_div((int64_t)B * D, 256), 256, 0, s>>>(part, nc, B, D, dshift, dmod_ld, dscale, dmod_ld);
     VAW_CHECK_LAUNCH("ln_modulate_bwd");
@@ -725,6 +736,31 @@
     }
 }
 
+__global__ void __launch_bounds__(256)
+colsum_cast_kernel(const float* __restrict__ X, bf16_t* __restrict__ Xa, int64_t M, int64_t N, int64_t ldx, float* __restrict__ out,
+                   float beta) {
+    __shared__ __attribute__((aligned(16))) float part[4][256];
+    const int cg = threadIdx.x & 63, rg = threadIdx.x >> 6;
+    const int64_t col = (int64_t)blockIdx.x * 256 + cg * 4;
+    f32x4 acc = {0, 0, 0, 0};
+    if (col < N) {
+        for (int64_t r = rg; r < M; r += 4) {
+            const f32x4 v = load4(X + r * ldx + col);
+            store4(Xa + r * ldx + col, v);
+            acc += f32x4{(float)(bf16_t)v[0], (float)(bf16_t)v[1], (float)(bf16_t)v[2], (float)(bf16_t)v[3]};
+        }
+    }
+    store4(&part[rg][cg * 4], acc);
+    __syncthreads();
+    const int64_t c = (int64_t)blockIdx.x * 256 + threadIdx.x;
+    if (c < N) {
+        const float p = ((part[0][threadIdx.x] + part[1][threadIdx.x]) + part[2][threadIdx.x]) + part[3][threadIdx.x];
+        float t = 0.f;
+        t += 0.f + p;
+        out[c] = (beta != 0.f ? beta * out[c] : 0.f) + t;
+    }
+}
+
 template <typename T>
 __global__ void colsum_partial_scalar_kernel(const T* __restrict__ X, int64_t M, int64_t N, int64_t ldx, float* __restrict__ part_out) {
     const int64_t c = (int64_t)blockIdx.x * blockDim.x + threadIdx.x;
@@ -818,3 +854,14 @@
     VAW_CHECK_LAUNCH("colsum");
     return VAW_OK;
 }
+
+extern "C" int vaw_colsum_cast(const float* X, void* Xa, int64_t M, int64_t N, int64_t ldx, float* out, float beta, vaw_stream stream) {
+    VAW_CHECK_ARG(X && Xa && out && M > 0 && N > 0 && ldx >= N, "colsum_cast: bad arguments");
+    if (M > 512 || N % 4 || ldx % 4 || ((uintptr_t)X & 15) || ((uintptr_t)Xa & 7)) {
+        vaw_set_error("colsum_cast: needs M <= 512, N %% 4 == 0, ldx %% 4 == 0 and aligned operands (M=%ld N=%ld ldx=%ld)", (long)M, (long)N, (long)ldx);
+        return VAW_ERR_UNSUPPORTED;
+    }
+    colsum_cast_kernel<<<ceil_div(N, 256), 256, 0, (hipStream_t)stream>>>(X, (bf16_t*)Xa, M, N, ldx, out, beta);
+    VAW_CHECK_LAUNCH("colsum_cast");
+    return VAW_OK;
+}
diff --git a/variance-aware-weight_amd/dit.py b/variance-aware-weight_amd/dit.py
--- a/variance-aware-weight_amd/dit.py
+++ b/variance-aware-weight_amd/dit.py
@@ -153,7 +153,7 @@
         if m._ws_cur.gen != ctx.gen:
             raise L.VawError("DiT backward: activations were overwritten by a later forward of the same batch size")
         dx = m._backward_impl(dout.contiguous(), ctx.need_dx)
-        return torch.zeros_like(m._anchor), None, dx, None, None
+        return (None if ops.STEP_FUSIONS else torch.zeros_like(m._anchor)), None, dx, None, None
 
 
 class DiT(FlatModule):
@@ -376,9 +376,13 @@
         L.check(lib.vaw_silu_fwd(dt, ptr(ws.h1), ptr(ws.h1s), B * D, st), "silu")
         ops.gemm(dt, 1, 1, B, D, D, ptr(ws.h1s), D, self._w("t_embedder.mlp.2.weight"), D, ptr(ws.temb), D,
                  bias=self._p32("t_embedder.mlp.2.bias"), out_f32=True)
-        L.check(lib.vaw_add_embedding(ptr(ws.temb), self._p32("y_embedder.embedding_table.weight"), ptr(ws.y), ptr(ws.c),
-                                      B, D, ye.embedding_table.num_embeddings, st), "add_embedding")
-        L.check(lib.vaw_silu_fwd(dt, ptr(ws.c), ptr(ws.cs), B * D, st), "silu")
+        if ops.STEP_FUSIONS:
+            L.check(lib.vaw_add_embedding_silu(dt, ptr(ws.temb), self._p32("y_embedder.embedding_table.weight"), ptr(ws.y), ptr(ws.c),
+                                               ptr(ws.cs), B, D, ye.embedding_table.num_embeddings, st), "add_embedding_silu")
+        else:
+            L.check(lib.vaw_add_embedding(ptr(ws.temb), self._p32("y_embedder.embedding_table.weight"), ptr(ws.y), ptr(ws.c),
+                                          B, D, ye.embedding_table.num_embeddings, st), "add_embedding")
+            L.check(lib.vaw_silu_fwd(dt, ptr(ws.c), ptr(ws.cs), B * D, st), "silu")
         self._need("ada_hi")
         ops.gemm(dt, 1, 1, B, ld, D, ptr(ws.cs), D, self._w("blocks.0.adaLN_modulation.1.weight"), D, ptr(ws.mod), ld,
                  bias=self._p32("blocks.0.adaLN_modulation.1.bias"), out_f32=True)
@@ -450,14 +454,19 @@
 
     def _adaln_wgrad(self, dt, ws, r0, nrows, B, beta):
         D, ld = self.D, self.mod_cols
+        db = self._g("blocks.0.adaLN_modulation.1.bias") + 4 * r0
+        summed = False
         if dt == BF16:
-            ops.cast_bf16(ws.dmod, ws.dmod_a)
             dmod_a, es = ptr(ws.dmod_a), 2
+            summed = ops.STEP_FUSIONS and ops.colsum_cast(ptr(ws.dmod) + 4 * r0, dmod_a + es * r0, B, nrows, ld, db, beta)
+            if not summed:
+                ops.cast_bf16(ws.dmod, ws.dmod_a)
         else:
             dmod_a, es = ptr(ws.dmod), 4
         ops.gemm(dt, 0, 0, nrows, D, ws.Bk, dmod_a + es * r0, ld, ptr(ws.cs), D, self._g("blocks.0.adaLN_modulation.1.weight") + 4 * r0 * D,
                  D, beta=beta, out_f32=True)
-        ops.colsum(dt, dmod_a + es * r0, B, nrows, ld, self._g("blocks.0.adaLN_modulation.1.bias") + 4 * r0, beta)
+        if not summed:
+            ops.colsum(dt, dmod_a + es * r0, B, nrows, ld, db, beta)
         return dmod_a
 
     def _backward_impl(self, dout, need_dx):
@@ -478,9 +487,11 @@
         own_dy = defer and not fp8
         fuse_rows = fp8 and ws.d_bwd and self.fp8_fuse_epilogue and self.fp8_fuse_rows and M % 64 == 0 and D % 128 == 0
 
+        dres_lo = ptr(ws.dao) if (ops.STEP_FUSIONS and dt == BF16) else 0
+
         def ln_bwd_and_gate(dout_p, x_p, mean_p, rstd_p, scale_p, dres_in, dsh, dsc, nxt):
             if nxt is None:
-                ops.ln_modulate_bwd(dt, dout_p, x_p, mean_p, rstd_p, scale_p, ld, dres_in, dres, dsh, dsc, ld, B, T, D)
+                ops.ln_modulate_bwd(dt, dout_p, x_p, mean_p, rstd_p, scale_p, ld, dres_in, dres, dsh, dsc, ld, B, T, D, dx_bf16=dres_lo)
                 return
             l2, which = nxt
             nb = ws.blk[l2]
@@ -515,11 +526,10 @@
                 names = [("cp_fc2", "mlp.fc2."), ("cp_fc1", "mlp.fc1."), ("cp_proj", "attn.proj.")] + ([("cp_qkv", "attn.qkv.")] if qkv_too else [])
                 cps += [(b[key_cp], pre + nm) for key_cp, nm in names]
             rows = tuple(int(cp.rows.value) for cp, _ in cps)
-            ent = ws.bias_groups.get(key)
-            if ent is None or ent[1] != rows:
+            grp = ws.bias_groups.get((key, rows))
+            if grp is None:
                 jobs = [(cp.buf.data_ptr(), self._g(nm + "bias"), r, cp.N) for (cp, nm), r in zip(cps, rows)]
-                ent = ws.bias_groups[key] = (ops.ReduceGroup(jobs, dout.device), rows)
-            grp = ent[0]
+                grp = ws.bias_groups[(key, rows)] = ops.ReduceGroup(jobs, dout.device)
             grp.launch(beta)
 
         def flush():
@@ -597,8 +607,9 @@
         pending.reverse()
         flush()
         if dt == BF16:
-            ops.cast_bf16(ws.dres, ws.dD)
-            dx0 = dD
+            if not dres_lo:
+                ops.cast_bf16(ws.dres, ws.dD)
+            dx0 = dres_lo or dD
         else:
             dx0 = dres
         self._wgrad(dt, "x_embedder.proj.", dx0, ptr(ws.xp), D, self.Kp, M, beta)
@@ -610,20 +621,29 @@
         rows = ld if ada_half is None else 6 * ada_half * D
         dmod_a = self._adaln_wgrad(dt, ws, 0, rows, B, beta)
         ops.gemm(dt, 1, 0, B, D, ld, dmod_a, ld, self._w("blocks.0.adaLN_modulation.1.weight"), D, ptr(ws.dcs), D, out_f32=True)
-        L.check(lib.vaw_silu_bwd(ptr(ws.c), ptr(ws.dcs), ptr(ws.dc), B * D, st), "silu_bwd")
+        fuse_cast = ops.STEP_FUSIONS and dt == BF16
+        if fuse_cast:
+            L.check(lib.vaw_silu_bwd_cast(ptr(ws.c), ptr(ws.dcs), ptr(ws.dc), ptr(ws.dc_a), B * D, st), "silu_bwd_cast")
+        else:
+            L.check(lib.vaw_silu_bwd(ptr(ws.c), ptr(ws.dcs), ptr(ws.dc), B * D, st), "silu_bwd")
         ye = self.y_embedder.embedding_table
         L.check(lib.vaw_embedding_bwd(ptr(ws.dc), ptr(ws.y), self._g("y_embedder.embedding_table.weight"), B, D,
                                       ye.num_embeddings, beta, st), "embedding_bwd")
         if dt == BF16:
-            ops.cast_bf16(ws.dc, ws.dc_a)
+            if not fuse_cast:
+                ops.cast_bf16(ws.dc, ws.dc_a)
             dc_a = ptr(ws.dc_a)
         else:
             dc_a = ptr(ws.dc)
         self._wgrad(dt, "t_embedder.mlp.2.", dc_a, ptr(ws.h1s), D, D, ws.Bk, beta)
         ops.gemm(dt, 1, 0, B, D, D, dc_a, D, self._w("t_embedder.mlp.2.weight"), D, ptr(ws.dh1s), D, out_f32=True)
-        L.check(lib.vaw_silu_bwd(ptr(ws.h1), ptr(ws.dh1s), ptr(ws.dh1), B * D, st), "silu_bwd")
+        if fuse_cast:
+            L.check(lib.vaw_silu_bwd_cast(ptr(ws.h1), ptr(ws.dh1s), ptr(ws.dh1), ptr(ws.dh1_a), B * D, st), "silu_bwd_cast")
+        else:
+            L.check(lib.vaw_silu_bwd(ptr(ws.h1), ptr(ws.dh1s), ptr(ws.dh1), B * D, st), "silu_bwd")
         if dt == BF16:
-            ops.cast_bf16(ws.dh1, ws.dh1_a)
+            if not fuse_cast:
+                ops.cast_bf16(ws.dh1, ws.dh1_a)
             dh1_a = ptr(ws.dh1_a)
         else:
             dh1_a = ptr(ws.dh1)
diff --git a/variance-aware-weight_amd/gaussian_diffusion.py b/variance-aware-weight_amd/gaussian_diffusion.py
--- a/variance-aware-weight_amd/gaussian_diffusion.py
+++ b/variance-aware-weight_amd/gaussian_diffusion.py
@@ -383,6 +383,30 @@
         return terms
 
 
+    def fused_latent_step_ok(self):
+        return (self.loss_type in (LossType.MSE, LossType.RESCALED_MSE) and not getattr(self.args, "learn_align", False) and
+                self.model_var_type not in (ModelVarType.LEARNED, ModelVarType.LEARNED_RANGE) and self.args.time_dist[0] == "uniform")
+
+    def latent_step_backward(self, model, latent, latent_scale, model_kwargs=None, gscale=None):
+        mean, _ = torch.chunk(latent, 2, dim=1)
+        eps = torch.randn_like(mean)
+        noise = torch.randn_like(eps)
+        B = latent.shape[0]
+        t = torch.randint(0, self.num_timesteps, (B,), device=latent.device)
+        tb = self._tables(latent.device)
+        t_mul = 1000.0 / self.num_timesteps if self.rescale_timesteps else None
+        x_start, x_t, t_in = ops.latent_qsample(latent.contiguous(), eps, noise, t, tb["a"], tb["s"], latent_scale, t_mul)
+        raw_output = model(x_t, t if t_in is None else t_in, **(model_kwargs or {}))
+        model_output = raw_output[0] if isinstance(raw_output, tuple) else raw_output
+        assert model_output.shape == x_start.shape
+        out = model_output.detach().contiguous()
+        mse, mean_loss = ops.wmse_fwd_t(out, x_start, noise, t, tb["ca"], tb["cb"], tb["w"])
+        g = float(np.float32(1.0) / np.float32(B)) if gscale is None else float(gscale)
+        dout = ops.wmse_bwd_t(out, x_start, noise, t, tb["ca"], tb["cb"], tb["w"], g)
+        model_output.backward(dout)
+        return mean_loss, mse
+
+
 class FlowMatching:
 
     def __init__(self, *, args, model_mean_type, device="cuda"):
diff --git a/variance-aware-weight_amd/ops.py b/variance-aware-weight_amd/ops.py
--- a/variance-aware-weight_amd/ops.py
+++ b/variance-aware-weight_amd/ops.py
@@ -1,9 +1,13 @@
 import ctypes as C
+import os
 
 import torch
 
 from . import _lib as L
 from ._lib import BF16, F32, AttnDesc, Epilogue, check, need_cuda, ptr, stream_ptr
+
+
+STEP_FUSIONS = os.environ.get("VAW_STEP_FUSIONS", "1") != "0"
 
 
 def dt_of(t):
@@ -39,6 +43,51 @@
     B = x.shape[0]
     check(L.lib().vaw_mix_rows(ptr(x), ptr(y), ptr(ca), ptr(cb), ptr(out), B, x.numel() // B, stream_ptr()), "vaw_mix_rows")
     return out
+
+
+def latent_qsample(latent, eps, noise, t, tab_a, tab_s, latent_scale, t_mul=None):
+    need_cuda(latent, eps, noise, t, tab_a, tab_s)
+    _f32c(latent, eps, noise, tab_a, tab_s)
+    B = latent.shape[0]
+    assert latent.shape[1] % 2 == 0 and eps.shape == noise.shape == (B, latent.shape[1] // 2, *latent.shape[2:])
+    assert t.dtype == torch.int64 and t.shape == (B,) and t.is_contiguous()
+    x0, xt = torch.empty_like(eps), torch.empty_like(eps)
+    ts = torch.empty(B, device=latent.device, dtype=torch.float32) if t_mul is not None else None
+    check(L.lib().vaw_latent_qsample(ptr(latent), ptr(eps), ptr(noise), ptr(t), ptr(tab_a), ptr(tab_s), tab_a.numel(), float(latent_scale),
+                                     float(t_mul or 0.0), ptr(x0), ptr(xt), ptr(ts), B, eps.numel() // B, stream_ptr()), "vaw_latent_qsample")
+    return x0, xt, ts
+
+
+def mean_f32(v, out=None):
+    need_cuda(v)
+    _f32c(v)
+    out = torch.empty(1, device=v.device, dtype=torch.float32) if out is None else out
+    check(L.lib().vaw_mean_f32(ptr(v), v.numel(), ptr(out), stream_ptr()), "vaw_mean_f32")
+    return out
+
+
+def wmse_fwd_t(model_out, x0, noise, t, tab_ca, tab_cb, tab_w, want_mean=True):
+    need_cuda(model_out, x0, noise, t, tab_ca, tab_cb, tab_w)
+    _f32c(model_out, x0, noise, tab_ca, tab_cb, tab_w)
+    B = x0.shape[0]
+    assert model_out.shape == x0.shape == noise.shape and t.dtype == torch.int64 and t.shape == (B,) and t.is_contiguous()
+    assert tab_ca.shape == tab_cb.shape == tab_w.shape
+    mse = torch.empty(B, device=x0.device, dtype=torch.float32)
+    mean = torch.empty(1, device=x0.device, dtype=torch.float32) if want_mean else None
+    check(L.lib().vaw_wmse_fwd_t(ptr(model_out), ptr(x0), ptr(noise), ptr(t), ptr(tab_ca), ptr(tab_cb), ptr(tab_w), tab_w.numel(), ptr(mse),
+                                 ptr(mean), B, x0.numel() // B, stream_ptr()), "vaw_wmse_fwd_t")
+    return mse, mean
+
+
+def wmse_bwd_t(model_out, x0, noise, t, tab_ca, tab_cb, tab_w, gscale):
+    need_cuda(model_out, x0, noise, t, tab_ca, tab_cb, tab_w)
+    _f32c(model_out, x0, noise, tab_ca, tab_cb, tab_w)
+    B = x0.shape[0]
+    assert model_out.shape == x0.shape == noise.shape and t.dtype == torch.int64 and t.shape == (B,) and t.is_contiguous()
+    dout = torch.empty_like(model_out)
+    check(L.lib().vaw_wmse_bwd_t(ptr(model_out), ptr(x0), ptr(noise), ptr(t), ptr(tab_ca), ptr(tab_cb), ptr(tab_w), tab_w.numel(),
+                                 float(gscale), ptr(dout), B, x0.numel() // B, stream_ptr()), "vaw_wmse_bwd_t")
+    return dout
 
 
 class _WeightedMSE(torch.autograd.Function):
@@ -418,6 +467,16 @@
     check(L.lib().vaw_colsum(dt, X, M, N, ldx, out, beta, ptr(ws), ws.numel(), stream_ptr()), "vaw_colsum")
 
 
+def colsum_cast(X, Xa, M, N, ldx, out, beta=0.0):
+    if M > 512 or N % 4 or ldx % 4 or X % 16 or Xa % 8:
+        return False
+    plan = row_plan(L.ROW_COLSUM, BF16, M, 1, N, ldx=ldx, base_addr=Xa)
+    if plan.variant != L.RV_COLSUM_VEC4 or plan.nc != 1:
+        return False
+    check(L.lib().vaw_colsum_cast(X, Xa, M, N, ldx, out, beta, stream_ptr()), "vaw_colsum_cast")
+    return True
+
+
 def ln_modulate_fwd(dt, x, shift, scale, mod_ld, out, mean, rstd, B, T, D, eps=1e-6):
     check(L.lib().vaw_ln_modulate_fwd(dt, x, shift, scale, mod_ld, out, mean, rstd, B, T, D, eps, stream_ptr()),
           "vaw_ln_modulate_fwd")
@@ -446,8 +505,12 @@
     return scratch_f32(torch.device("cuda", torch.cuda.current_device()), L.lib().vaw_row_bwd_workspace_floats(B, T, D))
 
 
-def ln_modulate_bwd(dt, dout, x, mean, rstd, scale, mod_ld, dres_in, dx, dshift, dscale, dmod_ld, B, T, D):
+def ln_modulate_bwd(dt, dout, x, mean, rstd, scale, mod_ld, dres_in, dx, dshift, dscale, dmod_ld, B, T, D, dx_bf16=0):
     ws = _row_ws(B, T, D)
+    if dx_bf16:
+        check(L.lib().vaw_ln_modulate_bwd_lo(dt, dout, x, mean, rstd, scale, mod_ld, dres_in or None, dx, dx_bf16, dshift, dscale,
+                                             dmod_ld, B, T, D, ws.data_ptr(), ws.numel(), stream_ptr()), "vaw_ln_modulate_bwd_lo")
+        return
     check(L.lib().vaw_ln_modulate_bwd(dt, dout, x, mean, rstd, scale, mod_ld, dres_in or None, dx, dshift, dscale,
                                       dmod_ld, B, T, D, ws.data_ptr(), ws.numel(), stream_ptr()), "vaw_ln_modulate_bwd")
 
diff --git a/variance-aware-weight_amd/trainer.py b/variance-aware-weight_amd/trainer.py
--- a/variance-aware-weight_amd/trainer.py
+++ b/variance-aware-weight_amd/trainer.py
@@ -1,5 +1,6 @@
 from contextlib import nullcontext
 
+import numpy as np
 import torch
 import torch.nn as nn
 
@@ -109,6 +110,11 @@
             return terms
         return self.diffusion.training_losses(self.model, images, features, model_kwargs=model_kwargs)
 
+    def _fused_latent_step(self):
+        d = self.diffusion
+        return (ops.STEP_FUSIONS and self.args.in_chans == 4 and not self._cpu_rng and self.schedule_sampler is None and
+                torch.device(self.device).type == "cuda" and hasattr(d, "fused_latent_step_ok") and d.fused_latent_step_ok())
+
     def _apply_gradient_clipping(self):
         if self.args.grad_clip:
             if self._fused:
@@ -132,6 +138,13 @@
 
     def _graph_body(self, images, labels):
         a = self.args
+        if self._fused_latent_step():
+            mean_loss, _ = self.diffusion.latent_step_backward(self.model, images, a.latent_scale, {"y": labels} if a.class_cond else {})
+            self._apply_gradient_clipping()
+            self.optimizer.step()
+            self.optimizer.zero_grad()
+            loss = mean_loss.reshape(())
+            return loss, loss
         if a.in_chans == 4:
             images = sample_from_latent(images, a.latent_scale, False)
         loss_dict = self._compute_loss(images, labels, None)
@@ -209,18 +222,27 @@
         total, mse_avg = None, None
         for i in range(accum):
             images, labels = self._get_next_batch()
-            if a.in_chans == 4:
+            fused = self._fused_latent_step()
+            if a.in_chans == 4 and not fused:
                 images = sample_from_latent(images, a.latent_scale, self._cpu_rng)
             if a.parallel and accum > 1 and i < accum - 1:
                 ctx = self.model.no_sync()
             else:
                 ctx = nullcontext()
-            with ctx:
-                loss_dict = self._compute_loss(images, labels, None)
-                loss = loss_dict["loss"].mean() / accum
-                loss.backward()
-            ld = loss.detach()
-            md = loss_dict["mse"].detach().mean() / accum if "mse" in loss_dict else torch.zeros_like(ld)
+            if fused:
+                inv_b = np.float32(1.0) / np.float32(images.shape[0])
+                gscale = inv_b if accum == 1 else (np.float32(1.0) / np.float32(accum)) * inv_b
+                with ctx:
+                    mean_loss, _ = self.diffusion.latent_step_backward(self.model, images, a.latent_scale,
+                                                                       {"y": labels} if a.class_cond else {}, gscale)
+                ld = md = mean_loss.reshape(()) if accum == 1 else mean_loss.reshape(()) / accum
+            else:
+                with ctx:
+                    loss_dict = self._compute_loss(images, labels, None)
+                    loss = loss_dict["loss"].mean() / accum
+                    loss.backward()
+                ld = loss.detach()
+                md = loss_dict["mse"].detach().mean() / accum if "mse" in loss_dict else torch.zeros_like(ld)
             total = ld if total is None else total + ld
             mse_avg = md if mse_avg is None else mse_avg + md
             if (i + 1) % accum == 0:
```

New measurement: 20220 images/sec (median of 6 runs). No clear change (+0.5%).
